# nikisalli/nightmare_rl

Hardware: AMD Instinct MI355X
Metric: env-steps/sec at N parallel Nightmare-v3 envs, 1/2/4/8 MI355X (higher is better)
Workload: dtype f32; 1 GPU; 4096 Nightmare-v3 envs per GPU, random-action rollout U(-1,1)^18, full step(): 2 x 8 ms substeps (18-DoF dynamics + floor contact, PGS x3 + noslip x4) + obs/reward/termination/reset; envs_per_gpu=4096, decimation=2

## Files before the change

### nightmare_rl_amd/csrc/nm_core.h

```cpp
#pragma once
#include <type_traits>
#include <stddef.h>

#include "simt.h"

#ifdef NM_MEASURE
#define NM_ABLATE(mask) (mask)
#else
#define NM_ABLATE(mask) 0
#endif
namespace nm {
using namespace simt;

constexpr int kNQ = 25, kNV = 24, kNU = 18, kNLEG = 6, kNCOL = 7, kNSENS = 13, kNOBS = 66, kNREW = 16;
constexpr int kLinkN = 25;
constexpr int kLegN = 3 * kLinkN;
constexpr int kBaseN = 10;
constexpr int kColN = 24;
constexpr int kMaxCon = 16;
constexpr int kMaxRow = 4 * kMaxCon;
constexpr int kMaxConBig = 44;
constexpr int kBigSlots = (4 * kMaxConBig + NM_WAVE - 1) / NM_WAVE;
constexpr int kJRow = 16;
enum { R_ACTION_RATE, R_ANG_VEL_XY, R_BASE_HEIGHT, R_BODY_CONTACT, R_DEFAULT_POS, R_DOF_ACC, R_DOF_VEL, R_FEET_AIR_TIME, R_FEET_CONTACT,
       R_LIN_VEL_Z, R_ORIENTATION, R_STAND_STILL, R_TORQUES, R_TRACK_ANG, R_TRACK_LIN, R_TERMINATION };

template <class real> struct Model {
  const real* hullv;
  const real* hullnv;
  real legc[kNLEG * kLegN];
  real basec[kBaseN];
  real colc[kNCOL * kColN];
  real footc[kNLEG * 4];
  real qpos0[kNQ];
  int maxnbr;
  int link_rot_id[3];
  real total_mass;
  real h, kv, ctrl_max, grav, mu;
  real solref_K, solref_B, si_d0, si_dmax, si_width, si_mid, si_power;
  real pgs_scale, pgs_tol, noslip_tol, tol_planemesh;
  int pgs_iters, noslip_iters, mpr_iters;
  real mpr_tol;
  real dt, p_gain, clip_obs, obs_lin, obs_ang, obs_dofpos, obs_dofvel, max_lin_x, max_ang, term_force, sigma, max_ep_len, default_pos[3];
  float action_scale, clip_actions;
  int resample_every;
  real rew_scale[kNREW];
  real ep_len_s;
  int rew_extra;
  int tibia_mode, body_mode;
  int collide_batch_min;
  real tibia_max, body_max, base_h_target, max_contact_force;
};

template <class real> struct Args {
  int N;
  uint64_t seed;
  int64_t env_offset;
  real *qpos, *qvel, *qwarm;
  real *dofpos, *dofvel, *act, *cmd, *epsum;
  real* feetair;
  int* feetflags;
  int64_t* eplen;
  uint32_t* rngctr;
  int* hullcache;
  const float* actions;
  const real* cmd_u;
  float *obs, *rew, *timeout_now;
  float* ret_acc;
  int64_t* done;
  real* stat_sum;
  int* stat_cnt;
  int* wave_done;
  int *nto, *to_list;
  int *nprev, *to_prev;
  unsigned long long* to_owner;
  float *ep_stats, *time_outs;
  long long* counters;
  real* dbg;
  int nsub;
  int nxcd;
  int physics_only;
  int ablate;
  const real* noise_vec;
  const real* noise_u;
  uint64_t noise_step;
  real* rec;
  int rec_env;
};
constexpr int kTicketGroup = 64, kTicketStride = 32, kTicketTop = 0;
constexpr uint64_t kNoiseKey = 0x4E4F495345ull;
constexpr int kDbgN = 256;

template <class real> struct Sh {
  real qpos[28], qvel[24], warm[24], ctrl[20];
  real Rb[9], wv[6];
  real anc[kNU * 3], axs[kNU * 3];
  real colR[kNCOL * 9], colp[kNCOL * 3];
  real Minv[kNLEG * 6], W[kNLEG * 18], Lb[15], Dbi[6];
  real MinvH[kNLEG * 6], WH[kNLEG * 18], LbH[15], DbiH[6];
  real qas[24], qfs[24], qfc[24];
  real vv[24];
  real sens[16], cvb[6];
  real bh[2];
  real mbb[36], sc[36];
  real legtmp[kNLEG * 66];
  NM_FN real* cpos() { return legtmp; }
  NM_FN real* cnrm() { return legtmp + 3 * kMaxConBig; }
  NM_FN real* cdist() { return legtmp + 6 * kMaxConBig; }
  NM_FN int* cleg() { return reinterpret_cast<int*>(legtmp + 7 * kMaxConBig); }
  NM_FN int* cleg1() { return reinterpret_cast<int*>(legtmp + 8 * kMaxConBig); }
  real efc_f[kMaxRow];
#ifdef NM_DEBUG_SOLVER
  real dbg_b[kMaxRow], dbg_a[kMaxRow], dbg_f0[kMaxRow];
#endif
  int ncon, nwarn, it_pgs, it_noslip, anypair;
  int nhop;
  int ntog;
  real eact[kNU], epact[kNU], epdv[kNU];
  real ecmd[4], eepsum[kNREW];
  int eplen_lo, eplen_hi;
  unsigned ectr;
  int cstart[8], ccnt[8];
  real sink[NM_WAVE];
  int hcache[8];
};

static_assert(kNLEG * 66 >= 9 * kMaxConBig, "contact list must fit the leg staging area");
template <class real, int G> struct ShW {
  Sh<real> e[G];
  alignas(16) real jrow[kMaxRow * kJRow];
};
#define NM_OFS(field) ((int)(offsetof(Sh<real>, field) / sizeof(real)))
#define NM_IOFS(field) ((int)(offsetof(Sh<real>, field) / sizeof(int)))

template <class A, class B, class C> NM_FN void cross3(A* r, const B* a, const C* b) {
  A x = a[1] * b[2] - a[2] * b[1], y = a[2] * b[0] - a[0] * b[2], z = a[0] * b[1] - a[1] * b[0];
  r[0] = x; r[1] = y; r[2] = z;
}
template <class A, class B, class C> NM_FN A dot3(const B* a, const C* b) { return a[0] * b[0] + a[1] * b[1] + a[2] * b[2]; }
template <class A, class B, class C> NM_FN void matvec3(A* r, const B* m, const C* v) {
  A x = m[0] * v[0] + m[1] * v[1] + m[2] * v[2], y = m[3] * v[0] + m[4] * v[1] + m[5] * v[2], z = m[6] * v[0] + m[7] * v[1] + m[8] * v[2];
  r[0] = x; r[1] = y; r[2] = z;
}
template <class A, class B, class C> NM_FN void matvec3_fma(A* r, const B* m, const C* v) {
  A x = vfma(A(m[2]), A(v[2]), vfma(A(m[1]), A(v[1]), A(m[0]) * A(v[0])));
  A y = vfma(A(m[5]), A(v[2]), vfma(A(m[4]), A(v[1]), A(m[3]) * A(v[0])));
  A z = vfma(A(m[8]), A(v[2]), vfma(A(m[7]), A(v[1]), A(m[6]) * A(v[0])));
  r[0] = x; r[1] = y; r[2] = z;
}
template <class A, class B, class C> NM_FN void matmul3(A* r, const B* a, const C* b) {
#pragma unroll
  for (int i = 0; i < 3; i++)
#pragma unroll
    for (int j = 0; j < 3; j++) r[3 * i + j] = a[3 * i] * b[j] + a[3 * i + 1] * b[3 + j] + a[3 * i + 2] * b[6 + j];
}
template <class A, class B, class C> NM_FN void inert_mul(A* r, const B* i, const C* v) {
  r[0] = i[0] * v[0] + i[3] * v[1] + i[4] * v[2] - i[8] * v[4] + i[7] * v[5];
  r[1] = i[3] * v[0] + i[1] * v[1] + i[5] * v[2] + i[8] * v[3] - i[6] * v[5];
  r[2] = i[4] * v[0] + i[5] * v[1] + i[2] * v[2] - i[7] * v[3] + i[6] * v[4];
  r[3] = i[8] * v[1] - i[7] * v[2] + i[9] * v[3];
  r[4] = i[6] * v[2] - i[8] * v[0] + i[9] * v[4];
  r[5] = i[7] * v[0] - i[6] * v[1] + i[9] * v[5];
}
template <class A, class B, class C> NM_FN void cross_motion(A* r, const B* vel, const C* v) {
  A a[3], b[3], c[3];
  cross3(a, vel, v); cross3(b, vel, v + 3); cross3(c, vel + 3, v);
  r[0] = a[0]; r[1] = a[1]; r[2] = a[2]; r[3] = b[0] + c[0]; r[4] = b[1] + c[1]; r[5] = b[2] + c[2];
}
template <class A, class B, class C> NM_FN void cross_force(A* r, const B* vel, const C* f) {
  A a[3], b[3], c[3];
  cross3(a, vel, f); cross3(b, vel + 3, f + 3); cross3(c, vel, f + 3);
  r[0] = a[0] + b[0]; r[1] = a[1] + b[1]; r[2] = a[2] + b[2]; r[3] = c[0]; r[4] = c[1]; r[5] = c[2];
}
template <class A, class B, class C> NM_FN A dot6(const B* a, const C* b) {
  return a[0] * b[0] + a[1] * b[1] + a[2] * b[2] + a[3] * b[3] + a[4] * b[4] + a[5] * b[5];
}
template <class real> NM_FN real lanesum6(const V<real>& x) {
  return ((rdlane(x, 0) + rdlane(x, 1)) + (rdlane(x, 2) + rdlane(x, 3))) + (rdlane(x, 4) + rdlane(x, 5));
}
template <class X, class real> NM_FN void spatial_inertia(X* I10, const X* R, const X* Ib, const X* d, X m, real) {
  X T[9];
#pragma unroll
  for (int i = 0; i < 3; i++) {
    T[3 * i + 0] = R[3 * i] * Ib[0] + R[3 * i + 1] * Ib[3] + R[3 * i + 2] * Ib[4];
    T[3 * i + 1] = R[3 * i] * Ib[3] + R[3 * i + 1] * Ib[1] + R[3 * i + 2] * Ib[5];
    T[3 * i + 2] = R[3 * i] * Ib[4] + R[3 * i + 1] * Ib[5] + R[3 * i + 2] * Ib[2];
  }
  X xx = T[0] * R[0] + T[1] * R[1] + T[2] * R[2], yy = T[3] * R[3] + T[4] * R[4] + T[5] * R[5], zz = T[6] * R[6] + T[7] * R[7] + T[8] * R[8];
  X xy = T[0] * R[3] + T[1] * R[4] + T[2] * R[5], xz = T[0] * R[6] + T[1] * R[7] + T[2] * R[8], yz = T[3] * R[6] + T[4] * R[7] + T[5] * R[8];
  I10[0] = xx + m * (d[1] * d[1] + d[2] * d[2]);
  I10[1] = yy + m * (d[0] * d[0] + d[2] * d[2]);
  I10[2] = zz + m * (d[0] * d[0] + d[1] * d[1]);
  I10[3] = xy - m * d[0] * d[1];
  I10[4] = xz - m * d[0] * d[2];
  I10[5] = yz - m * d[1] * d[2];
  I10[6] = m * d[0]; I10[7] = m * d[1]; I10[8] = m * d[2];
  I10[9] = m;
}
template <class X, class real> NM_FN void ldl3(X* r, const X* a, real one) {
  X i2 = vrcp(a[5]);
  X l21 = a[4] * i2, l20 = a[2] * i2;
  X m11 = a[3] - l21 * a[4], m01 = a[1] - l21 * a[2], m00 = a[0] - l20 * a[2];
  X i1 = vrcp(m11);
  X l10 = m01 * i1;
  X d0 = m00 - l10 * m01;
  r[0] = l21; r[1] = l20; r[2] = l10; r[3] = i2; r[4] = i1; r[5] = vrcp(d0);
}
template <class X, class Y> NM_FN void ldl3_solve(X* x, const X* f, const Y* y) {
  X y2 = y[2];
  X y1 = y[1] - f[0] * y2;
  X y0 = y[0] - f[1] * y2 - f[2] * y1;
  X x0 = y0 * f[5];
  X x1 = y1 * f[4] - f[2] * x0;
  x[2] = y2 * f[3] - f[0] * x1 - f[1] * x0;
  x[1] = x1; x[0] = x0;
}
template <class X, class real, class Acc> NM_FN void ldl6(Acc S, X* L, X* Dinv, real one) {
  X Lf[36], D[6];
#pragma unroll
  for (int j = 0; j < 6; j++) {
    X d = S(j, j);
#pragma unroll
    for (int k = 0; k < j; k++) d = d - Lf[6 * j + k] * Lf[6 * j + k] * D[k];
    D[j] = d;
    X di = vrcp(d);
    Dinv[j] = di;
#pragma unroll
    for (int i = j + 1; i < 6; i++) {
      X s = S(j, i);
#pragma unroll
      for (int k = 0; k < j; k++) s = s - Lf[6 * i + k] * Lf[6 * j + k] * D[k];
      Lf[6 * i + j] = s * di;
    }
  }
  int n = 0;
#pragma unroll
  for (int i = 1; i < 6; i++)
#pragma unroll
    for (int j = 0; j < i; j++) L[n++] = Lf[6 * i + j];
}
template <class LT, class X> NM_FN void ldl6_solve(const LT* L, const LT* Dinv, X* x) {
  int n = 0;
#pragma unroll
  for (int i = 1; i < 6; i++)
#pragma unroll
    for (int j = 0; j < i; j++) x[i] = x[i] - L[n++] * x[j];
#pragma unroll
  for (int i = 0; i < 6; i++) x[i] = x[i] * Dinv[i];
#pragma unroll
  for (int i = 5; i >= 1; i--) {
    n = i * (i - 1) / 2;
#pragma unroll
    for (int j = 0; j < i; j++) x[j] = x[j] - L[n + j] * x[i];
  }
}

NM_FN uint32_t rand_u24_bits(uint64_t seed, uint64_t genv, uint32_t ctr) {
  uint64_t x = seed + 0x9E3779B97F4A7C15ull * (genv + 1) + 0xD1B54A32D192ED03ull * (uint64_t)ctr;
  x ^= x >> 30; x *= 0xBF58476D1CE4E5B9ull;
  x ^= x >> 27; x *= 0x94D049BB133111EBull;
  x ^= x >> 31;
  return (uint32_t)(x >> 40);
}

#ifndef NM_EMUL
template <class T> NM_FN void nm_consume(T x) { asm volatile("" ::"v"(x) : "memory"); }
#endif

#if defined(NM_STAMPS) && !defined(NM_EMUL)
__device__ unsigned long long g_stamps[16];
NM_FN void nm_stamp(int k) {
  __shared__ unsigned long long tl, acc[16];
#ifdef NM_STAMPS_B
  asm volatile("s_waitcnt vmcnt(0) lgkmcnt(0)" ::: "memory");
#endif
  unsigned long long n = __builtin_amdgcn_s_memtime();
  if (NM_TID == 0) {
    if (k < 0) for (int i = 0; i < 16; i++) acc[i] = 0;
    else acc[k] += n - tl;
    if (k == 10) for (int i = 0; i < 16; i++) atomicAdd(&g_stamps[i], acc[i]);
    tl = n;
  }
}
#else
NM_FN void nm_stamp(int) {}
#endif
#ifdef NM_STAMPS_B
#define NM_ESTAMP(k)
#define NM_BSTAMP(k) nm_stamp(k)
#else
#define NM_ESTAMP(k) nm_stamp(k)
#define NM_BSTAMP(k)
#endif

constexpr int kLinkTmp = 22;

template <class real> NM_FN V<real> legsum(const V<real>& x, const VB& isleg) {
  return gsum8(sel(isleg, x, V<real>(real(0))));
}

template <class real, int G> NM_FN void stage_smooth(ShW<real, G>& w, const Model<real>& M, bool last) {
  typedef V<real> vr;
  real* lds = reinterpret_cast<real*>(&w.e[0]);
  static_assert((G & (G - 1)) == 0 && 2 * G <= 8, "lane groups: G envs x 2 factorisations");
  const V<int> lane0 = opaque_lane();
  const V<int> sub = lane0 & 7, grp = lane0 >> 3;
  const V<int> leg = vmin(sub, V<int>(5)), eo = (grp & (G - 1)) * (int)(sizeof(Sh<real>) / sizeof(real));
  const VB pass1 = (grp & G) != 0;
  const VB isleg = sub < V<int>(6);
#define LDG(field, i) ldsv(lds, eo + (NM_OFS(field) + (i)))
  const VB st_all = VB(true), st_leg = VB(true);
#define STG(field, i, val) stsv(lds, eo + (NM_OFS(field) + (i)), val, st_all)
#define LDL(field, idx) ldsv(lds, eo + (idx) + NM_OFS(field))
#define STL(field, idx, val) stsv(lds, eo + (idx) + NM_OFS(field), val, st_leg)
  const V<int> slot = leg * (3 * kLinkTmp);

  vr Rb[9];
  {
    vr qw = LDG(qpos, 3), qx = LDG(qpos, 4), qy = LDG(qpos, 5), qz = LDG(qpos, 6);
    {
      const vr in_ = vrcp(vsqrt(qw * qw + qx * qx + qy * qy + qz * qz));
      qw = qw * in_; qx = qx * in_; qy = qy * in_; qz = qz * in_;
      STG(qpos, 3, qw); STG(qpos, 4, qx); STG(qpos, 5, qy); STG(qpos, 6, qz);
    }
    vr q00 = qw * qw, q01 = qw * qx, q02 = qw * qy, q03 = qw * qz, q11 = qx * qx, q12 = qx * qy, q13 = qx * qz, q22 = qy * qy,
       q23 = qy * qz, q33 = qz * qz;
    Rb[0] = q00 + q11 - q22 - q33; Rb[4] = q00 - q11 + q22 - q33; Rb[8] = q00 - q11 - q22 + q33;
    Rb[1] = real(2) * (q12 - q03); Rb[2] = real(2) * (q13 + q02); Rb[3] = real(2) * (q12 + q03);
    Rb[5] = real(2) * (q23 - q01); Rb[6] = real(2) * (q13 - q02); Rb[7] = real(2) * (q23 + q01);
  }
  vr vb[6], ab[6];
  {
    vr wl[3] = {LDG(qvel, 3), LDG(qvel, 4), LDG(qvel, 5)};
    matvec3(vb, Rb, wl);
    vb[3] = LDG(qvel, 0); vb[4] = LDG(qvel, 1); vb[5] = LDG(qvel, 2);
    vr t[3];
    cross3(t, vb + 3, vb);
    ab[0] = ab[1] = ab[2] = vr(real(0));
    ab[3] = t[0]; ab[4] = t[1]; ab[5] = t[2] + M.grav;
  }
#pragma unroll
  for (int j = 0; j < 9; j++) { STG(colR, j, Rb[j]); STG(Rb, j, Rb[j]); }
#pragma unroll
  for (int j = 0; j < 3; j++) STG(colp, j, vr(real(0)));
#pragma unroll
  for (int j = 0; j < 6; j++) STG(wv, j, vb[j]);

  const V<int> mylink = (grp >> (G == 1 ? 0 : (G == 2 ? 1 : 2))) & 3;
  const VB isbase = mylink == 3;
#ifndef NM_NO_ROLE_ROT
  {
    const V<int> lk = vmin(mylink, V<int>(2));
    const V<int> cbr = leg * kLegN + lk * kLinkN;
    const vr ax[3] = {ldsv(M.legc, cbr + 12), ldsv(M.legc, cbr + 13), ldsv(M.legc, cbr + 14)};
    vr s_, co;
    vsincos(LDL(qpos, leg * 3 + lk + 7), &s_, &co);
    const vr oc = vr(real(1)) - co;
    vr Rl[9];
    Rl[0] = co + oc * ax[0] * ax[0]; Rl[1] = oc * ax[0] * ax[1] - s_ * ax[2]; Rl[2] = oc * ax[0] * ax[2] + s_ * ax[1];
    Rl[3] = oc * ax[0] * ax[1] + s_ * ax[2]; Rl[4] = co + oc * ax[1] * ax[1]; Rl[5] = oc * ax[1] * ax[2] - s_ * ax[0];
    Rl[6] = oc * ax[0] * ax[2] - s_ * ax[1]; Rl[7] = oc * ax[1] * ax[2] + s_ * ax[0]; Rl[8] = co + oc * ax[2] * ax[2];
#pragma unroll
    for (int j = 0; j < 9; j++) STL(legtmp, leg * 27 + lk * 9 + j, Rl[j]);
    wave_sync();
  }
#endif
  vr mcom[3] = {vr(real(0)), vr(real(0)), vr(real(0))};
  {
    vr Rp[9], pp[3], vpar[6], apar[6];
    vr cR[9], cpos[3], cS[6], cv[6], ca[6];
#pragma unroll
    for (int k = 0; k < 9; k++) Rp[k] = Rb[k];
    pp[0] = pp[1] = pp[2] = vr(real(0));
#pragma unroll
    for (int k = 0; k < 6; k++) { vpar[k] = vb[k]; apar[k] = ab[k]; }
#pragma unroll
    for (int k = 0; k < 3; k++) {
      sched_fence();
      const V<int> cb = leg * kLegN + k * kLinkN;
      vr q = LDL(qpos, leg * 3 + (7 + k)), qd = LDL(qvel, leg * 3 + (6 + k));
      vr pos[3], t3[3], aw[3], R[9];
      {
        vr bpos[3] = {ldsv(M.legc, cb), ldsv(M.legc, cb + 1), ldsv(M.legc, cb + 2)};
        matvec3(t3, Rp, bpos);
        pos[0] = pp[0] + t3[0]; pos[1] = pp[1] + t3[1]; pos[2] = pp[2] + t3[2];
      }
      {
        vr ax[3] = {ldsv(M.legc, cb + 12), ldsv(M.legc, cb + 13), ldsv(M.legc, cb + 14)};
        vr R0[9];
        {
          if (uniform(M.link_rot_id[k])) {
#pragma unroll
            for (int j = 0; j < 9; j++) R0[j] = Rp[j];
          } else {
            vr bR[9];
#pragma unroll
            for (int j = 0; j < 9; j++) bR[j] = ldsv(M.legc, cb + 3 + j);
            matmul3(R0, Rp, bR);
          }
        }
        matvec3(aw, R0, ax);
        vr Rl[9];
#ifndef NM_NO_ROLE_ROT
#pragma unroll
        for (int j = 0; j < 9; j++) Rl[j] = LDL(legtmp, leg * 27 + (k * 9 + j));
        (void)q;
#else
        vr s, co;
        vsincos(q, &s, &co);
        vr oc = vr(real(1)) - co;
        Rl[0] = co + oc * ax[0] * ax[0]; Rl[1] = oc * ax[0] * ax[1] - s * ax[2]; Rl[2] = oc * ax[0] * ax[2] + s * ax[1];
        Rl[3] = oc * ax[0] * ax[1] + s * ax[2]; Rl[4] = co + oc * ax[1] * ax[1]; Rl[5] = oc * ax[1] * ax[2] - s * ax[0];
        Rl[6] = oc * ax[0] * ax[2] - s * ax[1]; Rl[7] = oc * ax[1] * ax[2] + s * ax[0]; Rl[8] = co + oc * ax[2] * ax[2];
#endif
        matmul3(R, R0, Rl);
      }
#pragma unroll
      for (int j = 0; j < 3; j++) {
        STL(anc, leg * 9 + (3 * k + j), pos[j]);
        STL(axs, leg * 9 + (3 * k + j), aw[j]);
      }
      if (k == 2) {
#pragma unroll
        for (int j = 0; j < 9; j++) STL(colR, (leg + 1) * 9 + j, R[j]);
#pragma unroll
        for (int j = 0; j < 3; j++) STL(colp, (leg + 1) * 3 + j, pos[j]);
      }
      sched_fence();
      vr S[6];
      S[0] = aw[0]; S[1] = aw[1]; S[2] = aw[2];
      cross3(S + 3, pos, aw);
      {
        vr Sd[6];
        cross_motion(Sd, vpar, S);
#pragma unroll
        for (int j = 0; j < 6; j++) {
          vpar[j] = vpar[j] + S[j] * qd;
          apar[j] = apar[j] + Sd[j] * qd;
        }
      }
      if (k == 0) {
#pragma unroll
        for (int j = 0; j < 9; j++) cR[j] = sel(isbase, Rb[j], R[j]);
#pragma unroll
        for (int j = 0; j < 3; j++) cpos[j] = sel(isbase, vr(real(0)), pos[j]);
#pragma unroll
        for (int j = 0; j < 6; j++) { cS[j] = S[j]; cv[j] = sel(isbase, vb[j], vpar[j]); ca[j] = sel(isbase, ab[j], apar[j]); }
      } else {
        const VB mine = mylink == k;
#pragma unroll
        for (int j = 0; j < 9; j++) cR[j] = sel(mine, R[j], cR[j]);
#pragma unroll
        for (int j = 0; j < 3; j++) cpos[j] = sel(mine, pos[j], cpos[j]);
#pragma unroll
        for (int j = 0; j < 6; j++) { cS[j] = sel(mine, S[j], cS[j]); cv[j] = sel(mine, vpar[j], cv[j]); ca[j] = sel(mine, apar[j], ca[j]); }
      }
#pragma unroll
      for (int j = 0; j < 9; j++) Rp[j] = R[j];
      pp[0] = pos[0]; pp[1] = pos[1]; pp[2] = pos[2];
    }
    sched_fence();
    {
      static_assert(offsetof(Model<real>, basec) == offsetof(Model<real>, legc) + sizeof(real) * kNLEG * kLegN, "basec follows legc");
      const V<int> cbm = sel(isbase, V<int>(kNLEG * kLegN - 15), leg * kLegN + mylink * kLinkN);
      vr I10[10], f[6];
      {
        vr ipos[3] = {ldsv(M.legc, cbm + 15), ldsv(M.legc, cbm + 16), ldsv(M.legc, cbm + 17)};
        vr Ib[6];
#pragma unroll
        for (int j = 0; j < 6; j++) Ib[j] = ldsv(M.legc, cbm + 18 + j);
        vr mass = ldsv(M.legc, cbm + 24);
        vr d[3], t3[3];
        matvec3(t3, cR, ipos);
        d[0] = cpos[0] + t3[0]; d[1] = cpos[1] + t3[1]; d[2] = cpos[2] + t3[2];
        spatial_inertia(I10, cR, Ib, d, mass, real(0));
        mcom[0] = mass * d[0]; mcom[1] = mass * d[1]; mcom[2] = mass * d[2];
      }
      {
        vr t6[6], u6[6];
        inert_mul(t6, I10, ca);
        inert_mul(u6, I10, cv);
        cross_force(f, cv, u6);
#pragma unroll
        for (int j = 0; j < 6; j++) f[j] = f[j] + t6[j];
      }
      const V<int> o = sel(isbase, V<int>(NM_OFS(sc) + 9 - NM_OFS(legtmp)), slot + mylink * kLinkTmp);
#pragma unroll
      for (int j = 0; j < 6; j++) STL(legtmp, o + j, cS[j]);
#pragma unroll
      for (int j = 0; j < 10; j++) STL(legtmp, o + (6 + j), I10[j]);
#pragma unroll
      for (int j = 0; j < 6; j++) STL(legtmp, o + (16 + j), f[j]);
      if (last) {
#pragma unroll
        for (int j = 0; j < 3; j++) stsv(lds, eo + mylink * 3 + (NM_OFS(sc) + j), legsum<real>(mcom[j], isleg), st_all);
      }
    }
  }
  wave_sync();

  vr Ml[6], Mlb[3][6], cl[3], fs[6], Ic[10];
#pragma unroll
  for (int j = 0; j < 6; j++) fs[j] = vr(real(0));
#pragma unroll
  for (int j = 0; j < 10; j++) Ic[j] = vr(real(0));
#pragma unroll
  for (int k = 2; k >= 0; k--) {
    sched_fence();
    const V<int> o = slot + k * kLinkTmp;
    vr S[6], F[6];
#pragma unroll
    for (int j = 0; j < 6; j++) S[j] = LDL(legtmp, o + j);
#pragma unroll
    for (int j = 0; j < 10; j++) Ic[j] += LDL(legtmp, o + (6 + j));
#pragma unroll
    for (int j = 0; j < 6; j++) fs[j] += LDL(legtmp, o + (16 + j));
    cl[k] = dot6<vr>(S, fs);
    inert_mul(F, Ic, S);
    Mlb[k][0] = F[3]; Mlb[k][1] = F[4]; Mlb[k][2] = F[5];
#pragma unroll
    for (int j = 0; j < 3; j++) Mlb[k][3 + j] = F[0] * Rb[j] + F[1] * Rb[3 + j] + F[2] * Rb[6 + j];
    const int dk = (k == 0) ? 0 : (k == 1 ? 3 : 5);
    Ml[dk] = dot6<vr>(S, F);
#pragma unroll
    for (int jj = 0; jj < k; jj++) {
      vr Sj[6];
#pragma unroll
      for (int j = 0; j < 6; j++) Sj[j] = LDL(legtmp, slot + (jj * kLinkTmp + j));
      Ml[(jj == 0) ? k : 4] = dot6<vr>(Sj, F);
    }
  }
  sched_fence();
  vr Icb[10], cbias[6];
  {
    vr Ib10[10];
#pragma unroll
    for (int j = 0; j < 10; j++) Ib10[j] = LDG(sc, 15 + j);
    if (last) {
      vr ipos[3] = {vr(M.basec[0]), vr(M.basec[1]), vr(M.basec[2])};
      vr d[3];
      matvec3(d, Rb, ipos);
      vr cr[3], t[3];
#pragma unroll
      for (int j = 0; j < 3; j++) cr[j] = (M.basec[9] * d[j] + (LDG(sc, j) + LDG(sc, 3 + j) + LDG(sc, 6 + j))) / M.total_mass;
      cross3(t, vb, cr);
#pragma unroll
      for (int j = 0; j < 3; j++) { STG(cvb, j, vb[j]); STG(cvb, 3 + j, vb[3 + j] + t[j]); }
      STG(bh, 0, LDG(qpos, 2) + d[2]);
    }
    vr fb[6];
#pragma unroll
    for (int j = 0; j < 6; j++) fb[j] = LDG(sc, 25 + j) + legsum<real>(fs[j], isleg);
    cbias[0] = fb[3]; cbias[1] = fb[4]; cbias[2] = fb[5];
#pragma unroll
    for (int j = 0; j < 3; j++) cbias[3 + j] = Rb[j] * fb[0] + Rb[3 + j] * fb[1] + Rb[6 + j] * fb[2];
#pragma unroll
    for (int j = 0; j < 10; j++) Icb[j] = Ib10[j] + legsum<real>(Ic[j], isleg);
  }
  {
#pragma unroll
    for (int i = 0; i < 3; i++)
#pragma unroll
      for (int j = i; j < 3; j++) STG(mbb, 6 * i + j, (i == j) ? Icb[9] : vr(real(0)));
    vr T[9];
#pragma unroll
    for (int j = 0; j < 3; j++) {
      vr a[3] = {Rb[j], Rb[3 + j], Rb[6 + j]}, c[3];
      cross3(c, a, Icb + 6);
#pragma unroll
      for (int i = 0; i < 3; i++) STG(mbb, 6 * i + 3 + j, c[i]);
      T[j] = Icb[0] * a[0] + Icb[3] * a[1] + Icb[4] * a[2];
      T[3 + j] = Icb[3] * a[0] + Icb[1] * a[1] + Icb[5] * a[2];
      T[6 + j] = Icb[4] * a[0] + Icb[5] * a[1] + Icb[2] * a[2];
    }
#pragma unroll
    for (int i = 0; i < 3; i++)
#pragma unroll
      for (int j = i; j < 3; j++) STG(mbb, 6 * (3 + i) + 3 + j, Rb[i] * T[j] + Rb[3 + i] * T[3 + j] + Rb[6 + i] * T[6 + j]);
  }
  wave_sync();

  {
    sched_fence();
    constexpr int kFacH = NM_OFS(MinvH) - NM_OFS(Minv);
    static_assert(NM_OFS(WH) - NM_OFS(W) == kFacH && NM_OFS(LbH) - NM_OFS(Lb) == kFacH && NM_OFS(DbiH) - NM_OFS(Dbi) == kFacH, "factor blocks");
    static_assert(kNLEG * 66 >= 36 + 24 + 24, "leg staging area holds the second Schur complement and the junk rows");
    const V<int> eoF = eo + sel(pass1, V<int>(kFacH), V<int>(0));
    const V<int> eoS = eo + sel(pass1, V<int>(NM_OFS(legtmp)), V<int>(NM_OFS(sc)));
    const V<int> eoQ = eo + sel(pass1, V<int>(NM_OFS(legtmp) + 36), V<int>(NM_OFS(qfs)));
    const V<int> eoA = eo + sel(pass1, V<int>(NM_OFS(legtmp) + 60), V<int>(NM_OFS(qas)));
    vr Mh[6];
    const vr dg = sel(pass1, vr(M.h * M.kv), vr(real(0)));
    Mh[0] = Ml[0] + dg; Mh[1] = Ml[1]; Mh[2] = Ml[2]; Mh[3] = Ml[3] + dg; Mh[4] = Ml[4]; Mh[5] = Ml[5] + dg;
    vr Mi[6], W[3][6];
    ldl3(Mi, Mh, real(1));
#pragma unroll
    for (int j = 0; j < 6; j++) {
      vr col[3] = {Mlb[0][j], Mlb[1][j], Mlb[2][j]}, r3[3];
      ldl3_solve(r3, Mi, col);
      W[0][j] = r3[0]; W[1][j] = r3[1]; W[2][j] = r3[2];
    }
#pragma unroll
    for (int j = 0; j < 6; j++) stsv(lds, eoF + leg * 6 + (NM_OFS(Minv) + j), Mi[j], st_leg);
#pragma unroll
    for (int k = 0; k < 3; k++)
#pragma unroll
      for (int j = 0; j < 6; j++) stsv(lds, eoF + leg * 18 + (NM_OFS(W) + 6 * k + j), W[k][j], st_leg);
#pragma unroll
    for (int i = 0; i < 6; i++)
#pragma unroll
      for (int j = i; j < 6; j++) {
        vr cij = Mlb[0][i] * W[0][j] + Mlb[1][i] * W[1][j] + Mlb[2][i] * W[2][j];
        stsv(lds, eoS + (6 * i + j), LDG(mbb, 6 * i + j) - legsum<real>(cij, isleg), st_all);
      }
    wave_sync();
    vr L[15], Di[6];
    ldl6([&](int r, int c) { return ldsv(lds, eoS + (6 * r + c)); }, L, Di, real(1));
#pragma unroll
    for (int j = 0; j < 15; j++) stsv(lds, eoF + (NM_OFS(Lb) + j), L[j], st_all);
#pragma unroll
    for (int j = 0; j < 6; j++) stsv(lds, eoF + (NM_OFS(Dbi) + j), Di[j], st_all);
    {
      vr y[3], t[3];
#pragma unroll
      for (int k = 0; k < 3; k++) {
        vr ctrl = LDL(ctrl, leg * 3 + k), qd = LDL(qvel, leg * 3 + (6 + k));
        ctrl = vmin(vmax(ctrl, vr(-M.ctrl_max)), vr(M.ctrl_max));
        y[k] = M.kv * ctrl - M.kv * qd - cl[k];
        stsv(lds, eoQ + leg * 3 + (6 + k), y[k], st_leg);
      }
      ldl3_solve(t, Mi, y);
      vr xb[6];
#pragma unroll
      for (int j = 0; j < 6; j++) {
        vr wy = W[0][j] * y[0] + W[1][j] * y[1] + W[2][j] * y[2];
        xb[j] = -cbias[j] - legsum<real>(wy, isleg);
        stsv(lds, eoQ + j, -cbias[j], st_all);
      }
      ldl6_solve(L, Di, xb);
#pragma unroll
      for (int j = 0; j < 6; j++) stsv(lds, eoA + j, xb[j], st_all);
#pragma unroll
      for (int k = 0; k < 3; k++) {
        vr x = t[k];
#pragma unroll
        for (int j = 0; j < 6; j++) x = x - W[k][j] * xb[j];
        stsv(lds, eoA + leg * 3 + (6 + k), x, st_leg);
      }
    }
  }
  wave_sync();
#undef LDG
#undef STG
#undef LDL
#undef STL
}

template <class real> struct Sup { real v[3], v1[3], v2[3]; };
template <class real> NM_FN real ccd_eps() { return sizeof(real) == 8 ? real(2.220446049250313e-16) : real(1.1920929e-7); }
template <class real> NM_FN bool ccd_zero(real x) { return vabs(x) < ccd_eps<real>(); }
template <class real> NM_FN bool ccd_eq(real a, real b) {
  real ab = vabs(a - b);
  if (ab < ccd_eps<real>()) return true;
  real fa = vabs(a), fb = vabs(b);
  return ab < ccd_eps<real>() * (fb > fa ? fb : fa);
}
template <class acc, class real> NM_FN void hull_support(const Sh<real>& sh, const Model<real>& M, int g, const acc* dir, acc* out) {
  typedef V<acc> vr;
  const V<int> lane = lane_id();
  acc R[9], p[3];
#pragma unroll
  for (int j = 0; j < 9; j++) R[j] = (acc)sh.colR[9 * g + j];
#pragma unroll
  for (int j = 0; j < 3; j++) p[j] = (acc)sh.colp[3 * g + j];
  const real* cc = M.colc + kColN * g;
  const int nvert = (int)cc[5], vadr = (int)cc[6];
  const acc ld[3] = {R[0] * dir[0] + R[3] * dir[1] + R[6] * dir[2], R[1] * dir[0] + R[4] * dir[1] + R[7] * dir[2],
                     R[2] * dir[0] + R[5] * dir[1] + R[8] * dir[2]};
  vr best = vr(acc(-1e30));
  for (int it = 0; it * NM_WAVE < nvert; it++) {
    V<int> vi = lane + it * NM_WAVE;
    VB ok = vi < nvert;
    V<int> ad = (sel(ok, vi, V<int>(0)) + vadr) * 4;
    vr val = ld[0] * vcvt<acc>(gldv(M.hullv, ad)) + ld[1] * vcvt<acc>(gldv(M.hullv, ad + 1)) + ld[2] * vcvt<acc>(gldv(M.hullv, ad + 2));
    best = sel(ok & (val > best), val, best);
  }
  acc sv; int si;
  wargmax(best, lane, &sv, &si);
  V<int> ifirst = V<int>(1 << 30);
  for (int it = 0; it * NM_WAVE < nvert; it++) {
    V<int> vi = lane + it * NM_WAVE;
    VB ok = vi < nvert;
    V<int> ad = (sel(ok, vi, V<int>(0)) + vadr) * 4;
    vr val = ld[0] * vcvt<acc>(gldv(M.hullv, ad)) + ld[1] * vcvt<acc>(gldv(M.hullv, ad + 1)) + ld[2] * vcvt<acc>(gldv(M.hullv, ad + 2));
    ifirst = sel(ok & (val >= vr(sv - acc(1e-7))) & (vi < ifirst), vi, ifirst);
  }
  wargmax(to_real<acc>(-ifirst), lane, &sv, &si);
  si = (int)(-sv);
  const real* vp = M.hullv + 4 * (vadr + si);
  const acc v[3] = {(acc)vp[0], (acc)vp[1], (acc)vp[2]};
  acc t[3];
  matvec3(t, R, v);
  out[0] = p[0] + t[0]; out[1] = p[1] + t[1]; out[2] = p[2] + t[2];
}
template <class acc, class real> NM_COLD void mpr_support(const Sh<real>& sh, const Model<real>& M, int g1, int g2, const acc* dir, Sup<acc>& s) {
  acc nd[3] = {-dir[0], -dir[1], -dir[2]};
  hull_support<acc>(sh, M, g1, dir, s.v1);
  hull_support<acc>(sh, M, g2, nd, s.v2);
  s.v[0] = s.v1[0] - s.v2[0]; s.v[1] = s.v1[1] - s.v2[1]; s.v[2] = s.v1[2] - s.v2[2];
}
template <class real> NM_FN void sub3(real* r, const real* a, const real* b) { r[0] = a[0] - b[0]; r[1] = a[1] - b[1]; r[2] = a[2] - b[2]; }
template <class real> NM_FN void ccd_normalize(real* v) { real s = real(1) / vsqrt(v[0] * v[0] + v[1] * v[1] + v[2] * v[2]); v[0] *= s; v[1] *= s; v[2] *= s; }
template <class real> NM_FN void portal_dir(const Sup<real>* p, real* dir) {
  real a[3], b[3];
  sub3(a, p[2].v, p[1].v); sub3(b, p[3].v, p[1].v);
  cross3(dir, a, b);
  ccd_normalize(dir);
}
template <class real> NM_FN bool portal_reach_tol(const Sup<real>* p, const Sup<real>& v4, const real* dir, real tol) {
  real dv4 = dot3<real>(v4.v, dir);
  real d1 = dv4 - dot3<real>(p[1].v, dir), d2 = dv4 - dot3<real>(p[2].v, dir), d3 = dv4 - dot3<real>(p[3].v, dir);
  real m = vmin(vmin(d1, d2), d3);
  return ccd_eq(m, tol) || m < tol;
}
template <class real> NM_FN void expand_portal(Sup<real>* p, const Sup<real>& v4) {
  real v4v0[3];
  cross3(v4v0, v4.v, p[0].v);
  if (dot3<real>(p[1].v, v4v0) > real(0)) {
    if (dot3<real>(p[2].v, v4v0) > real(0)) p[1] = v4; else p[3] = v4;
  } else {
    if (dot3<real>(p[3].v, v4v0) > real(0)) p[2] = v4; else p[1] = v4;
  }
}
template <class real> NM_FN real point_seg_dist2(const real* x0, const real* b, real* wit) {
  real dd[3];
  sub3(dd, b, x0);
  real t = -dot3<real>(x0, dd) / dot3<real>(dd, dd);
  if (t < real(0) || ccd_zero(t)) { wit[0] = x0[0]; wit[1] = x0[1]; wit[2] = x0[2]; }
  else if (t > real(1) || ccd_eq(t, real(1))) { wit[0] = b[0]; wit[1] = b[1]; wit[2] = b[2]; }
  else { wit[0] = x0[0] + t * dd[0]; wit[1] = x0[1] + t * dd[1]; wit[2] = x0[2] + t * dd[2]; }
  return dot3<real>(wit, wit);
}
template <class real> NM_FN real point_tri_dist2(const real* x0, const real* B, const real* C, real* wit) {
  real d1[3], d2[3];
  sub3(d1, B, x0); sub3(d2, C, x0);
  real v = dot3<real>(d1, d1), w = dot3<real>(d2, d2), p = dot3<real>(x0, d1), q = dot3<real>(x0, d2), r = dot3<real>(d1, d2);
  real dd = w * v - r * r, s, t;
  if (ccd_zero(dd)) { s = real(-1); t = real(-1); }
  else { s = (q * r - w * p) / dd; t = (-s * r - q) / w; }
  if ((ccd_zero(s) || s > real(0)) && (ccd_eq(s, real(1)) || s < real(1)) && (ccd_zero(t) || t > real(0)) && (ccd_eq(t, real(1)) || t < real(1)) &&
      (ccd_eq(t + s, real(1)) || t + s < real(1))) {
    wit[0] = x0[0] + s * d1[0] + t * d2[0]; wit[1] = x0[1] + s * d1[1] + t * d2[1]; wit[2] = x0[2] + s * d1[2] + t * d2[2];
    return dot3<real>(wit, wit);
  }
  real w2[3];
  real dist = point_seg_dist2(x0, B, wit);
  real dist2 = point_seg_dist2(x0, C, w2);
  if (dist2 < dist) { dist = dist2; wit[0] = w2[0]; wit[1] = w2[1]; wit[2] = w2[2]; }
  dist2 = point_seg_dist2(B, C, w2);
  if (dist2 < dist) { dist = dist2; wit[0] = w2[0]; wit[1] = w2[1]; wit[2] = w2[2]; }
  return dist;
}
template <class real_, class st> NM_COLD bool mpr_penetration(const Sh<st>& sh, const Model<st>& M, int g1, int g2, real_* depth, real_* dir_out, real_* pos) {
  typedef real_ real;
  Sup<real> p[4], v4;
  real dir[3], va[3], vb[3], dot;
  const real mpr_tol = (real)M.mpr_tol;
  {
    real R1[9], R2[9], c1[3], c2[3];
#pragma unroll
    for (int k = 0; k < 9; k++) { R1[k] = (real)sh.colR[9 * g1 + k]; R2[k] = (real)sh.colR[9 * g2 + k]; }
#pragma unroll
    for (int k = 0; k < 3; k++) { c1[k] = (real)M.colc[kColN * g1 + k]; c2[k] = (real)M.colc[kColN * g2 + k]; }
    real t1[3], t2[3];
    matvec3(t1, R1, c1); matvec3(t2, R2, c2);
#pragma unroll
    for (int k = 0; k < 3; k++) {
      p[0].v1[k] = (real)sh.colp[3 * g1 + k] + t1[k];
      p[0].v2[k] = (real)sh.colp[3 * g2 + k] + t2[k];
      p[0].v[k] = p[0].v1[k] - p[0].v2[k];
    }
  }
  if (ccd_eq(p[0].v[0], real(0)) && ccd_eq(p[0].v[1], real(0)) && ccd_eq(p[0].v[2], real(0))) p[0].v[0] += ccd_eps<real>() * real(10);
  dir[0] = -p[0].v[0]; dir[1] = -p[0].v[1]; dir[2] = -p[0].v[2];
  ccd_normalize(dir);
  mpr_support<real>(sh, M, g1, g2, dir, p[1]);
  dot = dot3<real>(p[1].v, dir);
  if (ccd_zero(dot) || dot < real(0)) return false;
  cross3(dir, p[0].v, p[1].v);
  if (ccd_zero(dot3<real>(dir, dir))) {
    if (ccd_eq(p[1].v[0], real(0)) && ccd_eq(p[1].v[1], real(0)) && ccd_eq(p[1].v[2], real(0))) return false;
    *depth = vsqrt(dot3<real>(p[1].v, p[1].v));
    dir_out[0] = p[1].v[0]; dir_out[1] = p[1].v[1]; dir_out[2] = p[1].v[2];
    ccd_normalize(dir_out);
#pragma unroll
    for (int k = 0; k < 3; k++) pos[k] = real(0.5) * (p[1].v1[k] + p[1].v2[k]);
    return true;
  }
  ccd_normalize(dir);
  mpr_support<real>(sh, M, g1, g2, dir, p[2]);
  dot = dot3<real>(p[2].v, dir);
  if (ccd_zero(dot) || dot < real(0)) return false;
  sub3(va, p[1].v, p[0].v); sub3(vb, p[2].v, p[0].v);
  cross3(dir, va, vb);
  ccd_normalize(dir);
  if (dot3<real>(dir, p[0].v) > real(0)) {
    Sup<real> t = p[1]; p[1] = p[2]; p[2] = t;
    dir[0] = -dir[0]; dir[1] = -dir[1]; dir[2] = -dir[2];
  }
  for (int size = 3, guard = 0; size < 4; guard++) {
    if (guard > 64) return false;
    mpr_support<real>(sh, M, g1, g2, dir, p[3]);
    dot = dot3<real>(p[3].v, dir);
    if (ccd_zero(dot) || dot < real(0)) return false;
    bool cont = false;
    cross3(va, p[1].v, p[3].v);
    dot = dot3<real>(va, p[0].v);
    if (dot < real(0) && !ccd_zero(dot)) { p[2] = p[3]; cont = true; }
    if (!cont) {
      cross3(va, p[3].v, p[2].v);
      dot = dot3<real>(va, p[0].v);
      if (dot < real(0) && !ccd_zero(dot)) { p[1] = p[3]; cont = true; }
    }
    if (cont) {
      sub3(va, p[1].v, p[0].v); sub3(vb, p[2].v, p[0].v);
      cross3(dir, va, vb);
      ccd_normalize(dir);
    } else size = 4;
  }
  for (int guard = 0;; guard++) {
    portal_dir(p, dir);
    dot = dot3<real>(dir, p[1].v);
    if (ccd_zero(dot) || dot > real(0)) break;
    if (guard > 100) return false;
    mpr_support<real>(sh, M, g1, g2, dir, v4);
    dot = dot3<real>(v4.v, dir);
    if (!(ccd_zero(dot) || dot > real(0)) || portal_reach_tol(p, v4, dir, mpr_tol)) return false;
    expand_portal(p, v4);
  }
  for (int it = 0;; it++) {
    portal_dir(p, dir);
    mpr_support<real>(sh, M, g1, g2, dir, v4);
    if (portal_reach_tol(p, v4, dir, mpr_tol) || it > M.mpr_iters) {
      real pd[3];
      *depth = vsqrt(point_tri_dist2(p[1].v, p[2].v, p[3].v, pd));
      if (ccd_zero(pd[0]) && ccd_zero(pd[1]) && ccd_zero(pd[2])) { pd[0] = dir[0]; pd[1] = dir[1]; pd[2] = dir[2]; }
      ccd_normalize(pd);
      dir_out[0] = pd[0]; dir_out[1] = pd[1]; dir_out[2] = pd[2];
      real b[4], t[3], sum;
      portal_dir(p, dir);
      cross3(t, p[1].v, p[2].v); b[0] = dot3<real>(t, p[3].v);
      cross3(t, p[3].v, p[2].v); b[1] = dot3<real>(t, p[0].v);
      cross3(t, p[0].v, p[1].v); b[2] = dot3<real>(t, p[3].v);
      cross3(t, p[2].v, p[1].v); b[3] = dot3<real>(t, p[0].v);
      sum = b[0] + b[1] + b[2] + b[3];
      if (ccd_zero(sum) || sum < real(0)) {
        b[0] = real(0);
        cross3(t, p[2].v, p[3].v); b[1] = dot3<real>(t, dir);
        cross3(t, p[3].v, p[1].v); b[2] = dot3<real>(t, dir);
        cross3(t, p[1].v, p[2].v); b[3] = dot3<real>(t, dir);
        sum = b[1] + b[2] + b[3];
      }
      real inv = real(1) / sum;
#pragma unroll
      for (int k = 0; k < 3; k++) {
        real p1 = b[0] * p[0].v1[k] + b[1] * p[1].v1[k] + b[2] * p[2].v1[k] + b[3] * p[3].v1[k];
        real p2 = b[0] * p[0].v2[k] + b[1] * p[1].v2[k] + b[2] * p[2].v2[k] + b[3] * p[3].v2[k];
        pos[k] = real(0.5) * (p1 * inv + p2 * inv);
      }
      return true;
    }
    expand_portal(p, v4);
  }
}

template <class real> NM_FN void pairs_narrow(Sh<real>& sh, const Model<real>& M, int* dropped, uint64_t m) {
  if (!m) return;
  int ncon = sh.ncon;
  while (m) {
    int pidx = __builtin_ctzll(m);
    m &= m - 1;
    int a = (pidx >= 5) + (pidx >= 9) + (pidx >= 12) + (pidx >= 14);
    int s0 = a == 0 ? 0 : (a == 1 ? 5 : (a == 2 ? 9 : (a == 3 ? 12 : 14)));
    int h1 = a + 1, h2 = h1 + 1 + (pidx - s0);
    {
      const real *R1 = sh.colR + 9 * h1, *R2 = sh.colR + 9 * h2, *k1 = M.colc + kColN * h1, *k2 = M.colc + kColN * h2;
      real t1[3], t2[3], dd[3];
      matvec3(t1, R1, k1); matvec3(t2, R2, k2);
#pragma unroll
      for (int k = 0; k < 3; k++) dd[k] = (sh.colp[3 * h1 + k] + t1[k]) - (sh.colp[3 * h2 + k] + t2[k]);
      real bound = k1[3] + k2[3];
      if (dot3<real>(dd, dd) > bound * bound) continue;
    }
    typedef double acc;
    acc depth, dir[3], pos[3];
    if (!mpr_penetration<acc>(sh, M, h1, h2, &depth, dir, pos)) continue;
    if (!(depth > acc(0))) continue;
    if (ncon >= kMaxConBig) { *dropped += 1; continue; }
    sh.cpos()[3 * ncon] = (real)pos[0]; sh.cpos()[3 * ncon + 1] = (real)pos[1]; sh.cpos()[3 * ncon + 2] = (real)pos[2];
    sh.cnrm()[3 * ncon] = (real)dir[0]; sh.cnrm()[3 * ncon + 1] = (real)dir[1]; sh.cnrm()[3 * ncon + 2] = (real)dir[2];
    sh.cdist()[ncon] = (real)(-depth);
    sh.cleg()[ncon] = h2 - 1;
    sh.cleg1()[ncon] = h1 - 1;
    sh.anypair = 1;
    ncon++;
  }
  sh.ncon = ncon;
  wave_sync();
}


template <class real> NM_FN void stage_collide_pairs(Sh<real>& sh, const Model<real>& M, int* dropped) {
  typedef V<real> vr;
  const V<int> lane = lane_id();
  const VB isp = lane < 15;
  const V<int> pl = sel(isp, lane, V<int>(0));
  V<int> i1 = sel(pl >= 5, V<int>(1), V<int>(0)) + sel(pl >= 9, V<int>(1), V<int>(0)) + sel(pl >= 12, V<int>(1), V<int>(0)) +
              sel(pl >= 14, V<int>(1), V<int>(0));
  V<int> st = sel(i1 == 0, V<int>(0), sel(i1 == 1, V<int>(5), sel(i1 == 2, V<int>(9), sel(i1 == 3, V<int>(12), V<int>(14)))));
  V<int> g1 = i1 + 1, g2 = g1 + 1 + (pl - st);
  vr c1[3], c2[3], e[2];
  V<int> gg[2] = {g1, g2};
  vr u[3];
#pragma unroll
// ... 98 lines not shown
    best = sel(take, val, best);
    ibest = sel(take, vi, ibest);
  }
  real sv; int si;
  wmaxfirst(best, &sv, &si);
  if (popc64(ballot(best == vr(sv))) == 1) return rdlane(ibest, si);
  wargmax(best, ibest, &sv, &si);
  return si;
}
template <class real> NM_FN real hull_tie_tol() { return sizeof(real) == 8 ? real(1e-13) : real(4e-7); }
constexpr int kMaxHop = 3;
template <class real> constexpr real kObbSlack() { return real(1e-5); }

constexpr int kSelfLane = 63;
constexpr int kSlackScale = 1 << 20;
constexpr int kBatchLane0 = kSelfLane + 1 - kNCOL;
template <class real> NM_FN void hull_ring(const Model<real>& M, int gv, V<int>& nbg, V<real>* v) {
  const V<int> lane = lane_id();
  const VB nbl = lane < M.maxnbr;
  V<real> o[4];
  gld4(M.hullnv, (sel(nbl, lane, V<int>(M.maxnbr)) + gv * (M.maxnbr + 1)) * 4, o);
  v[0] = o[0]; v[1] = o[1]; v[2] = o[2];
  nbg = to_int(o[3]);
}
template <class real> struct Rings {
  V<int> nb[kNCOL];
  V<real> vv[kNCOL][3];
  int cur[kNCOL];
};
template <class real> NM_FN void collide_rings(const Sh<real>& sh, const Model<real>& M, Rings<real>& r) {
#pragma unroll
  for (int g = 0; g < kNCOL; g++) {
    const int vadr = (int)M.colc[kColN * g + 6];
    r.cur[g] = uniform(sh.hcache[g]);
    hull_ring(M, vadr + r.cur[g], r.nb[g], r.vv[g]);
  }
}
template <class real> NM_FN void stage_collide(Sh<real>& sh, const Model<real>& M, int* dropped, Rings<real>& rg, bool pairs = true) {
  typedef V<real> vr;
  const V<int> lane = lane_id();
  const real bz = sh.qpos[2];
  const VB nbl = lane < M.maxnbr;
  V<int>* nb = rg.nb;
  vr (*vv)[3] = rg.vv;
  int* cur = rg.cur;
  real pz[kNCOL], ldv[kNCOL][3], sv[kNCOL];
  bool near[kNCOL];
  vr val[kNCOL];
#pragma unroll
  for (int g = 0; g < kNCOL; g++) {
    const real* R = sh.colR + 9 * g;
    const real* cc = M.colc + kColN * g;
    pz[g] = sh.colp[3 * g + 2] + bz;
    const real cz = R[6] * cc[0] + R[7] * cc[1] + R[8] * cc[2] + pz[g];
    near[g] = !(cz - cc[3] > real(0));
    ldv[g][0] = -R[6]; ldv[g][1] = -R[7]; ldv[g][2] = -R[8];
    val[g] = ldv[g][0] * vv[g][0] + ldv[g][1] * vv[g][1] + ldv[g][2] * vv[g][2];
    sv[g] = rdlane(val[g], kSelfLane);
  }
  NM_BSTAMP(11);
#pragma unroll
  for (int g = 0; g < kNCOL; g++) {
    const real tol = hull_tie_tol<real>();
    if (near[g] && wany(nbl & (nb[g] >= 0) & (val[g] >= vr(sv[g] - tol)))) {
      {
        const real* cc = M.colc + kColN * g;
        real top = ldv[g][0] * cc[8] + ldv[g][1] * cc[9] + ldv[g][2] * cc[10];
#pragma unroll
        for (int a = 0; a < 3; a++) top += cc[20 + a] * vabs(ldv[g][0] * cc[11 + 3 * a] + ldv[g][1] * cc[12 + 3 * a] + ldv[g][2] * cc[13 + 3 * a]);
        if (uniform(pz[g] - top > kObbSlack<real>())) { near[g] = false; continue; }
      }
      const int nvert = (int)M.colc[kColN * g + 5], vadr = (int)M.colc[kColN * g + 6];
      const real* ld = ldv[g];
      int si = cur[g];
      bool full = false;
      for (int hop = 0;; hop++) {
        const VB nbv = nbl & (nb[g] >= 0);
        if (!wany(nbv & (val[g] >= vr(sv[g] - tol)))) break;
        if (hop == kMaxHop || !wany(nbv & (val[g] > vr(sv[g] + tol)))) { full = true; break; }
        real bv; int lbest;
        wmaxfirst(sel(nbv, val[g], vr(real(-1e30))), &bv, &lbest);
        si = rdlane(nb[g], lbest);
        NM_BSTAMP(12);
        hull_ring(M, vadr + si, nb[g], vv[g]);
        val[g] = ld[0] * vv[g][0] + ld[1] * vv[g][1] + ld[2] * vv[g][2];
        sv[g] = rdlane(val[g], kSelfLane);
        NM_BSTAMP(14);
        sh.nhop += 1;
      }
      if (full) {
        NM_BSTAMP(12);
        const int held = si;
        si = support_exhaustive(M, ld, nvert, vadr);
        sh.hcache[7] += 1;
#ifdef NM_MEASURE
        sh.nhop += g == 0 ? 1000 : 100000;
#endif
        if (si != held) {
          hull_ring(M, vadr + si, nb[g], vv[g]);
          val[g] = ld[0] * vv[g][0] + ld[1] * vv[g][1] + ld[2] * vv[g][2];
          sv[g] = rdlane(val[g], kSelfLane);
        }
        NM_BSTAMP(15);
      }
      if (si != cur[g]) sh.hcache[g] = si;
    }
  }
  NM_BSTAMP(12);
  int total = 0;
  unsigned hitbits = 0;
#pragma unroll
  for (int g = 0; g < kNCOL; g++) hitbits |= (uniform(near[g] && pz[g] - sv[g] < real(0)) ? 1u : 0u) << g;
  const int nhit = popc64(hitbits);
  bool batch = false;
  if (nhit >= M.collide_batch_min) {
    const uint64_t hitm = (uint64_t)hitbits << kBatchLane0;
    vr X[3] = {vv[kNCOL - 1][0], vv[kNCOL - 1][1], vv[kNCOL - 1][2]}, svl = val[kNCOL - 1];
    V<int> slackl = nb[kNCOL - 1];
    V<int> lb = lane;
#pragma unroll
    for (int g = kNCOL - 2; g >= 0; g--) {
      order_after(lb, X[0]);
      const VB mg = lb == kBatchLane0 + g;
      X[0] = sel(mg, vv[g][0], X[0]); X[1] = sel(mg, vv[g][1], X[1]); X[2] = sel(mg, vv[g][2], X[2]);
      svl = sel(mg, val[g], svl);
      slackl = sel(mg, nb[g], slackl);
    }
    const VB ml = lane >= kBatchLane0;
    const V<int> gl = sel(ml, lane - kBatchLane0, V<int>(0));
    const vr pzl = ldsv(sh.colp, gl * 3 + 2) + bz;
    const vr distl = pzl - svl;
    const VB wr = in_mask(hitm);
    const VB lone = distl * real(-0.5 * kSlackScale) < to_real<real>(slackl);
    if (!wany(wr & !lone)) {
      vr Rl[9], pl[2], pnt[3];
#pragma unroll
      for (int j = 0; j < 9; j++) Rl[j] = ldsv(sh.colR, gl * 9 + j);
#pragma unroll
      for (int j = 0; j < 2; j++) pl[j] = ldsv(sh.colp, gl * 3 + j);
      matvec3_fma(pnt, Rl, X);
      pnt[0] = pnt[0] + pl[0]; pnt[1] = pnt[1] + pl[1]; pnt[2] = pnt[2] + ldsv(sh.colp, gl * 3 + 2);
      const V<int> slot = lane_rank(hitm);
      const V<int> sl = sel(wr, slot, V<int>(0));
      stsv(sh.cpos(), sl * 3, pnt[0], wr);
      stsv(sh.cpos(), sl * 3 + 1, pnt[1], wr);
      stsv(sh.cpos(), sl * 3 + 2, pnt[2] - real(0.5) * distl, wr);
      stsv(sh.cdist(), sl, distl, wr);
      stsv(sh.cleg(), sl, gl - 1, wr);
      stsv(sh.cstart, gl, slot, ml);
      stsv(sh.ccnt, gl, sel(wr, V<int>(1), V<int>(0)), ml);
      total = nhit;
      batch = true;
    }
  }
  if (!batch) {
#pragma unroll
  for (int g = 0; g < kNCOL; g++) {
    const real* R = sh.colR + 9 * g;
    const real* p = sh.colp + 3 * g;
    const real dist = pz[g] - sv[g];
    const bool hitg = (hitbits >> g) & 1;
    int nextra = 0;
    if (hitg) {
      vr pnt[3];
      matvec3_fma(pnt, R, vv[g]);
      pnt[0] = pnt[0] + p[0]; pnt[1] = pnt[1] + p[1]; pnt[2] = pnt[2] + p[2];
      const real first[3] = {rdlane(pnt[0], kSelfLane), rdlane(pnt[1], kSelfLane), rdlane(pnt[2], kSelfLane) - real(0.5) * dist};
      const real tol = M.tol_planemesh * M.colc[kColN * g + 3];
      vr dd[3] = {pnt[0] - first[0], pnt[1] - first[1], pnt[2] - first[2]};
      vr d2 = dd[0] * dd[0] + dd[1] * dd[1] + dd[2] * dd[2];
      const VB ok = nbl & (nb[g] >= 0) & (val[g] > vr(pz[g])) & !(d2 < vr(tol * tol));
      const uint64_t m = ballot(ok);
      if (m == 0) {
        const VB wr = (lane == kSelfLane) & VB(total < kMaxConBig);
        const int sl = vmin(total, kMaxConBig - 1);
        stsv(sh.cpos(), V<int>(sl * 3), pnt[0], wr);
        stsv(sh.cpos(), V<int>(sl * 3 + 1), pnt[1], wr);
        stsv(sh.cpos(), V<int>(sl * 3 + 2), pnt[2] - real(0.5) * dist, wr);
        stsv(sh.cdist(), V<int>(sl), vr(dist), wr);
        stsv(sh.cleg(), V<int>(sl), V<int>(g - 1), wr);
      } else {
      nextra = vmin(popc64(m), 3);
      const V<int> rank = lane_rank(m);
      const VB self = lane == kSelfLane;
      const V<int> slot = sel(self, V<int>(total), rank + (total + 1));
      const VB wr = (self | (ok & (rank < 3))) & (slot < kMaxConBig);
      const V<int> sl = sel(wr, slot, V<int>(0));
      const vr cd = sel(self, vr(dist), pnt[2] + bz);
      stsu(sh.cpos(), sl * 3, pnt[0], wr, sh.sink);
      stsu(sh.cpos(), sl * 3 + 1, pnt[1], wr, sh.sink);
      stsu(sh.cpos(), sl * 3 + 2, pnt[2] - real(0.5) * cd, wr, sh.sink);
      stsu(sh.cdist(), sl, cd, wr, sh.sink);
      stsu(sh.cleg(), sl, V<int>(g - 1), wr, sh.sink);
      }
    }
    const int ng = hitg ? 1 + nextra : 0;
    const int c0 = vmin(total, kMaxConBig), c1 = vmin(total + ng, kMaxConBig);
    sh.cstart[g] = c0;
    sh.ccnt[g] = c1 - c0;
    total += ng;
  }
  }
  const int ncon = vmin(total, kMaxConBig);
  *dropped += total - ncon;
  sh.ncon = ncon;
  sh.cstart[7] = ncon;
  sh.anypair = 0;
  wave_sync();
  NM_BSTAMP(13);
  nm_stamp(3);
  if (pairs) stage_collide_pairs(sh, M, dropped);
  nm_stamp(4);
}


template <int C, int N, class F> NM_FN void for_contacts(int ncon, F&& f) {
  if constexpr (C < N) {
    if (C < ncon) {
      f(std::integral_constant<int, C>{});
      for_contacts<C + 1, N>(ncon, f);
    }
  }
}
template <class F> NM_FN void sfor4(F&& f) {
  f(std::integral_constant<int, 0>{}); f(std::integral_constant<int, 1>{}); f(std::integral_constant<int, 2>{}); f(std::integral_constant<int, 3>{});
}
template <int NP, int P = 0, class F> NM_FN void sfor_pairs(int ncon, F&& f) {
  if constexpr (P < NP) {
    if (P / 2 < ncon) {
      f(std::integral_constant<int, P>{});
      f(std::integral_constant<int, P + 1>{});
      sfor_pairs<NP, P + 2>(ncon, f);
    }
  }
}
template <class X> NM_FN void pgs_row_prepare(const X& Rr, const X& f, const X& ARinv, X& k0, X& k1, X& nf) {
  k0 = -ARinv;
  k1 = (Rr * f) * k0;
  nf = -f;
}
template <class X> NM_FN X pgs_row_delta(const X& g, const X& k0, const X& k1, const X& nf) { return vmax(vfma(g, k0, k1), nf); }
template <class X> NM_FN X pgs_row_cost(const X& dl, const X& hA, const X& g, const X& Rr, const X& f) { return dl * vfma(hA, dl, vfma(Rr, f, g)); }
template <class real, class X, class B> NM_FN void noslip_pair_prepare(const X& f, const X& fp, const B& small, X& lo, X& hi) {
  const X mean = real(0.5) * (fp - f);
  lo = sel(small, mean, -f);
  hi = sel(small, mean, fp);
}
template <class X> NM_FN X noslip_pair_delta(const X& dg, const X& invK1, const X& lo, const X& hi) { return vmin(vmax(-dg * invK1, lo), hi); }
template <class X> NM_FN X noslip_pair_cost(const X& d, const X& hK1, const X& dg) { return d * vfma(hK1, d, dg); }
template <class real, class X> NM_FN auto noslip_pair_bad(const X& change) { return change > X(real(1e-10)); }

template <class real, bool PAIR> NM_FN void stage_constraint_body(Sh<real>& sh, real* jrow, const Model<real>& M, bool last, bool nosweep) {
  typedef V<real> vr;
  const V<int> lane = lane_id();
  const int ncon = uniform(sh.ncon), nefc = 4 * ncon;
  if (nefc == 0) {
#pragma unroll
    for (int j = 0; j < 24; j++) sh.qfc[j] = real(0);
    if (last)
#pragma unroll
      for (int j = 0; j < kNSENS; j++) sh.sens[j] = real(0);
    wave_sync();
    return;
  }
  const VB act = lane < nefc;
  const V<int> c = sel(act, lane >> 2, V<int>(0));
  const V<int> tk = (lane >> 1) & 1, sg = lane & 1;
  vr cp[3] = {ldsv(sh.cpos(), c * 3), ldsv(sh.cpos(), c * 3 + 1), ldsv(sh.cpos(), c * 3 + 2)};
  vr dist = ldsv(sh.cdist(), c);
  V<int> L = ldsv(sh.cleg(), c);
  const VB onleg = L >= 0;
  const V<int> Lc = vmax(L, V<int>(0));
  constexpr bool anypair = PAIR;
  V<int> L1 = V<int>(-1);
  if (anypair) L1 = ldsv(sh.cleg1(), c);
  const VB onleg1 = L1 >= 0;
  const V<int> Lc1 = vmax(L1, V<int>(0));
  const V<int> q4 = lane & 3;
  vr smu = sel(sg == 0, vr(M.mu), vr(-M.mu));
  vr nrm[3] = {vr(real(0)), vr(real(0)), vr(real(1))};
  vr e[3] = {sel(q4 == 2, vr(real(-1)), vr(real(0))), sel(q4 == 1, vr(real(1)), vr(real(0))), sel((q4 == 0) | (q4 == 3), vr(real(1)), vr(real(0)))};
  if (anypair) {
    nrm[0] = ldsv(sh.cnrm(), c * 3); nrm[1] = ldsv(sh.cnrm(), c * 3 + 1); nrm[2] = ldsv(sh.cnrm(), c * 3 + 2);
    VB usey = (nrm[1] < vr(real(0.5))) & (nrm[1] > vr(real(-0.5)));
    vr y0[3] = {vr(real(0)), sel(usey, vr(real(1)), vr(real(0))), sel(usey, vr(real(0)), vr(real(1)))};
    vr dt = nrm[1] * y0[1] + nrm[2] * y0[2];
    vr t1[3] = {y0[0] - dt * nrm[0], y0[1] - dt * nrm[1], y0[2] - dt * nrm[2]}, t2[3];
    vr il = vr(real(1)) / vsqrt(t1[0] * t1[0] + t1[1] * t1[1] + t1[2] * t1[2]);
    t1[0] = t1[0] * il; t1[1] = t1[1] * il; t1[2] = t1[2] * il;
    cross3(t2, nrm, t1);
#pragma unroll
    for (int j = 0; j < 3; j++) e[j] = sel(q4 == 1, t1[j], sel(q4 == 2, t2[j], nrm[j]));
  }
  vr Fb[6], Fl[3], Fm[3] = {vr(real(0)), vr(real(0)), vr(real(0))};
  {
    vr m[3];
    cross3(m, cp, e);
    Fb[0] = e[0]; Fb[1] = e[1]; Fb[2] = e[2];
#pragma unroll
    for (int j = 0; j < 3; j++) Fb[3 + j] = sh.Rb[j] * m[0] + sh.Rb[3 + j] * m[1] + sh.Rb[6 + j] * m[2];
#pragma unroll
    for (int k = 0; k < 3; k++) {
      vr a[3], r[3], rel[3], mm[3];
#pragma unroll
      for (int j = 0; j < 3; j++) {
        a[j] = ldsv(sh.axs, Lc * 9 + (3 * k + j));
        r[j] = ldsv(sh.anc, Lc * 9 + (3 * k + j));
        rel[j] = cp[j] - r[j];
      }
      cross3(mm, rel, e);
      Fl[k] = sel(onleg, dot3<vr>(a, mm), vr(real(0)));
    }
  }
  if (anypair) {
#pragma unroll
    for (int k = 0; k < 3; k++) {
      vr a[3], r[3], rel[3], mm[3];
#pragma unroll
      for (int j = 0; j < 3; j++) {
        a[j] = ldsv(sh.axs, Lc1 * 9 + (3 * k + j));
        r[j] = ldsv(sh.anc, Lc1 * 9 + (3 * k + j));
        rel[j] = cp[j] - r[j];
      }
      cross3(mm, rel, e);
      Fm[k] = sel(onleg1 & act, -dot3<vr>(a, mm), vr(real(0)));
    }
#pragma unroll
    for (int j = 0; j < 6; j++) Fb[j] = sel(onleg1, vr(real(0)), Fb[j]);
  }
#pragma unroll
  for (int j = 0; j < 6; j++) Fb[j] = sel(act, Fb[j], vr(real(0)));
#pragma unroll
  for (int k = 0; k < 3; k++) Fl[k] = sel(act, Fl[k], vr(real(0)));
  vr uF[6];
#pragma unroll
  for (int j = 0; j < 6; j++) {
    uF[j] = Fb[j];
#pragma unroll
    for (int k = 0; k < 3; k++) uF[j] = uF[j] - ldsv(sh.W, Lc * 18 + (6 * k + j)) * Fl[k];
  }
  if (anypair) {
#pragma unroll
    for (int j = 0; j < 6; j++)
#pragma unroll
      for (int k = 0; k < 3; k++) uF[j] = uF[j] - ldsv(sh.W, Lc1 * 18 + (6 * k + j)) * Fm[k];
  }
#pragma unroll
  for (int j = 0; j < 6; j++) stsv(jrow, lane * kJRow + j, uF[j], lane < kMaxRow);
#pragma unroll
  for (int k = 0; k < 3; k++) stsv(jrow, lane * kJRow + (6 + k), Fl[k], lane < kMaxRow);
  if (anypair) {
#pragma unroll
    for (int k = 0; k < 3; k++) stsv(jrow, lane * kJRow + (10 + k), Fm[k], lane < kMaxRow);
  }
  vr Jb[6], Jl[3], Jm[3] = {vr(real(0)), vr(real(0)), vr(real(0))};
#pragma unroll
  for (int j = 0; j < 6; j++) Jb[j] = quad<0x00>(Fb[j]) + smu * quad<0xA5>(Fb[j]);
#pragma unroll
  for (int k = 0; k < 3; k++) Jl[k] = quad<0x00>(Fl[k]) + smu * quad<0xA5>(Fl[k]);
  if (anypair) {
#pragma unroll
    for (int k = 0; k < 3; k++) Jm[k] = quad<0x00>(Fm[k]) + smu * quad<0xA5>(Fm[k]);
  }
  vr u[6];
#pragma unroll
  for (int j = 0; j < 6; j++) u[j] = quad<0x00>(uF[j]) + smu * quad<0xA5>(uF[j]);

  vr imp;
  {
    vr x = vabs(dist) * vrcp(M.si_width);
    vr ylo, yhi;
    if (M.si_power == real(2)) {
      vr omx = vmax(vr(real(1)) - x, vr(real(0)));
      ylo = (x * x) * vrcp(M.si_mid);
      yhi = vr(real(1)) - (omx * omx) * vrcp(real(1) - M.si_mid);
    } else {
      ylo = vpow(x, vr(M.si_power)) / vpow(vr(M.si_mid), vr(M.si_power - real(1)));
      yhi = vr(real(1)) - vpow(vmax(vr(real(1)) - x, vr(real(0))), vr(M.si_power)) / vpow(vr(real(1) - M.si_mid), vr(M.si_power - real(1)));
    }
    vr y = sel(x <= vr(M.si_mid), ylo, yhi);
    imp = M.si_d0 + y * (M.si_dmax - M.si_d0);
    imp = sel(x >= vr(real(1)), vr(M.si_dmax), imp);
    imp = sel(x <= vr(real(0)), vr(M.si_d0), imp);
  }
  vr invw = ldsv(M.colc, (Lc + sel(onleg, V<int>(1), V<int>(0))) * kColN + 4);
  if (anypair) invw = invw + sel(onleg1, ldsv(M.colc, (Lc1 + 1) * kColN + 4), vr(real(0)));
  vr Rr = vmax((vr(real(1)) - imp) * (invw + M.mu * M.mu * invw) * vrcp(imp), vr(real(1e-15))) * (real(2) * M.mu * M.mu);
  vr Dd = vrcp(Rr);
  vr vel = vr(real(0)), jas = vr(real(0)), jaw = vr(real(0));
#pragma unroll
  for (int j = 0; j < 6; j++) {
    vel += Jb[j] * sh.qvel[j]; jas += Jb[j] * sh.qas[j]; jaw += Jb[j] * sh.warm[j];
  }
#pragma unroll
  for (int k = 0; k < 3; k++) {
    V<int> di = Lc * 3 + (6 + k);
    vel += Jl[k] * ldsv(sh.qvel, di); jas += Jl[k] * ldsv(sh.qas, di); jaw += Jl[k] * ldsv(sh.warm, di);
  }
  if (anypair) {
#pragma unroll
    for (int k = 0; k < 3; k++) {
      V<int> di = Lc1 * 3 + (6 + k);
      vel += Jm[k] * ldsv(sh.qvel, di); jas += Jm[k] * ldsv(sh.qas, di); jaw += Jm[k] * ldsv(sh.warm, di);
    }
  }
  vr aref = -M.solref_B * vel - M.solref_K * imp * dist;
  vr bb = jas - aref;

  vr t[3], t1m[3] = {vr(real(0)), vr(real(0)), vr(real(0))}, xb[6];
  {
    vr Mi[6];
#pragma unroll
    for (int j = 0; j < 6; j++) Mi[j] = ldsv(sh.Minv, Lc * 6 + j);
    ldl3_solve(t, Mi, Jl);
    if (anypair) {
      vr Mi1[6];
#pragma unroll
      for (int j = 0; j < 6; j++) Mi1[j] = ldsv(sh.Minv, Lc1 * 6 + j);
      ldl3_solve(t1m, Mi1, Jm);
    }
#pragma unroll
    for (int j = 0; j < 6; j++) xb[j] = u[j];
    ldl6_solve(sh.Lb, sh.Dbi, xb);
  }
  wave_sync();
  vr A[kMaxRow];
#pragma unroll
  for (int i = 0; i < kMaxRow; i++) A[i] = vr(real(0));
  auto build_contact = [&](auto ccT) {
    constexpr int cc = decltype(ccT)::value;
    if (cc < ncon) {
      const int Lcc = uniform(sh.cleg()[cc]);
      const VB same = onleg & (L == Lcc);
      VB s01 = VB(false), s10 = VB(false), s11 = VB(false);
      if (anypair) {
        const int L1cc = uniform(sh.cleg1()[cc]);
        s01 = onleg1 & (L1 == Lcc);
        s10 = onleg & (L == L1cc);
        s11 = onleg1 & (L1 == L1cc);
      }
      vr a3[3];
  #pragma unroll
      for (int r = 0; r < 3; r++) {
        const real* jr = jrow + (4 * cc + r) * kJRow;
        vr a = jr[0] * xb[0] + jr[1] * xb[1] + jr[2] * xb[2] + jr[3] * xb[3] + jr[4] * xb[4] + jr[5] * xb[5];
        a += sel(same, jr[6] * t[0] + jr[7] * t[1] + jr[8] * t[2], vr(real(0)));
        if (anypair) {
          a += sel(s01, jr[6] * t1m[0] + jr[7] * t1m[1] + jr[8] * t1m[2], vr(real(0)));
          a += sel(s10, jr[10] * t[0] + jr[11] * t[1] + jr[12] * t[2], vr(real(0)));
          a += sel(s11, jr[10] * t1m[0] + jr[11] * t1m[1] + jr[12] * t1m[2], vr(real(0)));
        }
        a3[r] = a;
      }
      A[4 * cc] = a3[0] + M.mu * a3[1];
      A[4 * cc + 1] = a3[0] - M.mu * a3[1];
      A[4 * cc + 2] = a3[0] + M.mu * a3[2];
      A[4 * cc + 3] = a3[0] - M.mu * a3[2];
    }
  };
#define NM_BUILD4(c0) build_contact(std::integral_constant<int, c0>{}); build_contact(std::integral_constant<int, c0 + 1>{}); \
                      build_contact(std::integral_constant<int, c0 + 2>{}); build_contact(std::integral_constant<int, c0 + 3>{});
  NM_BUILD4(0) NM_BUILD4(4) NM_BUILD4(8) NM_BUILD4(12)
#undef NM_BUILD4
  vr Ajj = u[0] * xb[0] + u[1] * xb[1] + u[2] * xb[2] + u[3] * xb[3] + u[4] * xb[4] + u[5] * xb[5] + (Jl[0] * t[0] + Jl[1] * t[1] + Jl[2] * t[2]);
  if (anypair) Ajj += Jm[0] * t1m[0] + Jm[1] * t1m[1] + Jm[2] * t1m[2];
  vr ARjj = Ajj + Rr;
  vr ARinv = sel(act, vrcp(ARjj), vr(real(0)));

  nm_stamp(5);
  vr jar = jaw - aref;
  vr f = sel(act & (jar < vr(real(0))), -Dd * jar, vr(real(0)));
  vr g = bb;
  for_contacts<0, kMaxCon>(ncon, [&](auto ccT) {
    constexpr int cc = decltype(ccT)::value;
#pragma unroll
    for (int r = 0; r < 4; r++) g += A[4 * cc + r] * rdlane(f, 4 * cc + r);
  });
  {
    real cost = wsum<real>(sel(act, f * (bb + real(0.5) * (g - bb + Rr * f)), vr(real(0))));
    if (cost > real(0)) { f = vr(real(0)); g = bb; }
  }
#ifdef NM_DEBUG_SOLVER
  stsv(sh.dbg_b, lane, bb, lane < kMaxRow); stsv(sh.dbg_a, lane, ARjj, lane < kMaxRow); stsv(sh.dbg_f0, lane, f, lane < kMaxRow);
#endif
  const vr hA = real(0.5) * ARjj;
  for (int iter = 0; iter < (nosweep ? 0 : M.pgs_iters); iter++) {
    vr k0, k1, nf;
    pgs_row_prepare(Rr, f, ARinv, k0, k1, nf);
    vr gcap = g;
    uint64_t rowm = mask_shl(1ull, 0);
    for_contacts<0, kMaxCon>(ncon, [&](auto ccT) {
      constexpr int cc = decltype(ccT)::value;
      sfor4([&](auto rT) {
        constexpr int i = 4 * cc + decltype(rT)::value;
        gcap = sel_mask(rowm, g, gcap);
        rowm = mask_shl(rowm, 1);
        const vr dl = pgs_row_delta(g, k0, k1, nf);
        g = vfma(A[i], vr(rdlane(dl, i)), g);
      });
    });
    const vr dcap = pgs_row_delta(gcap, k0, k1, nf);
    const vr ccap = pgs_row_cost(dcap, hA, gcap, Rr, f);
    f = f + dcap;
    sh.it_pgs = iter + 1;
    if (-wsum<real>(ccap) * M.pgs_scale < M.pgs_tol) break;
  }
  nm_stamp(6);
  {
    const V<int> lv = opaque_lane();
    const VB even = (lv & 1) == 0;
    vr Amq = vr(real(0));
    for_contacts<0, kMaxCon>(ncon, [&](auto ccT) {
      constexpr int cc = decltype(ccT)::value;
      Amq = sel(lv == 4 * cc, A[4 * cc + 1], Amq);
      Amq = sel(lv == 4 * cc + 2, A[4 * cc + 3], Amq);
    });
    Amq = sel(even, Amq, shfl_xor1(Amq));
    const vr K1 = Ajj + shfl_xor1(Ajj) - Amq - Amq;
    const VB small = K1 < vr(real(1e-15));
    const vr invK1 = vrcp(K1), hK1 = real(0.5) * K1;
    for_contacts<0, kMaxCon>(ncon, [&](auto ccT) {
      constexpr int cc = decltype(ccT)::value;
      A[4 * cc] = A[4 * cc] - A[4 * cc + 1];
      A[4 * cc + 2] = A[4 * cc + 2] - A[4 * cc + 3];
    });
    for (int iter = 0; iter < (nosweep ? 0 : M.noslip_iters); iter++) {
      real improvement = real(0);
      if (iter == 0) improvement = wsum<real>(sel(act, real(0.5) * f * f * Rr, vr(real(0))));
      vr lo, hi;
      noslip_pair_prepare<real>(f, shfl_xor1(f), small, lo, hi);
      vr dcap = vr(real(0)), dgcap = vr(real(0));
      uint64_t pairm = mask_shl(3ull, 0);
      sfor_pairs<kMaxRow / 2>(ncon, [&](auto pT) {
        constexpr int p = decltype(pT)::value;
        const vr dg = g - shfl_xor1(g);
        vr d = noslip_pair_delta(dg, invK1, lo, hi);
        d = sel(noslip_pair_bad<real>(noslip_pair_cost(d, hK1, dg)), vr(real(0)), d);
        g = vfma(A[2 * p], vr(rdlane(d, 2 * p)), g);
        dcap = sel_mask(pairm, d, dcap);
        dgcap = sel_mask(pairm, dg, dgcap);
        pairm = mask_shl(pairm, 2);
      });
      f = f + dcap;
      improvement = improvement - wsum<real>(sel(even, noslip_pair_cost(dcap, hK1, dgcap), vr(real(0))));
      sh.it_noslip = iter + 1;
      if (improvement * M.pgs_scale < M.noslip_tol) break;
    }
  }
  nm_stamp(7);
  stsv(sh.efc_f, lane, f, lane < kMaxRow);
  vr nf = vr(real(0));
  VB hit = VB(false), hit1 = VB(false);
  if (last) {
    nf = f + shfl_xor1(f);
    nf = nf + shfl_xor2(nf);
    auto foot_hit = [&](const V<int>& Lx, real sgn) {
      vr ft[3], fr, s[3], Rt[9];
#pragma unroll
      for (int j = 0; j < 3; j++) s[j] = ldsv(M.footc, Lx * 4 + j);
      fr = ldsv(M.footc, Lx * 4 + 3);
#pragma unroll
      for (int j = 0; j < 9; j++) Rt[j] = ldsv(sh.colR, (Lx + 1) * 9 + j);
      matvec3(ft, Rt, s);
#pragma unroll
      for (int j = 0; j < 3; j++) ft[j] = ft[j] + ldsv(sh.colp, (Lx + 1) * 3 + j);
      vr dif[3] = {cp[0] - ft[0], cp[1] - ft[1], cp[2] - ft[2]};
      vr b2 = sgn * (nrm[0] * dif[0] + nrm[1] * dif[1] + nrm[2] * dif[2]);
      vr cc = dif[0] * dif[0] + dif[1] * dif[1] + dif[2] * dif[2] - fr * fr;
      vr det = b2 * b2 - cc;
      vr sq = vsqrt(vmax(det, vr(real(0))));
      return !(det < vr(real(1e-15))) & (((-b2 - sq) >= vr(real(0))) | ((-b2 + sq) >= vr(real(0))));
    };
    hit = foot_hit(Lc, real(-1));
    if (anypair) hit1 = foot_hit(Lc1, real(1));
  }
#pragma unroll
  for (int j = 0; j < 6; j++) sh.qfc[j] = wsum<real>(Jb[j] * f);
  if (!anypair) {
    vr s3[3];
#pragma unroll
    for (int k = 0; k < 3; k++) {
      vr x = Jl[k] * f;
      x = x + shfl_xor1(x);
      s3[k] = x + shfl_xor2(x);
    }
    const vr tn = sel(act & (nf > vr(real(0))), nf, vr(real(0))), tf = sel(hit, tn, vr(real(0)));
    const VB lead = act & ((lane & 3) == 0);
    wave_sync();
#pragma unroll
    for (int k = 0; k < 3; k++) stsv(jrow, c * 8 + k, s3[k], lead);
    if (last) { stsv(jrow, c * 8 + 3, tn, lead); stsv(jrow, c * 8 + 4, tf, lead); }
    wave_sync();
    const VB on = lane < 30;
    const V<int> lg = sel(on, (lane * 13) >> 6, V<int>(0)), qq = lane - lg * 5;
    const V<int> c0 = ldsv(sh.cstart, lg + 1), cn = ldsv(sh.ccnt, lg + 1);
    vr acc = vr(real(0));
#pragma unroll
    for (int k = 0; k < 4; k++) {
      VB in = on & (cn > k);
      acc = acc + sel(in, ldsv(jrow, sel(in, (c0 + k) * 8 + qq, V<int>(0))), vr(real(0)));
    }
    stsv(sh.qfc, 6 + lg * 3 + qq, acc, on & (qq < 3));
    if (last) {
      stsv(sh.sens, lg, acc, on & (qq == 3));
      stsv(sh.sens, lg + 6, acc, on & (qq == 4));
      sh.sens[12] = wsum<real>(sel(act & ((lane & 3) == 0) & (L < 0), tn, vr(real(0))));
    }
  } else {
#pragma unroll
    for (int l = 0; l < 6; l++)
#pragma unroll
      for (int k = 0; k < 3; k++) sh.qfc[6 + 3 * l + k] = wsum<real>(sel(L == l, Jl[k] * f, vr(real(0))) + sel(L1 == l, Jm[k] * f, vr(real(0))));
    if (last) {
      VB head = act & ((lane & 3) == 0) & (nf > vr(real(0)));
#pragma unroll
      for (int l = 0; l < 6; l++) {
        VB onl = (L == l) | (L1 == l);
        sh.sens[l] = wsum<real>(sel(head & onl, nf, vr(real(0))));
        sh.sens[6 + l] = wsum<real>(sel(head & (((L == l) & hit) | ((L1 == l) & hit1)), nf, vr(real(0))));
      }
      sh.sens[12] = wsum<real>(sel(head & (L < 0), nf, vr(real(0))));
    }
  }
  wave_sync();
}

template <class real> NM_COLD void stage_constraint_pairs(Sh<real>& sh, real* jrow, const Model<real>& M, bool last, bool nosweep) {
  stage_constraint_body<real, true>(sh, jrow, M, last, nosweep);
}

constexpr int kMaxCon2 = 8, kMaxRow2 = 4 * kMaxCon2;
#ifdef NM_EMUL
inline long& nm_emul_together() { static long n = 0; return n; }
#endif
template <class real> NM_FN void stage_constraint2(ShW<real, 2>& w, const Model<real>& M, bool last, bool nosweep) {
  typedef V<real> vr;
  constexpr int kSR = (int)(sizeof(Sh<real>) / sizeof(real)), kSI = (int)(sizeof(Sh<real>) / sizeof(int));
  const V<int> lane = lane_id();
  const V<int> h = lane >> 5, hl = lane & 31;
  const VB h1 = h != 0;
  real* rbw = reinterpret_cast<real*>(&w.e[0]);
  int* ibw = reinterpret_cast<int*>(&w.e[0]);
  const real* rb = rbw;
  const int* ib = ibw;
  real* jrow = w.jrow;
  const V<int> ho = h * kSR, hoi = h * kSI, jh = h * (kMaxRow2 * kJRow);
  const int oLeg = NM_OFS(legtmp);
  const int oCleg = (int)((offsetof(Sh<real>, legtmp) + 7 * kMaxConBig * sizeof(real)) / sizeof(int));
#define SHR(field, idx) ldsv(rb, ho + ((idx) + NM_OFS(field)))
#define SHI(field, idx) ldsv(ib, hoi + ((idx) + NM_IOFS(field)))
  const int n0 = uniform(w.e[0].ncon), n1 = uniform(w.e[1].ncon), nmax = vmax(n0, n1);
  const V<int> nconv = sel(h1, V<int>(n1), V<int>(n0)), nefc = nconv * 4;
  const VB act = hl < nefc;
  const V<int> c = sel(act, hl >> 2, V<int>(0));
  const V<int> sg = hl & 1;
  vr cp[3] = {ldsv(rb, ho + (c * 3 + oLeg)), ldsv(rb, ho + (c * 3 + (oLeg + 1))), ldsv(rb, ho + (c * 3 + (oLeg + 2)))};
  vr dist = ldsv(rb, ho + (c + (oLeg + 6 * kMaxConBig)));
  V<int> L = ldsv(ib, hoi + (c + oCleg));
  {
    const VB any = nconv > 0;
    cp[0] = sel(any, cp[0], vr(real(0))); cp[1] = sel(any, cp[1], vr(real(0))); cp[2] = sel(any, cp[2], vr(real(0)));
    dist = sel(any, dist, vr(real(0)));
    L = sel(any, L, V<int>(-1));
  }
  const VB onleg = L >= 0;
  const V<int> Lc = vmax(L, V<int>(0));
  const V<int> q4 = hl & 3;
  vr smu = sel(sg == 0, vr(M.mu), vr(-M.mu));
  vr nrm[3] = {vr(real(0)), vr(real(0)), vr(real(1))};
  vr e[3] = {sel(q4 == 2, vr(real(-1)), vr(real(0))), sel(q4 == 1, vr(real(1)), vr(real(0))), sel((q4 == 0) | (q4 == 3), vr(real(1)), vr(real(0)))};
  vr Fb[6], Fl[3];
  {
    vr m[3];
    cross3(m, cp, e);
    Fb[0] = e[0]; Fb[1] = e[1]; Fb[2] = e[2];
#pragma unroll
    for (int j = 0; j < 3; j++) Fb[3 + j] = SHR(Rb, V<int>(j)) * m[0] + SHR(Rb, V<int>(3 + j)) * m[1] + SHR(Rb, V<int>(6 + j)) * m[2];
#pragma unroll
    for (int k = 0; k < 3; k++) {
      vr a[3], r[3], rel[3], mm[3];
#pragma unroll
      for (int j = 0; j < 3; j++) {
        a[j] = SHR(axs, Lc * 9 + (3 * k + j));
        r[j] = SHR(anc, Lc * 9 + (3 * k + j));
        rel[j] = cp[j] - r[j];
      }
      cross3(mm, rel, e);
      Fl[k] = sel(onleg, dot3<vr>(a, mm), vr(real(0)));
    }
  }
#pragma unroll
  for (int j = 0; j < 6; j++) Fb[j] = sel(act, Fb[j], vr(real(0)));
#pragma unroll
  for (int k = 0; k < 3; k++) Fl[k] = sel(act, Fl[k], vr(real(0)));
  vr uF[6];
#pragma unroll
  for (int j = 0; j < 6; j++) {
    uF[j] = Fb[j];
#pragma unroll
    for (int k = 0; k < 3; k++) uF[j] = uF[j] - SHR(W, Lc * 18 + (6 * k + j)) * Fl[k];
  }
#pragma unroll
  for (int j = 0; j < 6; j++) stsv(jrow, lane * kJRow + j, uF[j], VB(true));
#pragma unroll
  for (int k = 0; k < 3; k++) stsv(jrow, lane * kJRow + (6 + k), Fl[k], VB(true));
  vr Jb[6], Jl[3];
#pragma unroll
  for (int j = 0; j < 6; j++) Jb[j] = quad<0x00>(Fb[j]) + smu * quad<0xA5>(Fb[j]);
#pragma unroll
  for (int k = 0; k < 3; k++) Jl[k] = quad<0x00>(Fl[k]) + smu * quad<0xA5>(Fl[k]);
  vr u[6];
#pragma unroll
  for (int j = 0; j < 6; j++) u[j] = quad<0x00>(uF[j]) + smu * quad<0xA5>(uF[j]);

  vr imp;
  {
    vr x = vabs(dist) * vrcp(M.si_width);
    vr ylo, yhi;
    if (M.si_power == real(2)) {
      vr omx = vmax(vr(real(1)) - x, vr(real(0)));
      ylo = (x * x) * vrcp(M.si_mid);
      yhi = vr(real(1)) - (omx * omx) * vrcp(real(1) - M.si_mid);
    } else {
      ylo = vpow(x, vr(M.si_power)) / vpow(vr(M.si_mid), vr(M.si_power - real(1)));
      yhi = vr(real(1)) - vpow(vmax(vr(real(1)) - x, vr(real(0))), vr(M.si_power)) / vpow(vr(real(1) - M.si_mid), vr(M.si_power - real(1)));
    }
    vr y = sel(x <= vr(M.si_mid), ylo, yhi);
    imp = M.si_d0 + y * (M.si_dmax - M.si_d0);
    imp = sel(x >= vr(real(1)), vr(M.si_dmax), imp);
    imp = sel(x <= vr(real(0)), vr(M.si_d0), imp);
  }
  vr invw = ldsv(M.colc, (Lc + sel(onleg, V<int>(1), V<int>(0))) * kColN + 4);
  vr Rr = vmax((vr(real(1)) - imp) * (invw + M.mu * M.mu * invw) * vrcp(imp), vr(real(1e-15))) * (real(2) * M.mu * M.mu);
  vr Dd = vrcp(Rr);
  vr vel = vr(real(0)), jas = vr(real(0)), jaw = vr(real(0));
#pragma unroll
  for (int j = 0; j < 6; j++) {
    vel += Jb[j] * SHR(qvel, V<int>(j)); jas += Jb[j] * SHR(qas, V<int>(j)); jaw += Jb[j] * SHR(warm, V<int>(j));
  }
#pragma unroll
  for (int k = 0; k < 3; k++) {
    V<int> di = Lc * 3 + (6 + k);
    vel += Jl[k] * SHR(qvel, di); jas += Jl[k] * SHR(qas, di); jaw += Jl[k] * SHR(warm, di);
  }
  vr aref = -M.solref_B * vel - M.solref_K * imp * dist;
  vr bb = jas - aref;

  vr t[3], xb[6];
  {
    vr Mi[6];
#pragma unroll
    for (int j = 0; j < 6; j++) Mi[j] = SHR(Minv, Lc * 6 + j);
    ldl3_solve(t, Mi, Jl);
    vr Lbv[15], Dbv[6];
#pragma unroll
    for (int j = 0; j < 15; j++) Lbv[j] = SHR(Lb, V<int>(j));
#pragma unroll
    for (int j = 0; j < 6; j++) Dbv[j] = SHR(Dbi, V<int>(j));
#pragma unroll
    for (int j = 0; j < 6; j++) xb[j] = u[j];
    ldl6_solve(Lbv, Dbv, xb);
  }
  wave_sync();
  vr A[kMaxRow2];
#pragma unroll
  for (int i = 0; i < kMaxRow2; i++) A[i] = vr(real(0));
  auto build_contact = [&](auto ccT) {
    constexpr int cc = decltype(ccT)::value;
    if (cc < nmax) {
      const V<int> Lcc = ldsv(ib, hoi + (cc + oCleg));
      const VB same = onleg & (L == Lcc);
      const VB has = V<int>(cc) < nconv;
      vr a3[3];
#pragma unroll
      for (int r = 0; r < 3; r++) {
        const V<int> jr = jh + (4 * cc + r) * kJRow;
        vr a = ldsv(jrow, jr) * xb[0] + ldsv(jrow, jr + 1) * xb[1] + ldsv(jrow, jr + 2) * xb[2] + ldsv(jrow, jr + 3) * xb[3] + ldsv(jrow, jr + 4) * xb[4] +
               ldsv(jrow, jr + 5) * xb[5];
        a += sel(same, ldsv(jrow, jr + 6) * t[0] + ldsv(jrow, jr + 7) * t[1] + ldsv(jrow, jr + 8) * t[2], vr(real(0)));
        a3[r] = a;
      }
      A[4 * cc] = sel(has, a3[0] + M.mu * a3[1], vr(real(0)));
      A[4 * cc + 1] = sel(has, a3[0] - M.mu * a3[1], vr(real(0)));
      A[4 * cc + 2] = sel(has, a3[0] + M.mu * a3[2], vr(real(0)));
      A[4 * cc + 3] = sel(has, a3[0] - M.mu * a3[2], vr(real(0)));
    }
  };
#define NM_BUILD4(c0) build_contact(std::integral_constant<int, c0>{}); build_contact(std::integral_constant<int, c0 + 1>{}); \
                      build_contact(std::integral_constant<int, c0 + 2>{}); build_contact(std::integral_constant<int, c0 + 3>{});
  NM_BUILD4(0) NM_BUILD4(4)
#undef NM_BUILD4
  vr Ajj = u[0] * xb[0] + u[1] * xb[1] + u[2] * xb[2] + u[3] * xb[3] + u[4] * xb[4] + u[5] * xb[5] + (Jl[0] * t[0] + Jl[1] * t[1] + Jl[2] * t[2]);
  vr ARjj = Ajj + Rr;
  vr ARinv = sel(act, vrcp(ARjj), vr(real(0)));

  nm_stamp(5);
  vr jar = jaw - aref;
  vr f = sel(act & (jar < vr(real(0))), -Dd * jar, vr(real(0)));
  vr g = bb;
  for_contacts<0, kMaxCon2>(nmax, [&](auto ccT) {
    constexpr int cc = decltype(ccT)::value;
    sfor4([&](auto rT) { constexpr int i = 4 * cc + decltype(rT)::value; g = fma_half_lane<i>(A[i], f, g, h1); });
  });
  {
    const vr cost = hsum32(sel(act, f * (bb + real(0.5) * (g - bb + Rr * f)), vr(real(0))));
    const VB worse = cost > vr(real(0));
    f = sel(worse, vr(real(0)), f);
    g = sel(worse, bb, g);
  }
  const vr hA = real(0.5) * ARjj;
  V<int> itp = V<int>(0), itn = V<int>(0);
  {
    VB run = VB(true);
    for (int iter = 0; iter < (nosweep ? 0 : M.pgs_iters); iter++) {
      vr k0, k1, nf;
      pgs_row_prepare(Rr, f, ARinv, k0, k1, nf);
      k0 = sel(run, k0, vr(real(0))); k1 = sel(run, k1, vr(real(0))); nf = sel(run, nf, vr(real(0)));
      vr gcap = g;
      uint64_t rowm = mask_shl(0x0000000100000001ull, 0);
      for_contacts<0, kMaxCon2>(nmax, [&](auto ccT) {
        constexpr int cc = decltype(ccT)::value;
        sfor4([&](auto rT) {
          constexpr int i = 4 * cc + decltype(rT)::value;
          gcap = sel_mask(rowm, g, gcap);
          rowm = mask_shl(rowm, 1);
          const vr dl = pgs_row_delta(g, k0, k1, nf);
          g = fma_half_lane<i>(A[i], dl, g, h1);
        });
      });
      const vr dcap = pgs_row_delta(gcap, k0, k1, nf);
      const vr ccap = pgs_row_cost(dcap, hA, gcap, Rr, f);
      f = f + dcap;
      itp = itp + sel(run, V<int>(1), V<int>(0));
      run = run & !((-hsum32(ccap)) * M.pgs_scale < vr(M.pgs_tol));
      if (!wany(run)) break;
    }
  }
  nm_stamp(6);
  {
    const V<int> lv = opaque_lane() & 31;
    const VB even = (lv & 1) == 0;
    vr Amq = vr(real(0));
    for_contacts<0, kMaxCon2>(nmax, [&](auto ccT) {
      constexpr int cc = decltype(ccT)::value;
      Amq = sel(lv == 4 * cc, A[4 * cc + 1], Amq);
      Amq = sel(lv == 4 * cc + 2, A[4 * cc + 3], Amq);
    });
    Amq = sel(even, Amq, shfl_xor1(Amq));
    const vr K1 = Ajj + shfl_xor1(Ajj) - Amq - Amq;
    const VB small = K1 < vr(real(1e-15));
    const vr invK1 = vrcp(K1), hK1 = real(0.5) * K1;
    for_contacts<0, kMaxCon2>(nmax, [&](auto ccT) {
      constexpr int cc = decltype(ccT)::value;
      A[4 * cc] = A[4 * cc] - A[4 * cc + 1];
      A[4 * cc + 2] = A[4 * cc + 2] - A[4 * cc + 3];
    });
    VB run = VB(true);
    const bool anysmall = wany(small & act);
    for (int iter = 0; iter < (nosweep ? 0 : M.noslip_iters); iter++) {
      vr improvement = vr(real(0));
      if (iter == 0) improvement = hsum32(sel(act, real(0.5) * f * f * Rr, vr(real(0))));
      vr lo, hi;
      noslip_pair_prepare<real>(f, shfl_xor1(f), small, lo, hi);
      lo = sel(run, lo, vr(real(0))); hi = sel(run, hi, vr(real(0)));
      vr dcap = vr(real(0)), dgcap = vr(real(0));
      uint64_t pairm = mask_shl(0x0000000300000003ull, 0);
      auto pair_sweep = [&](auto checkT) {
        sfor_pairs<kMaxRow2 / 2>(nmax, [&](auto pT) {
          constexpr int p = decltype(pT)::value;
          const vr dg = g - shfl_xor1(g);
          vr d = noslip_pair_delta(dg, invK1, lo, hi);
          if constexpr (decltype(checkT)::value) d = sel(noslip_pair_bad<real>(noslip_pair_cost(d, hK1, dg)), vr(real(0)), d);
          g = fma_half_lane<2 * p>(A[2 * p], d, g, h1);
          dcap = sel_mask(pairm, d, dcap);
          dgcap = sel_mask(pairm, dg, dgcap);
          pairm = mask_shl(pairm, 2);
        });
      };
      if (anysmall) pair_sweep(std::true_type{}); else pair_sweep(std::false_type{});
      f = f + dcap;
      improvement = improvement - hsum32(sel(even, noslip_pair_cost(dcap, hK1, dgcap), vr(real(0))));
      itn = itn + sel(run, V<int>(1), V<int>(0));
      run = run & !(improvement * M.pgs_scale < vr(M.noslip_tol));
      if (!wany(run)) break;
    }
  }
  nm_stamp(7);
  stsv(ibw, hoi + NM_IOFS(it_pgs), itp, VB(true));
  stsv(ibw, hoi + NM_IOFS(it_noslip), itn, VB(true));
  stsv(rbw, ho + (hl + NM_OFS(efc_f)), f, VB(true));
  stsv(rbw, ho + (hl + (kMaxRow2 + NM_OFS(efc_f))), vr(real(0)), VB(true));
  vr nf = vr(real(0));
  VB hit = VB(false);
  if (last) {
    nf = f + shfl_xor1(f);
    nf = nf + shfl_xor2(nf);
    vr ft[3], fr, sv3[3], Rt[9];
#pragma unroll
    for (int j = 0; j < 3; j++) sv3[j] = ldsv(M.footc, Lc * 4 + j);
    fr = ldsv(M.footc, Lc * 4 + 3);
#pragma unroll
    for (int j = 0; j < 9; j++) Rt[j] = SHR(colR, (Lc + 1) * 9 + j);
    matvec3(ft, Rt, sv3);
#pragma unroll
    for (int j = 0; j < 3; j++) ft[j] = ft[j] + SHR(colp, (Lc + 1) * 3 + j);
    vr dif[3] = {cp[0] - ft[0], cp[1] - ft[1], cp[2] - ft[2]};
    vr b2 = real(-1) * (nrm[0] * dif[0] + nrm[1] * dif[1] + nrm[2] * dif[2]);
    vr cq = dif[0] * dif[0] + dif[1] * dif[1] + dif[2] * dif[2] - fr * fr;
    vr det = b2 * b2 - cq;
    vr sq = vsqrt(vmax(det, vr(real(0))));
    hit = !(det < vr(real(1e-15))) & (((-b2 - sq) >= vr(real(0))) | ((-b2 + sq) >= vr(real(0))));
  }
#pragma unroll
  for (int j = 0; j < 6; j++) stsv(rbw, ho + (j + NM_OFS(qfc)), hsum32(Jb[j] * f), VB(true));
  {
    vr s3[3];
#pragma unroll
    for (int k = 0; k < 3; k++) {
      vr x = Jl[k] * f;
      x = x + shfl_xor1(x);
      s3[k] = x + shfl_xor2(x);
    }
    const vr tn = sel(act & (nf > vr(real(0))), nf, vr(real(0))), tf = sel(hit, tn, vr(real(0)));
    const VB lead = act & ((hl & 3) == 0);
    wave_sync();
#pragma unroll
    for (int k = 0; k < 3; k++) stsu(jrow, jh + (c * 8 + k), s3[k], lead, w.e[0].sink);
    if (last) { stsu(jrow, jh + (c * 8 + 3), tn, lead, w.e[0].sink); stsu(jrow, jh + (c * 8 + 4), tf, lead, w.e[0].sink); }
    wave_sync();
    const VB on = hl < 30;
    const V<int> lg = sel(on, (hl * 13) >> 6, V<int>(0)), qq = hl - lg * 5;
    const V<int> c0 = SHI(cstart, lg + 1), cn = SHI(ccnt, lg + 1);
    vr acc = vr(real(0));
#pragma unroll
    for (int k = 0; k < 4; k++) {
      VB in = on & (cn > k);
      acc = acc + sel(in, ldsv(jrow, jh + sel(in, (c0 + k) * 8 + qq, V<int>(0))), vr(real(0)));
    }
    stsu(rbw, ho + (lg * 3 + qq + (6 + NM_OFS(qfc))), acc, on & (qq < 3), w.e[0].sink);
    if (last) {
      stsu(rbw, ho + (lg + NM_OFS(sens)), acc, on & (qq == 3), w.e[0].sink);
      stsu(rbw, ho + (lg + (6 + NM_OFS(sens))), acc, on & (qq == 4), w.e[0].sink);
      stsv(rbw, ho + V<int>(12 + NM_OFS(sens)), hsum32(sel(act & ((hl & 3) == 0) & (L < 0), tn, vr(real(0)))), VB(true));
    }
  }
  wave_sync();
#undef SHR
#undef SHI
}

template <class real> struct BigRows {
  V<real> Jb[kBigSlots][6], Jl[kBigSlots][3], Jm[kBigSlots][3], Rr[kBigSlots], bb[kBigSlots], f[kBigSlots], ARinv[kBigSlots], hA[kBigSlots];
  V<real> invK1[kBigSlots], hK1[kBigSlots];
  V<int> L[kBigSlots], L1[kBigSlots];
  VB act[kBigSlots], small[kBigSlots];
};
template <class real> NM_FN void big_minv(Sh<real>& sh, const real* yb, const V<real>* yl, bool accumulate) {
  typedef V<real> vr;
  const V<int> lane = opaque_lane();
  const VB isleg = lane < kNLEG;
  const V<int> leg = vmin(lane, V<int>(kNLEG - 1));
  vr t[3], Mi[6], xb[6];
#pragma unroll
  for (int j = 0; j < 6; j++) Mi[j] = ldsv(sh.Minv, leg * 6 + j);
  ldl3_solve(t, Mi, yl);
#pragma unroll
  for (int j = 0; j < 6; j++) {
    vr wy = ldsv(sh.W, leg * 18 + j) * yl[0] + ldsv(sh.W, leg * 18 + (6 + j)) * yl[1] + ldsv(sh.W, leg * 18 + (12 + j)) * yl[2];
    xb[j] = vr(yb[j] - lanesum6<real>(sel(isleg, wy, vr(real(0)))));
  }
  {
    vr Lf[15], Di[6];
#pragma unroll
    for (int j = 0; j < 15; j++) Lf[j] = vr(sh.Lb[j]);
#pragma unroll
    for (int j = 0; j < 6; j++) Di[j] = vr(sh.Dbi[j]);
    ldl6_solve(Lf, Di, xb);
  }
  vr x[3];
#pragma unroll
  for (int k = 0; k < 3; k++) {
    x[k] = t[k];
#pragma unroll
    for (int j = 0; j < 6; j++) x[k] = x[k] - ldsv(sh.W, leg * 18 + (6 * k + j)) * xb[j];
  }
  wave_sync();
#pragma unroll
  for (int j = 0; j < 6; j++) {
    vr nv = accumulate ? ldsv(sh.vv, V<int>(j)) + xb[j] : xb[j];
    stsv(sh.vv, V<int>(j), nv, lane == 0);
  }
#pragma unroll
  for (int k = 0; k < 3; k++) {
    vr nv = accumulate ? ldsv(sh.vv, leg * 3 + (6 + k)) + x[k] : x[k];
    stsv(sh.vv, leg * 3 + (6 + k), nv, isleg);
  }
  wave_sync();
}
template <class real> NM_FN void big_update_v(Sh<real>& sh, const real* jb, const real* jl, const real* jm, int Li, int L1i) {
  typedef V<real> vr;
  const V<int> leg = vmin(opaque_lane(), V<int>(kNLEG - 1));
  vr yl[3];
#pragma unroll
  for (int k = 0; k < 3; k++) yl[k] = sel(leg == Li, vr(jl[k]), vr(real(0))) + sel(leg == L1i, vr(jm[k]), vr(real(0)));
  big_minv(sh, jb, yl, true);
}
template <class real> NM_FN V<real> big_residual(const Sh<real>& sh, const BigRows<real>& r, int k) {
  V<real> g = r.bb[k];
  const V<int> Lc = vmax(r.L[k], V<int>(0)), Lc1 = vmax(r.L1[k], V<int>(0));
#pragma unroll
  for (int j = 0; j < 6; j++) g += r.Jb[k][j] * sh.vv[j];
#pragma unroll
  for (int j = 0; j < 3; j++) g += r.Jl[k][j] * ldsv(sh.vv, Lc * 3 + (6 + j)) + r.Jm[k][j] * ldsv(sh.vv, Lc1 * 3 + (6 + j));
  return g;
}
template <class real> NM_FN void big_jtf(Sh<real>& sh, const BigRows<real>& r) {
  typedef V<real> vr;
#pragma unroll
  for (int j = 0; j < 6; j++) {
    vr a = vr(real(0));
#pragma unroll
    for (int k = 0; k < kBigSlots; k++) a += r.Jb[k][j] * r.f[k];
    sh.qfc[j] = wsum<real>(a);
  }
  for (int l = 0; l < kNLEG; l++)
#pragma unroll
    for (int j = 0; j < 3; j++) {
      vr a = vr(real(0));
#pragma unroll
      for (int k = 0; k < kBigSlots; k++)
        a += sel(r.L[k] == l, r.Jl[k][j] * r.f[k], vr(real(0))) + sel(r.L1[k] == l, r.Jm[k][j] * r.f[k], vr(real(0)));
      sh.qfc[6 + 3 * l + j] = wsum<real>(a);
    }
  wave_sync();
}
template <class real> NM_COLD void stage_constraint_big(Sh<real>& sh, const Model<real>& M, bool last, bool nosweep) {
  typedef V<real> vr;
  const V<int> lane = opaque_lane();
  const int ncon = uniform(sh.ncon), nefc = 4 * ncon;
  BigRows<real> r;
  const V<int> q4 = lane & 3;
  const vr smu = sel((lane & 1) == 0, vr(M.mu), vr(-M.mu));
  const VB even = (lane & 1) == 0;
#pragma unroll
  for (int k = 0; k < kBigSlots; k++) {
    const V<int> row = lane + NM_WAVE * k;
    const VB act = row < nefc;
    const V<int> c = sel(act, row >> 2, V<int>(0));
    vr cp[3] = {ldsv(sh.cpos(), c * 3), ldsv(sh.cpos(), c * 3 + 1), ldsv(sh.cpos(), c * 3 + 2)};
    vr nrm[3] = {ldsv(sh.cnrm(), c * 3), ldsv(sh.cnrm(), c * 3 + 1), ldsv(sh.cnrm(), c * 3 + 2)};
    const vr dist = ldsv(sh.cdist(), c);
    const V<int> L = sel(act, ldsv(sh.cleg(), c), V<int>(-1)), L1 = sel(act, ldsv(sh.cleg1(), c), V<int>(-1));
    const VB onleg = L >= 0, onleg1 = L1 >= 0;
    const V<int> Lc = vmax(L, V<int>(0)), Lc1 = vmax(L1, V<int>(0));
    vr e[3];
    {
      VB usey = (nrm[1] < vr(real(0.5))) & (nrm[1] > vr(real(-0.5)));
      vr y0[3] = {vr(real(0)), sel(usey, vr(real(1)), vr(real(0))), sel(usey, vr(real(0)), vr(real(1)))};
      vr dt = nrm[1] * y0[1] + nrm[2] * y0[2];
      vr t1[3] = {y0[0] - dt * nrm[0], y0[1] - dt * nrm[1], y0[2] - dt * nrm[2]}, t2[3];
      vr il = vr(real(1)) / vsqrt(t1[0] * t1[0] + t1[1] * t1[1] + t1[2] * t1[2]);
      t1[0] = t1[0] * il; t1[1] = t1[1] * il; t1[2] = t1[2] * il;
      cross3(t2, nrm, t1);
#pragma unroll
      for (int j = 0; j < 3; j++) e[j] = sel(q4 == 1, t1[j], sel(q4 == 2, t2[j], nrm[j]));
    }
    vr Fb[6], Fl[3], Fm[3];
    {
      vr m[3];
      cross3(m, cp, e);
      Fb[0] = e[0]; Fb[1] = e[1]; Fb[2] = e[2];
#pragma unroll
      for (int j = 0; j < 3; j++) Fb[3 + j] = sh.Rb[j] * m[0] + sh.Rb[3 + j] * m[1] + sh.Rb[6 + j] * m[2];
#pragma unroll
      for (int kk = 0; kk < 3; kk++) {
        vr a[3], rel[3], mm[3], a1[3], rel1[3], mm1[3];
#pragma unroll
        for (int j = 0; j < 3; j++) {
          a[j] = ldsv(sh.axs, Lc * 9 + (3 * kk + j));
          rel[j] = cp[j] - ldsv(sh.anc, Lc * 9 + (3 * kk + j));
          a1[j] = ldsv(sh.axs, Lc1 * 9 + (3 * kk + j));
          rel1[j] = cp[j] - ldsv(sh.anc, Lc1 * 9 + (3 * kk + j));
        }
        cross3(mm, rel, e);
        cross3(mm1, rel1, e);
        Fl[kk] = sel(onleg & act, dot3<vr>(a, mm), vr(real(0)));
        Fm[kk] = sel(onleg1 & act, -dot3<vr>(a1, mm1), vr(real(0)));
      }
#pragma unroll
      for (int j = 0; j < 6; j++) Fb[j] = sel(act & !onleg1, Fb[j], vr(real(0)));
    }
    vr uF[6];
#pragma unroll
    for (int j = 0; j < 6; j++) {
      uF[j] = Fb[j];
#pragma unroll
      for (int kk = 0; kk < 3; kk++) uF[j] = uF[j] - ldsv(sh.W, Lc * 18 + (6 * kk + j)) * Fl[kk] - ldsv(sh.W, Lc1 * 18 + (6 * kk + j)) * Fm[kk];
    }
    vr u[6];
#pragma unroll
    for (int j = 0; j < 6; j++) {
      r.Jb[k][j] = quad<0x00>(Fb[j]) + smu * quad<0xA5>(Fb[j]);
      u[j] = quad<0x00>(uF[j]) + smu * quad<0xA5>(uF[j]);
    }
#pragma unroll
    for (int j = 0; j < 3; j++) {
      r.Jl[k][j] = quad<0x00>(Fl[j]) + smu * quad<0xA5>(Fl[j]);
      r.Jm[k][j] = quad<0x00>(Fm[j]) + smu * quad<0xA5>(Fm[j]);
    }
    vr imp;
    {
      vr x = vabs(dist) * vrcp(M.si_width);
      vr ylo, yhi;
      if (M.si_power == real(2)) {
        vr omx = vmax(vr(real(1)) - x, vr(real(0)));
        ylo = (x * x) * vrcp(M.si_mid);
        yhi = vr(real(1)) - (omx * omx) * vrcp(real(1) - M.si_mid);
      } else {
        ylo = vpow(x, vr(M.si_power)) / vpow(vr(M.si_mid), vr(M.si_power - real(1)));
        yhi = vr(real(1)) - vpow(vmax(vr(real(1)) - x, vr(real(0))), vr(M.si_power)) / vpow(vr(real(1) - M.si_mid), vr(M.si_power - real(1)));
      }
      vr y = sel(x <= vr(M.si_mid), ylo, yhi);
      imp = M.si_d0 + y * (M.si_dmax - M.si_d0);
      imp = sel(x >= vr(real(1)), vr(M.si_dmax), imp);
      imp = sel(x <= vr(real(0)), vr(M.si_d0), imp);
    }
    vr invw = ldsv(M.colc, (Lc + sel(onleg, V<int>(1), V<int>(0))) * kColN + 4);
    invw = invw + sel(onleg1, ldsv(M.colc, (Lc1 + 1) * kColN + 4), vr(real(0)));
    const vr Rr = vmax((vr(real(1)) - imp) * (invw + M.mu * M.mu * invw) * vrcp(imp), vr(real(1e-15))) * (real(2) * M.mu * M.mu);
    vr vel = vr(real(0)), jas = vr(real(0)), jaw = vr(real(0));
#pragma unroll
    for (int j = 0; j < 6; j++) {
      vel += r.Jb[k][j] * sh.qvel[j]; jas += r.Jb[k][j] * sh.qas[j]; jaw += r.Jb[k][j] * sh.warm[j];
    }
#pragma unroll
    for (int j = 0; j < 3; j++) {
      V<int> di = Lc * 3 + (6 + j), di1 = Lc1 * 3 + (6 + j);
      vel += r.Jl[k][j] * ldsv(sh.qvel, di) + r.Jm[k][j] * ldsv(sh.qvel, di1);
      jas += r.Jl[k][j] * ldsv(sh.qas, di) + r.Jm[k][j] * ldsv(sh.qas, di1);
      jaw += r.Jl[k][j] * ldsv(sh.warm, di) + r.Jm[k][j] * ldsv(sh.warm, di1);
    }
    const vr aref = -M.solref_B * vel - M.solref_K * imp * dist;
    vr t[3], t1m[3], xb[6];
    {
      vr Mi[6], Mi1[6];
#pragma unroll
      for (int j = 0; j < 6; j++) { Mi[j] = ldsv(sh.Minv, Lc * 6 + j); Mi1[j] = ldsv(sh.Minv, Lc1 * 6 + j); }
      ldl3_solve(t, Mi, r.Jl[k]);
      ldl3_solve(t1m, Mi1, r.Jm[k]);
#pragma unroll
      for (int j = 0; j < 6; j++) xb[j] = u[j];
      ldl6_solve(sh.Lb, sh.Dbi, xb);
    }
    vr Ajj = r.Jl[k][0] * t[0] + r.Jl[k][1] * t[1] + r.Jl[k][2] * t[2] + (r.Jm[k][0] * t1m[0] + r.Jm[k][1] * t1m[1] + r.Jm[k][2] * t1m[2]);
    vr Apq = r.Jl[k][0] * shfl_xor1(t[0]) + r.Jl[k][1] * shfl_xor1(t[1]) + r.Jl[k][2] * shfl_xor1(t[2]) +
             (r.Jm[k][0] * shfl_xor1(t1m[0]) + r.Jm[k][1] * shfl_xor1(t1m[1]) + r.Jm[k][2] * shfl_xor1(t1m[2]));
#pragma unroll
    for (int j = 0; j < 6; j++) { Ajj += u[j] * xb[j]; Apq += u[j] * shfl_xor1(xb[j]); }
    Apq = sel(even, Apq, shfl_xor1(Apq));
    const vr K1 = Ajj + shfl_xor1(Ajj) - Apq - Apq;
    r.small[k] = K1 < vr(real(1e-15));
    r.invK1[k] = vrcp(K1);
    r.hK1[k] = real(0.5) * K1;
    const vr ARjj = Ajj + Rr;
    r.ARinv[k] = sel(act, vrcp(ARjj), vr(real(0)));
    r.hA[k] = real(0.5) * ARjj;
    r.Rr[k] = Rr;
    r.bb[k] = jas - aref;
    r.L[k] = L; r.L1[k] = L1; r.act[k] = act;
    const vr jar = jaw - aref;
    r.f[k] = sel(act & (jar < vr(real(0))), -vrcp(Rr) * jar, vr(real(0)));
  }
  {
    big_jtf(sh, r);
    const V<int> leg = vmin(lane, V<int>(kNLEG - 1));
    vr yl[3] = {ldsv(sh.qfc, leg * 3 + 6), ldsv(sh.qfc, leg * 3 + 7), ldsv(sh.qfc, leg * 3 + 8)};
    real yb[6];
#pragma unroll
    for (int j = 0; j < 6; j++) yb[j] = sh.qfc[j];
    big_minv(sh, yb, yl, false);
    vr cterm = vr(real(0));
#pragma unroll
    for (int k = 0; k < kBigSlots; k++) {
      const vr g = big_residual(sh, r, k);
      cterm += sel(r.act[k], r.f[k] * (r.bb[k] + real(0.5) * (g - r.bb[k] + r.Rr[k] * r.f[k])), vr(real(0)));
    }
    if (wsum<real>(cterm) > real(0)) {
#pragma unroll
      for (int k = 0; k < kBigSlots; k++) r.f[k] = vr(real(0));
      wave_sync();
      stsv(sh.vv, sel(lane < 24, lane, V<int>(0)), real(0), lane < 24);
      wave_sync();
    }
  }
  for (int iter = 0; iter < (nosweep ? 0 : M.pgs_iters); iter++) {
    real improvement = real(0);
#pragma unroll
    for (int k = 0; k < kBigSlots; k++) {
      for (int ln = 0; ln < NM_WAVE; ln++) {
        if (NM_WAVE * k + ln >= nefc) break;
        vr k0, k1, nf;
        pgs_row_prepare(r.Rr[k], r.f[k], r.ARinv[k], k0, k1, nf);
        const vr gk = big_residual(sh, r, k);
        const vr dl = pgs_row_delta(gk, k0, k1, nf);
        const vr change = pgs_row_cost(dl, r.hA[k], gk, r.Rr[k], r.f[k]);
        const real d = rdlane(dl, ln);
        improvement -= rdlane(change, ln);
        r.f[k] = sel(lane == ln, r.f[k] + dl, r.f[k]);
        real jb[6], jl[3], jm[3];
#pragma unroll
        for (int j = 0; j < 6; j++) jb[j] = rdlane(r.Jb[k][j], ln) * d;
#pragma unroll
        for (int j = 0; j < 3; j++) { jl[j] = rdlane(r.Jl[k][j], ln) * d; jm[j] = rdlane(r.Jm[k][j], ln) * d; }
        big_update_v(sh, jb, jl, jm, rdlane(r.L[k], ln), rdlane(r.L1[k], ln));
      }
    }
    sh.it_pgs = iter + 1;
    if (improvement * M.pgs_scale < M.pgs_tol) break;
  }
  for (int iter = 0; iter < (nosweep ? 0 : M.noslip_iters); iter++) {
    real improvement = real(0);
    if (iter == 0) {
      vr a = vr(real(0));
#pragma unroll
      for (int k = 0; k < kBigSlots; k++) a += sel(r.act[k], real(0.5) * r.f[k] * r.f[k] * r.Rr[k], vr(real(0)));
      improvement = wsum<real>(a);
    }
#pragma unroll
    for (int k = 0; k < kBigSlots; k++) {
      for (int pp = 0; pp < NM_WAVE / 2; pp++) {
        if (NM_WAVE * k + 2 * pp >= nefc) break;
        const vr g = big_residual(sh, r, k);
        vr lo, hi;
        noslip_pair_prepare<real>(r.f[k], shfl_xor1(r.f[k]), r.small[k], lo, hi);
        const vr dg = g - shfl_xor1(g);
        vr d = noslip_pair_delta(dg, r.invK1[k], lo, hi);
        const vr change = noslip_pair_cost(d, r.hK1[k], dg);
        const VB bad = noslip_pair_bad<real>(change);
        d = sel(bad, vr(real(0)), d);
        const real d0 = rdlane(d, 2 * pp), d1 = rdlane(d, 2 * pp + 1);
        improvement -= rdlane(sel(bad, vr(real(0)), change), 2 * pp);
        r.f[k] = sel((lane >> 1) == pp, r.f[k] + d, r.f[k]);
        real jb[6], jl[3], jm[3];
#pragma unroll
        for (int j = 0; j < 6; j++) jb[j] = rdlane(r.Jb[k][j], 2 * pp) * d0 + rdlane(r.Jb[k][j], 2 * pp + 1) * d1;
#pragma unroll
        for (int j = 0; j < 3; j++) {
          jl[j] = rdlane(r.Jl[k][j], 2 * pp) * d0 + rdlane(r.Jl[k][j], 2 * pp + 1) * d1;
          jm[j] = rdlane(r.Jm[k][j], 2 * pp) * d0 + rdlane(r.Jm[k][j], 2 * pp + 1) * d1;
        }
        big_update_v(sh, jb, jl, jm, rdlane(r.L[k], 2 * pp), rdlane(r.L1[k], 2 * pp));
      }
    }
    sh.it_noslip = iter + 1;
    if (improvement * M.pgs_scale < M.noslip_tol) break;
  }
  big_jtf(sh, r);
  stsv(sh.efc_f, lane, r.f[0], lane < kMaxRow);
  if (last) {
    vr s_all[kNLEG], s_foot[kNLEG], s_base = vr(real(0));
#pragma unroll
    for (int l = 0; l < kNLEG; l++) { s_all[l] = vr(real(0)); s_foot[l] = vr(real(0)); }
#pragma unroll
    for (int k = 0; k < kBigSlots; k++) {
      const V<int> row = lane + NM_WAVE * k;
      const V<int> c = sel(r.act[k], row >> 2, V<int>(0));
      vr cp[3] = {ldsv(sh.cpos(), c * 3), ldsv(sh.cpos(), c * 3 + 1), ldsv(sh.cpos(), c * 3 + 2)};
      vr nrm[3] = {ldsv(sh.cnrm(), c * 3), ldsv(sh.cnrm(), c * 3 + 1), ldsv(sh.cnrm(), c * 3 + 2)};
      vr nf = r.f[k] + shfl_xor1(r.f[k]);
      nf = nf + shfl_xor2(nf);
      auto foot_hit = [&](const V<int>& Lx, real sgn) {
        vr ft[3], fr, sp[3], Rt[9];
#pragma unroll
        for (int j = 0; j < 3; j++) sp[j] = ldsv(M.footc, Lx * 4 + j);
        fr = ldsv(M.footc, Lx * 4 + 3);
#pragma unroll
        for (int j = 0; j < 9; j++) Rt[j] = ldsv(sh.colR, (Lx + 1) * 9 + j);
        matvec3(ft, Rt, sp);
#pragma unroll
        for (int j = 0; j < 3; j++) ft[j] = ft[j] + ldsv(sh.colp, (Lx + 1) * 3 + j);
        vr dif[3] = {cp[0] - ft[0], cp[1] - ft[1], cp[2] - ft[2]};
        vr b2 = sgn * (nrm[0] * dif[0] + nrm[1] * dif[1] + nrm[2] * dif[2]);
        vr cc = dif[0] * dif[0] + dif[1] * dif[1] + dif[2] * dif[2] - fr * fr;
        vr det = b2 * b2 - cc;
        vr sq = vsqrt(vmax(det, vr(real(0))));
        return !(det < vr(real(1e-15))) & (((-b2 - sq) >= vr(real(0))) | ((-b2 + sq) >= vr(real(0))));
      };
      const VB hit = foot_hit(vmax(r.L[k], V<int>(0)), real(-1)), hit1 = foot_hit(vmax(r.L1[k], V<int>(0)), real(1));
      const VB head = r.act[k] & ((lane & 3) == 0) & (nf > vr(real(0)));
#pragma unroll
      for (int l = 0; l < kNLEG; l++) {
        s_all[l] += sel(head & ((r.L[k] == l) | (r.L1[k] == l)), nf, vr(real(0)));
        s_foot[l] += sel(head & (((r.L[k] == l) & hit) | ((r.L1[k] == l) & hit1)), nf, vr(real(0)));
      }
      s_base += sel(head & (r.L[k] < 0), nf, vr(real(0)));
    }
#pragma unroll
    for (int l = 0; l < kNLEG; l++) { sh.sens[l] = wsum<real>(s_all[l]); sh.sens[6 + l] = wsum<real>(s_foot[l]); }
    sh.sens[12] = wsum<real>(s_base);
  }
  wave_sync();
}
template <class real> NM_COLD void floor_frames(Sh<real>& sh) {
  const V<int> lane = lane_id();
  const int nfloor = uniform(sh.cstart[7]);
  const VB on = lane < nfloor;
  const V<int> c = sel(on, lane, V<int>(0));
  stsv(sh.cleg1(), c, V<int>(-1), on);
  stsv(sh.cnrm(), c * 3, V<real>(real(0)), on);
  stsv(sh.cnrm(), c * 3 + 1, V<real>(real(0)), on);
  stsv(sh.cnrm(), c * 3 + 2, V<real>(real(1)), on);
  wave_sync();
}
template <class real> NM_FN void stage_constraint(Sh<real>& sh, real* jrow, const Model<real>& M, bool last, bool nosweep = false) {
  if (uniform(sh.ncon) > kMaxCon) { floor_frames(sh); stage_constraint_big<real>(sh, M, last, nosweep); }
  else if (uniform(sh.anypair) != 0) { floor_frames(sh); stage_constraint_pairs<real>(sh, jrow, M, last, nosweep); }
  else stage_constraint_body<real, false>(sh, jrow, M, last, nosweep);
}

template <class real, int G> NM_FN void stage_integrate(ShW<real, G>& w, const Model<real>& M) {
  typedef V<real> vr;
  real* lds = reinterpret_cast<real*>(&w.e[0]);
  const V<int> lane0 = opaque_lane();
  const V<int> sub = lane0 & 7, grp = lane0 >> 3;
  const V<int> leg = vmin(sub, V<int>(5)), eo = (grp & (G - 1)) * (int)(sizeof(Sh<real>) / sizeof(real));
  const VB pass1 = (grp & G) != 0;
  const VB isleg = sub < V<int>(6);
#define LDG(field, i) ldsv(lds, eo + (NM_OFS(field) + (i)))
#define LDL(field, idx) ldsv(lds, eo + (idx) + NM_OFS(field))
  constexpr int kFacH = NM_OFS(MinvH) - NM_OFS(Minv);
  static_assert(NM_OFS(WH) - NM_OFS(W) == kFacH && NM_OFS(LbH) - NM_OFS(Lb) == kFacH && NM_OFS(DbiH) - NM_OFS(Dbi) == kFacH, "factor blocks");
  static_assert(sizeof(Sh<real>::mbb) / sizeof(real) >= 24 && sizeof(Sh<real>::sc) / sizeof(real) >= 28 && sizeof(Sh<real>::vv) / sizeof(real) >= 24, "junk rows");
  const V<int> eoF = eo + sel(pass1, V<int>(kFacH), V<int>(0));
  vr xl[3], xb[6];
  {
    vr y[3], t[3], Mi[6];
#pragma unroll
    for (int k = 0; k < 3; k++) y[k] = LDL(qfc, leg * 3 + (6 + k)) + sel(pass1, LDL(qfs, leg * 3 + (6 + k)), vr(real(0)));
#pragma unroll
    for (int j = 0; j < 6; j++) Mi[j] = ldsv(lds, eoF + leg * 6 + (NM_OFS(Minv) + j));
    ldl3_solve(t, Mi, y);
#pragma unroll
    for (int j = 0; j < 6; j++) {
      vr wy = ldsv(lds, eoF + leg * 18 + (NM_OFS(W) + j)) * y[0] + ldsv(lds, eoF + leg * 18 + (NM_OFS(W) + 6 + j)) * y[1] +
              ldsv(lds, eoF + leg * 18 + (NM_OFS(W) + 12 + j)) * y[2];
      xb[j] = LDG(qfc, j) - legsum<real>(wy, isleg) + sel(pass1, LDG(qfs, j), vr(real(0)));
    }
    {
      vr L[15], Di[6];
#pragma unroll
      for (int j = 0; j < 15; j++) L[j] = ldsv(lds, eoF + (NM_OFS(Lb) + j));
#pragma unroll
      for (int j = 0; j < 6; j++) Di[j] = ldsv(lds, eoF + (NM_OFS(Dbi) + j));
      ldl6_solve(L, Di, xb);
    }
#pragma unroll
    for (int k = 0; k < 3; k++) {
      vr x = t[k];
#pragma unroll
      for (int j = 0; j < 6; j++) x = x - ldsv(lds, eoF + leg * 18 + (NM_OFS(W) + 6 * k + j)) * xb[j];
      xl[k] = x;
    }
  }
  vr qacc_l[3], qacc_b[6];
#pragma unroll
  for (int k = 0; k < 3; k++) qacc_l[k] = xl[k] + LDL(qas, leg * 3 + (6 + k));
#pragma unroll
  for (int j = 0; j < 6; j++) qacc_b[j] = xb[j] + LDG(qas, j);
  const vr* qint_l = xl; const vr* qint_b = xb;
  VB badl = (visbad(qacc_l[0]) | visbad(qacc_l[1]) | visbad(qacc_l[2])) & isleg;
#pragma unroll
  for (int j = 0; j < 6; j++) badl = badl | visbad(qacc_b[j]);
  const VB gbad = gsum8(sel(badl, V<int>(1), V<int>(0))) > 0;
  const VB okl = VB(true), okb = VB(true);
  wave_sync();
  vr nv[6];
#pragma unroll
  for (int j = 0; j < 6; j++) nv[j] = LDG(qvel, j) + M.h * qint_b[j];
  vr np_[3], nq[4];
#pragma unroll
  for (int j = 0; j < 3; j++) np_[j] = LDG(qpos, j) + M.h * nv[j];
  {
    vr n = vsqrt(nv[3] * nv[3] + nv[4] * nv[4] + nv[5] * nv[5]);
    VB rot = !(n < vr(real(1e-15)));
    vr ns = sel(rot, n, vr(real(1)));
    vr ang = M.h * n, sn, cs;
    vsincos(real(0.5) * ang, &sn, &cs);
    rot = rot & (ang != vr(real(0)));
    const vr isn = vrcp(ns) * sn;
    vr qr[4] = {sel(rot, cs, vr(real(1))), sel(rot, nv[3] * isn, vr(real(0))), sel(rot, nv[4] * isn, vr(real(0))),
                sel(rot, nv[5] * isn, vr(real(0)))};
    vr a[4] = {LDG(qpos, 3), LDG(qpos, 4), LDG(qpos, 5), LDG(qpos, 6)};
    vr t[4] = {a[0] * qr[0] - a[1] * qr[1] - a[2] * qr[2] - a[3] * qr[3], a[0] * qr[1] + a[1] * qr[0] + a[2] * qr[3] - a[3] * qr[2],
               a[0] * qr[2] - a[1] * qr[3] + a[2] * qr[0] + a[3] * qr[1], a[0] * qr[3] + a[1] * qr[2] - a[2] * qr[1] + a[3] * qr[0]};
    vr nn = vsqrt(t[0] * t[0] + t[1] * t[1] + t[2] * t[2] + t[3] * t[3]);
#pragma unroll
    for (int j = 0; j < 4; j++) nq[j] = t[j] * vrcp(nn);
  }
  vr jq[3], jv[3];
#pragma unroll
  for (int k = 0; k < 3; k++) {
    jv[k] = LDL(qvel, leg * 3 + (6 + k)) + M.h * qint_l[k];
    jq[k] = LDL(qpos, leg * 3 + (7 + k)) + M.h * jv[k];
  }
  wave_sync();
  const V<int> eoV = eo + sel(pass1, V<int>(NM_OFS(qvel)), V<int>(NM_OFS(mbb)));
  const V<int> eoP = eo + sel(pass1, V<int>(NM_OFS(qpos)), V<int>(NM_OFS(sc)));
  const V<int> eoW = eo + sel(pass1, V<int>(NM_OFS(vv)), V<int>(NM_OFS(warm)));
#pragma unroll
  for (int j = 0; j < 6; j++) {
    stsv(lds, eoV + j, nv[j], okb);
    stsv(lds, eoW + j, qacc_b[j], okb);
  }
#pragma unroll
  for (int j = 0; j < 3; j++) stsv(lds, eoP + j, np_[j], okb);
#pragma unroll
  for (int j = 0; j < 4; j++) stsv(lds, eoP + (3 + j), nq[j], okb);
#pragma unroll
  for (int k = 0; k < 3; k++) {
    stsv(lds, eoV + leg * 3 + (6 + k), jv[k], okl);
    stsv(lds, eoP + leg * 3 + (7 + k), jq[k], okl);
    stsv(lds, eoW + leg * 3 + (6 + k), qacc_l[k], okl);
  }
  wave_sync();
  for (int e = 0; e < G; e++) {
    if (rdlane(sel(gbad, V<int>(1), V<int>(0)), 8 * e) != 0) {
      Sh<real>& sh = w.e[e];
      const V<int> lane = opaque_lane();
      sh.nwarn += 1;
      vr q0 = ldsv(M.qpos0, sel(lane < kNQ, lane, V<int>(0)));
      real vz = -M.grav * M.h;
      q0 = sel(lane == 2, q0 + vz * M.h, q0);
      stsv(sh.qpos, lane, q0, lane < kNQ);
      stsv(sh.qvel, lane, sel(lane == 2, vr(vz), vr(real(0))), lane < kNV);
      stsv(sh.warm, lane, sel(lane == 2, vr(-M.grav), vr(real(0))), lane < kNV);
      stsv(sh.ctrl, lane, real(0), lane < kNU);
      wave_sync();
    }
  }
#undef LDG
#undef LDL
}

template <class real> NM_FN void reset_data(Sh<real>& sh, const Model<real>& M) {
  const V<int> lane = opaque_lane();
  stsv(sh.qpos, lane, ldsv(M.qpos0, sel(lane < kNQ, lane, V<int>(0))), lane < kNQ);
  stsv(sh.qvel, lane, real(0), lane < kNV);
  stsv(sh.warm, lane, real(0), lane < kNV);
  stsv(sh.ctrl, lane, real(0), lane < kNU);
  wave_sync();
}

#ifndef NM_PRIO
#define NM_PRIO 3
#endif
#if !defined(NM_EMUL)
NM_FN void nm_set_priority(int load) {
  if (load >= NM_PRIO + 4) __builtin_amdgcn_s_setprio(3);
  else if (load >= NM_PRIO + 2) __builtin_amdgcn_s_setprio(2);
  else if (load >= NM_PRIO) __builtin_amdgcn_s_setprio(1);
  else __builtin_amdgcn_s_setprio(0);
}
#else
inline void nm_set_priority(int) {}
#endif

template <class real, int G> NM_FN void substep(ShW<real, G>& w, const Model<real>& M, bool last, int* dropped, int ablate) {
  const V<int> lane = opaque_lane();
  if constexpr (G == 2) {
    constexpr int kSR = (int)(sizeof(Sh<real>) / sizeof(real));
    real* rbw = reinterpret_cast<real*>(&w.e[0]);
    const V<int> hl = lane & 31, ho = (lane >> 5) * kSR;
    {
      const VB bad = (visbad(ldsv(rbw, ho + (sel(hl < kNQ, hl, V<int>(0)) + NM_OFS(qpos)))) & (hl < kNQ)) |
                     (visbad(ldsv(rbw, ho + (sel(hl < kNV, hl, V<int>(0)) + NM_OFS(qvel)))) & (hl < kNV));
      const uint64_t bm = ballot(bad);
      if (bm) {
#pragma unroll
        for (int e = 0; e < 2; e++)
          if ((bm >> (32 * e)) & 0xffffffffull) { w.e[e].nwarn += 1; reset_data(w.e[e], M); }
      }
    }
  } else {
    for (int e = 0; e < G; e++) {
      Sh<real>& sh = w.e[e];
      {
        VB bad = (visbad(ldsv(sh.qpos, sel(lane < kNQ, lane, V<int>(0)))) & (lane < kNQ)) |
                 (visbad(ldsv(sh.qvel, sel(lane < kNV, lane, V<int>(0)))) & (lane < kNV));
        if (wany(bad)) { sh.nwarn += 1; reset_data(sh, M); }
      }
    }
  }
  wave_sync();
  nm_stamp(1);
  if (!(ablate & 8)) stage_smooth(w, M, last);
  nm_stamp(2);
  for (int e = 0; e < G; e++) {
    Sh<real>& sh = w.e[e];
    if (!(ablate & 1)) { Rings<real> rg; collide_rings(sh, M, rg); stage_collide(sh, M, dropped, rg, G != 2 && !(ablate & 16)); }
    else { sh.ncon = 0; sh.anypair = 0; wave_sync(); }
  }
  if constexpr (G == 2) {
    if (!(ablate & 1) && !(ablate & 16)) stage_collide_pairs2(w, M, dropped);
  }
  for (int e = 0; e < G; e++)
    if (ablate & 4) { w.e[e].ncon = 0; w.e[e].anypair = 0; wave_sync(); }
  bool together = false;
  if constexpr (G == 2) {
    const int n0 = uniform(w.e[0].ncon), n1 = uniform(w.e[1].ncon);
    nm_set_priority(n0 + n1);
    together = n0 + n1 >= 1 && n0 <= kMaxCon2 && n1 <= kMaxCon2 && uniform(w.e[0].anypair) == 0 && uniform(w.e[1].anypair) == 0 && !(ablate & 32);
    if (!last) w.e[1].ntog = n0 * 64 + n1;
    if (together) {
#ifdef NM_EMUL
      nm_emul_together() += 1;
#endif
      w.e[0].ntog += 1;
      stage_constraint2(w, M, last, (ablate & 2) != 0);
      nm_stamp(8);
    }
  }
  if (!together)
    for (int e = 0; e < G; e++) {
      stage_constraint(w.e[e], w.jrow, M, last, (ablate & 2) != 0);
      nm_stamp(8);
    }
  stage_integrate(w, M);
  nm_stamp(9);
}


template <class real> NM_FN void env_load(Sh<real>& sh, const Model<real>& M, const Args<real>& A, int env) {
  typedef V<real> vr;
  const V<int> lane = opaque_lane();
  const VB l18 = lane < kNU;
  const V<int> l18c = sel(l18, lane, V<int>(0));
  const vr q_in = gldv(A.qpos, sel(lane < kNQ, lane, V<int>(0)) + env * kNQ);
  const vr v_in = gldv(A.qvel, sel(lane < kNV, lane, V<int>(0)) + env * kNV);
  const vr w_in = gldv(A.qwarm, sel(lane < kNV, lane, V<int>(0)) + env * kNV);
  const V<int> hc_in = gldv(A.hullcache, sel(lane < 8, lane, V<int>(0)) + env * 8);
  const V<float> a_in = gldv(A.actions, l18c + env * kNU);
  vr cmd_in = vr(real(0)), eps_in = vr(real(0)), prev_act = vr(real(0)), prev_dofvel = vr(real(0)), dofpos_old = vr(real(0));
  int64_t ep = 0;
  uint32_t ctr_in = 0;
  if (!A.physics_only) {
    cmd_in = gldv(A.cmd, sel(lane < 3, lane, V<int>(0)) + env * 3);
    eps_in = gldv(A.epsum, sel(lane < kNREW, lane, V<int>(0)) + env * kNREW);
    ep = gld1(A.eplen, env);
    ctr_in = gld1(A.rngctr, env);
    prev_act = gldv(A.act, l18c + env * kNU);
    prev_dofvel = gldv(A.dofvel, l18c + env * kNU);
    dofpos_old = gldv(A.dofpos, l18c + env * kNU);
  }
  stsv(sh.qpos, lane, q_in, lane < kNQ);
  stsv(sh.qvel, lane, v_in, lane < kNV);
  stsv(sh.warm, lane, w_in, lane < kNV);
  stsv(sh.hcache, lane, sel(lane == 0, hc_in & V<int>(0xffff), hc_in), lane < 8);
  sh.nwarn = 0;
  sh.nhop = 0;
  sh.ntog = 0;
  V<float> af = a_in * M.action_scale;
  af = vmin(vmax(af, V<float>(-M.clip_actions)), V<float>(M.clip_actions));
  vr act;
  vr defp;
  {
    V<int> m3 = lane % 3;
    defp = sel(m3 == 1, vr(M.default_pos[1]), sel(m3 == 0, vr(M.default_pos[0]), vr(M.default_pos[2])));
  }
#ifdef NM_EMUL
  for (int i = 0; i < NM_WAVE; i++) act.v[i] = (real)af.v[i];
#else
  act = (real)af;
#endif
  if (!A.physics_only) {
    stsv(sh.ecmd, lane, cmd_in, lane < 3);
    stsv(sh.eepsum, lane, eps_in, lane < kNREW);
    sh.eplen_lo = (int)(uint32_t)(ep & 0xffffffffll);
    sh.eplen_hi = (int)(ep >> 32);
    sh.ectr = ctr_in;
    stsv(sh.ctrl, lane, ((act - defp) - dofpos_old) * M.p_gain, l18);
  } else {
    wave_sync();
    stsv(sh.ctrl, lane, ((act - defp) - ldsv(sh.qpos, l18c + 7)) * M.p_gain, l18);
  }
  stsv(sh.eact, lane, act, l18); stsv(sh.epact, lane, prev_act, l18); stsv(sh.epdv, lane, prev_dofvel, l18);
  wave_sync();
}

template <class real> NM_FN void env_debug(Sh<real>& sh, const Args<real>& A, int env, int dropped) {
  const V<int> lane = opaque_lane();
  {
    real* dbg = A.dbg + (size_t)env * kDbgN;
    gstv(dbg, lane, ldsv(sh.qas, sel(lane < 24, lane, V<int>(0))), lane < 24);
    gstv(dbg, lane + 24, ldsv(sh.qfs, sel(lane < 24, lane, V<int>(0))), lane < 24);
    gstv(dbg, lane + 48, ldsv(sh.qfc, sel(lane < 24, lane, V<int>(0))), lane < 24);
    gstv(dbg, lane + 72, ldsv(sh.sens, sel(lane < 13, lane, V<int>(0))), lane < 13);
    gstv(dbg, lane + 88, ldsv(sh.cvb, sel(lane < 6, lane, V<int>(0))), lane < 6);
    gstv(dbg, lane + 96, ldsv(sh.cdist(), sel(lane < kMaxCon, lane, V<int>(0))), lane < kMaxCon);
    gstv(dbg, lane + 112, ldsv(sh.cpos(), sel(lane < 3 * kMaxCon, lane, V<int>(0))), lane < 3 * kMaxCon);
    gstv(dbg, V<int>(160), to_real<real>(sh.ncon), lane == 0);
    gstv(dbg, V<int>(161), to_real<real>(sh.nwarn), lane == 0);
    gstv(dbg, V<int>(162), to_real<real>(dropped), lane == 0);
    gstv(dbg, lane + 165, ldsv(sh.cnrm(), sel(lane < 6, lane, V<int>(0))), lane < 6);
    gstv(dbg, lane + 150, to_real<real>(ldsv(sh.hcache, sel(lane < 7, lane, V<int>(0)))), lane < 7);
    gstv(dbg, V<int>(158), to_real<real>(sh.hcache[7]), lane == 0);
    gstv(dbg, V<int>(159), to_real<real>(sh.nhop), lane == 0);
    gstv(dbg, V<int>(157), to_real<real>(sh.anypair), lane == 0);
    gstv(dbg, V<int>(156), to_real<real>(sh.ntog), lane == 0);
    gstv(dbg, V<int>(163), to_real<real>(sh.it_pgs), lane == 0);
    gstv(dbg, V<int>(164), to_real<real>(sh.it_noslip), lane == 0);
    gstv(dbg, lane + 176, ldsv(sh.efc_f, lane), lane < kMaxRow);
#ifdef NM_DEBUG_SOLVER
    gstv(dbg, lane + 240, ldsv(sh.dbg_b, sel(lane < 4, lane, V<int>(0))), lane < 4);
    gstv(dbg, lane + 244, ldsv(sh.dbg_a, sel(lane < 4, lane, V<int>(0))), lane < 4);
    gstv(dbg, lane + 248, ldsv(sh.dbg_f0, sel(lane < 4, lane, V<int>(0))), lane < 4);
#endif
  }
}

template <class real> NM_FN void env_finish(Sh<real>& sh, const Model<real>& M, const Args<real>& A, int env,
                                            int dropped, bool live) {
  typedef V<real> vr;
  if (!live) return;
  const V<int> lane = opaque_lane();
  const VB l18 = lane < kNU;
  const V<int> l18c = sel(l18, lane, V<int>(0));
  const vr act = ldsv(sh.eact, l18c), prev_act = ldsv(sh.epact, l18c), prev_dofvel = ldsv(sh.epdv, l18c);
  vr defp;
  {
    V<int> m3 = lane % 3;
    defp = sel(m3 == 1, vr(M.default_pos[1]), sel(m3 == 0, vr(M.default_pos[0]), vr(M.default_pos[2])));
  }
  {
    const V<int> hc = ldsv(sh.hcache, sel(lane < 8, lane, V<int>(0)));
    const vr q = ldsv(sh.qpos, sel(lane < kNQ, lane, V<int>(0))), v = ldsv(sh.qvel, sel(lane < kNV, lane, V<int>(0))),
             w = ldsv(sh.warm, sel(lane < kNV, lane, V<int>(0)));
    gstv(A.hullcache, lane + env * 8, hc, lane < 8);
    gstv(A.qpos, lane + env * kNQ, q, lane < kNQ);
    gstv(A.qvel, lane + env * kNV, v, lane < kNV);
    gstv(A.qwarm, lane + env * kNV, w, lane < kNV);
  }
  if (A.rec && env == A.rec_env) {
    gstv(A.rec, lane, ldsv(sh.qpos, sel(lane < kNQ, lane, V<int>(0))), lane < kNQ);
    gstv(A.rec, lane + kNQ, ldsv(sh.qvel, sel(lane < kNV, lane, V<int>(0))), lane < kNV);
    gstv(A.rec, V<int>(kNQ + kNV), to_real<real>(sh.nwarn), lane == 0);
  }
  if (A.dbg) env_debug(sh, A, env, dropped);
  if ((dropped | sh.nwarn) && A.stat_cnt) {
#ifdef NM_EMUL
    A.stat_cnt[1] += dropped; A.stat_cnt[2] += sh.nwarn;
#else
    if (NM_TID == 0) { nm_consume(atomicAdd(A.stat_cnt + 1, dropped)); nm_consume(atomicAdd(A.stat_cnt + 2, sh.nwarn)); }
#endif
  }
  if (A.physics_only) return;
  NM_ESTAMP(11);

  int64_t eplen = (((int64_t)sh.eplen_hi << 32) | (int64_t)(uint32_t)sh.eplen_lo) + 1;
  real bq[4] = {sh.qpos[3], -sh.qpos[4], -sh.qpos[5], -sh.qpos[6]};
  auto rot = [&](real* r, const real* v) {
    real tx = real(2) * (bq[2] * v[2] - bq[3] * v[1]), ty = real(2) * (bq[3] * v[0] - bq[1] * v[2]), tz = real(2) * (bq[1] * v[1] - bq[2] * v[0]);
    r[0] = v[0] + bq[0] * tx + (bq[2] * tz - bq[3] * ty);
    r[1] = v[1] + bq[0] * ty + (bq[3] * tx - bq[1] * tz);
// ... 598 lines not shown
```

### nightmare_rl_amd/csrc/simt.h

```cpp
#pragma once
#include <stdint.h>

#define NM_WAVE 64

#ifndef NM_EMUL
#include <hip/hip_runtime.h>
#define NM_FN __device__ __forceinline__
#define NM_COLD __device__ __noinline__
namespace simt {
template <class T> using V = T;
using VB = bool;

#ifdef NM_WG_WAVES
#define NM_TID ((int)(threadIdx.x & 63))
#else
#define NM_TID ((int)threadIdx.x)
#endif
NM_FN int lane_id() { return NM_TID; }
template <class T> NM_FN T sel(bool c, T a, T b) { return c ? a : b; }
NM_FN float vsqrt(float x) { return sqrtf(x); }
NM_FN double vsqrt(double x) { return sqrt(x); }
NM_FN float vabs(float x) { return fabsf(x); }
NM_FN double vabs(double x) { return fabs(x); }
NM_FN float vmax(float a, float b) { return fmaxf(a, b); }
NM_FN double vmax(double a, double b) { return fmax(a, b); }
NM_FN float vmin(float a, float b) { return fminf(a, b); }
NM_FN double vmin(double a, double b) { return fmin(a, b); }
NM_FN int vmin(int a, int b) { return a < b ? a : b; }
NM_FN int vmax(int a, int b) { return a > b ? a : b; }
NM_FN void vsincos(float x0, float* s, float* c) {
  const float x = fminf(fmaxf(x0, -4194304.0f), 4194304.0f);
  const float k = rintf(x * 0.636619772f);
  float r = fmaf(-k, 1.5707963705062866f, x);
  r = fmaf(-k, -4.371139000186241e-8f, r);
  const float r2 = r * r;
  const float ps = fmaf(r * r2, fmaf(r2, fmaf(r2, -1.9515295891e-4f, 8.3321608736e-3f), -1.6666654611e-1f), r);
  const float pc = fmaf(r2 * r2, fmaf(r2, fmaf(r2, 2.443315711809948e-5f, -1.388731625493765e-3f), 4.166664568298827e-2f), fmaf(r2, -0.5f, 1.0f));
  const int n = (int)k;
  const float sa = (n & 1) ? pc : ps, ca = (n & 1) ? ps : pc;
  *s = (n & 2) ? -sa : sa;
  *c = ((n + 1) & 2) ? -ca : ca;
}
NM_FN void vsincos(double x, double* s, double* c) { sincos(x, s, c); }
NM_FN float vexp(float x) { return expf(x); }
NM_FN double vexp(double x) { return exp(x); }
NM_FN float vacos(float x) { return acosf(x); }
NM_FN double vacos(double x) { return acos(x); }
NM_FN float vpow(float x, float p) { return powf(x, p); }
NM_FN double vpow(double x, double p) { return pow(x, p); }
NM_FN bool visbad(float x) { return !(fabsf(x) <= 1e10f); }
NM_FN bool visbad(double x) { return !(fabs(x) <= 1e10); }
template <class T> NM_FN T to_real(int i) { return (T)i; }
template <class T, class S> NM_FN T vcvt(S x) { return (T)x; }
NM_FN float vrcp(float x) { return __builtin_amdgcn_rcpf(x); }
NM_FN double vrcp(double x) { return 1.0 / x; }

NM_FN float vfma(float a, float b, float c) { return __builtin_fmaf(a, b, c); }
NM_FN double vfma(double a, double b, double c) { return __builtin_fma(a, b, c); }
NM_FN float sel_mask(uint64_t m, float a, float b) {
  float r;
  asm("v_cndmask_b32_e64 %0, %1, %2, %3" : "=v"(r) : "v"(b), "v"(a), "s"(m));
  return r;
}
NM_FN double sel_mask(uint64_t m, double a, double b) {
  int rl, rh;
  asm("v_cndmask_b32_e64 %0, %2, %3, %6\n\tv_cndmask_b32_e64 %1, %4, %5, %6" : "=&v"(rl), "=v"(rh)
      : "v"(__double2loint(b)), "v"(__double2loint(a)), "v"(__double2hiint(b)), "v"(__double2hiint(a)), "s"(m));
  return __hiloint2double(rh, rl);
}
NM_FN uint64_t mask_shl(uint64_t m, int k) { m <<= k; asm("" : "+s"(m)); return m; }
template <int I> NM_FN float fma_half_lane(float a, float x, float g, bool h1);
template <int I> NM_FN double fma_half_lane(double a, double x, double g, bool h1);
NM_FN int rdlane(int x, int l) { return __builtin_amdgcn_readlane(x, l); }
NM_FN float rdlane(float x, int l) { return __int_as_float(__builtin_amdgcn_readlane(__float_as_int(x), l)); }
NM_FN double rdlane(double x, int l) {
  int lo = __builtin_amdgcn_readlane(__double2loint(x), l), hi = __builtin_amdgcn_readlane(__double2hiint(x), l);
  return __hiloint2double(hi, lo);
}
template <int I> NM_FN float fma_half_lane(float a, float x, float g, bool h1) {
  const float s0 = rdlane(x, I), s1 = rdlane(x, 32 + I);
  return vfma(a, h1 ? s1 : s0, g);
}
template <int I> NM_FN double fma_half_lane(double a, double x, double g, bool h1) {
  const double s0 = rdlane(x, I), s1 = rdlane(x, 32 + I);
  return vfma(a, h1 ? s1 : s0, g);
}
template <class T> NM_FN T wrlane(T x, T v, int l) {
  int ln = NM_TID;
  asm volatile("" : "+v"(ln));
  return ln == l ? v : x;
}
NM_FN int opaque_lane() { int ln = NM_TID; asm volatile("" : "+v"(ln)); return ln; }
template <class T> NM_FN T uniform(T x) { return rdlane(x, 0); }
NM_FN bool uniform(bool x) { return __builtin_amdgcn_readfirstlane((int)x) != 0; }
#define NM_DPP_QUAD_XOR1 0xB1
#define NM_DPP_QUAD_XOR2 0x4E
#define NM_DPP_HALF_MIRROR 0x141
#define NM_DPP_ROW_MIRROR 0x140
template <int CTRL> NM_FN int dpp(int x) { return __builtin_amdgcn_mov_dpp(x, CTRL, 0xF, 0xF, true); }
template <int CTRL> NM_FN float dpp(float x) { return __int_as_float(dpp<CTRL>(__float_as_int(x))); }
template <int CTRL> NM_FN double dpp(double x) { return __hiloint2double(dpp<CTRL>(__double2hiint(x)), dpp<CTRL>(__double2loint(x))); }
template <int P, class T> NM_FN T quad(T x) { return dpp<P>(x); }
template <class T> NM_FN T shfl_xor1(T x) { return dpp<NM_DPP_QUAD_XOR1>(x); }
template <class T> NM_FN T shfl_xor2(T x) { return dpp<NM_DPP_QUAD_XOR2>(x); }
template <class T> NM_FN T wsum8(T x) {
  x = x + dpp<NM_DPP_QUAD_XOR1>(x);
  x = x + dpp<NM_DPP_QUAD_XOR2>(x);
  x = x + dpp<NM_DPP_HALF_MIRROR>(x);
  return rdlane(x, 0);
}
template <class T> NM_FN T gsum8(T x) {
  x = x + dpp<NM_DPP_QUAD_XOR1>(x);
  x = x + dpp<NM_DPP_QUAD_XOR2>(x);
  x = x + dpp<NM_DPP_HALF_MIRROR>(x);
  return x;
}
template <class T> NM_FN T wsum(T x) {
  x = x + dpp<NM_DPP_QUAD_XOR1>(x);
  x = x + dpp<NM_DPP_QUAD_XOR2>(x);
  x = x + dpp<NM_DPP_HALF_MIRROR>(x);
  x = x + dpp<NM_DPP_ROW_MIRROR>(x);
  return (rdlane(x, 0) + rdlane(x, 16)) + (rdlane(x, 32) + rdlane(x, 48));
}
template <class T> NM_FN T hsum32(T x) {
  x = x + dpp<NM_DPP_QUAD_XOR1>(x);
  x = x + dpp<NM_DPP_QUAD_XOR2>(x);
  x = x + dpp<NM_DPP_HALF_MIRROR>(x);
  x = x + dpp<NM_DPP_ROW_MIRROR>(x);
  const T s0 = rdlane(x, 0) + rdlane(x, 16), s1 = rdlane(x, 32) + rdlane(x, 48);
  return (NM_TID & 32) ? s1 : s0;
}
NM_FN bool wany(bool c) { return __ballot(c) != 0ull; }
NM_FN int lane_rank(uint64_t m) { return (int)__builtin_amdgcn_mbcnt_hi((uint32_t)(m >> 32), __builtin_amdgcn_mbcnt_lo((uint32_t)m, 0u)); }
NM_FN int popc64(uint64_t m) { return __popcll(m); }
NM_FN uint64_t ballot(bool c) { return __ballot(c); }
NM_FN bool in_mask(uint64_t m) { return __builtin_amdgcn_inverse_ballot_w64(m); }
template <class T> NM_FN void order_after(int& a, const T& dep) { asm volatile("" : "+v"(a) : "v"(dep)); }
template <class T> NM_FN void wargmax(T val, int idx, T* best, int* ibest) {
#define NM_AM_STEP(CTRL)                                                   \
  {                                                                        \
    T ov = dpp<CTRL>(val);                                                 \
    int oi = dpp<CTRL>(idx);                                               \
    bool take = (ov > val) | ((ov == val) & (oi < idx));                   \
    val = take ? ov : val;                                                 \
    idx = take ? oi : idx;                                                 \
  }
  NM_AM_STEP(NM_DPP_QUAD_XOR1) NM_AM_STEP(NM_DPP_QUAD_XOR2) NM_AM_STEP(NM_DPP_HALF_MIRROR) NM_AM_STEP(NM_DPP_ROW_MIRROR)
#undef NM_AM_STEP
  T bv = rdlane(val, 0);
  int bi = rdlane(idx, 0);
#pragma unroll
  for (int r = 16; r < 64; r += 16) {
    T ov = rdlane(val, r);
    int oi = rdlane(idx, r);
    bool take = (ov > bv) | ((ov == bv) & (oi < bi));
    bv = take ? ov : bv;
    bi = take ? oi : bi;
  }
  *best = bv;
  *ibest = bi;
}
template <class T> NM_FN void wmaxfirst(T val, T* best, int* lane_of_best) {
  T m = val;
  m = vmax(m, dpp<NM_DPP_QUAD_XOR1>(m));
  m = vmax(m, dpp<NM_DPP_QUAD_XOR2>(m));
  m = vmax(m, dpp<NM_DPP_HALF_MIRROR>(m));
  m = vmax(m, dpp<NM_DPP_ROW_MIRROR>(m));
  const T b = vmax(vmax(rdlane(m, 0), rdlane(m, 16)), vmax(rdlane(m, 32), rdlane(m, 48)));
  *best = b;
  *lane_of_best = (int)__builtin_ctzll(__ballot(val == b));
}
template <class T> NM_FN T ldsv(const T* a, int i) { return a[i]; }
template <class T> NM_FN void stsv(T* a, int i, T v, bool m) { if (m) a[i] = v; }
template <class T, class S> NM_FN void stsu(T* a, int i, T v, bool m, S* sink) {
  T* p = m ? a + i : reinterpret_cast<T*>(sink) + NM_TID;
  *p = v;
}
#define NM_GLOBAL(T) __attribute__((address_space(1))) T
typedef float nm_f4 __attribute__((ext_vector_type(4)));
typedef double nm_d4 __attribute__((ext_vector_type(4)));
template <class T> NM_FN T gldv(const T* p, int i) { return ((const NM_GLOBAL(T)*)p)[i]; }
template <class T> NM_FN void gstv(T* p, int i, T v, bool m) { if (m) ((NM_GLOBAL(T)*)p)[i] = v; }
template <class T> NM_FN T gld1(const T* p, size_t i) { return ((const NM_GLOBAL(T)*)p)[i]; }
template <class T> NM_FN void gst1(T* p, size_t i, T v) { ((NM_GLOBAL(T)*)p)[i] = v; }
NM_FN void gadd1(float* p, size_t i, float v) { __builtin_amdgcn_global_atomic_fadd_f32((NM_GLOBAL(float)*)p + i, v); }
NM_FN void gld3(const float* p, int i, float* o) { const nm_f4 t = *(const NM_GLOBAL(nm_f4)*)((const NM_GLOBAL(float)*)p + i); o[0] = t.x; o[1] = t.y; o[2] = t.z; }
NM_FN void gld3(const double* p, int i, double* o) { const nm_d4 t = *(const NM_GLOBAL(nm_d4)*)((const NM_GLOBAL(double)*)p + i); o[0] = t.x; o[1] = t.y; o[2] = t.z; }
NM_FN void gld4(const float* p, int i, float* o) { const nm_f4 t = *(const NM_GLOBAL(nm_f4)*)((const NM_GLOBAL(float)*)p + i); o[0] = t.x; o[1] = t.y; o[2] = t.z; o[3] = t.w; }
NM_FN void gld4(const double* p, int i, double* o) { const nm_d4 t = *(const NM_GLOBAL(nm_d4)*)((const NM_GLOBAL(double)*)p + i); o[0] = t.x; o[1] = t.y; o[2] = t.z; o[3] = t.w; }
NM_FN int to_int(float x) { return (int)x; }
NM_FN int to_int(double x) { return (int)x; }
NM_FN void wave_sync() {
  __builtin_amdgcn_fence(__ATOMIC_RELEASE, "wavefront");
  __builtin_amdgcn_wave_barrier();
  __builtin_amdgcn_fence(__ATOMIC_ACQUIRE, "wavefront");
}
NM_FN void sched_fence() { __builtin_amdgcn_sched_barrier(0); }
}

#else
#include <cmath>
#include <cstring>
#define NM_FN inline
#define NM_COLD inline
namespace simt {
template <class T> struct V {
  T v[NM_WAVE];
  V() {}
  V(T s) { for (int i = 0; i < NM_WAVE; i++) v[i] = s; }
#define NM_BIN(op)                                                                                   \
  friend V operator op(const V& a, const V& b) { V r; for (int i = 0; i < NM_WAVE; i++) r.v[i] = a.v[i] op b.v[i]; return r; }
  NM_BIN(+) NM_BIN(-) NM_BIN(*) NM_BIN(/) NM_BIN(%) NM_BIN(&) NM_BIN(|) NM_BIN(>>) NM_BIN(<<)
#undef NM_BIN
#define NM_CMP(op)                                                                                      \
  friend V<bool> operator op(const V& a, const V& b) { V<bool> r; for (int i = 0; i < NM_WAVE; i++) r.v[i] = a.v[i] op b.v[i]; return r; }
  NM_CMP(<) NM_CMP(>) NM_CMP(<=) NM_CMP(>=) NM_CMP(==) NM_CMP(!=)
#undef NM_CMP
  friend V operator-(const V& a) { V r; for (int i = 0; i < NM_WAVE; i++) r.v[i] = -a.v[i]; return r; }
  friend V operator!(const V& a) { V r; for (int i = 0; i < NM_WAVE; i++) r.v[i] = !a.v[i]; return r; }
  V& operator+=(const V& b) { for (int i = 0; i < NM_WAVE; i++) v[i] += b.v[i]; return *this; }
  V& operator-=(const V& b) { for (int i = 0; i < NM_WAVE; i++) v[i] -= b.v[i]; return *this; }
  V& operator*=(const V& b) { for (int i = 0; i < NM_WAVE; i++) v[i] *= b.v[i]; return *this; }
};
using VB = V<bool>;

NM_FN V<int> lane_id() { V<int> r; for (int i = 0; i < NM_WAVE; i++) r.v[i] = i; return r; }
#define NM_SEL(T)                                                                                              \
  NM_FN V<T> sel(const VB& c, const V<T>& a, const V<T>& b) { V<T> r; for (int i = 0; i < NM_WAVE; i++) r.v[i] = c.v[i] ? a.v[i] : b.v[i]; return r; } \
  NM_FN T sel(bool c, T a, T b) { return c ? a : b; }
NM_SEL(float) NM_SEL(double) NM_SEL(int)
#undef NM_SEL
#define NM_MAP1(name, expr)                                                                                   \
  NM_FN V<float> name(const V<float>& a) { V<float> r; for (int i = 0; i < NM_WAVE; i++) { float x = a.v[i]; r.v[i] = expr; } return r; } \
  NM_FN V<double> name(const V<double>& a) { V<double> r; for (int i = 0; i < NM_WAVE; i++) { double x = a.v[i]; r.v[i] = expr; } return r; } \
  NM_FN float name(float x) { return expr; }                                                                  \
  NM_FN double name(double x) { return expr; }
NM_MAP1(vsqrt, std::sqrt(x)) NM_MAP1(vabs, std::fabs(x)) NM_MAP1(vexp, std::exp(x)) NM_MAP1(vacos, std::acos(x))
#undef NM_MAP1
#define NM_MAP2(name, expr, T)                                                                               \
  NM_FN V<T> name(const V<T>& a, const V<T>& b) { V<T> r; for (int i = 0; i < NM_WAVE; i++) { T x = a.v[i], y = b.v[i]; r.v[i] = expr; } return r; } \
  NM_FN T name(T x, T y) { return expr; }
NM_MAP2(vmax, (x > y ? x : y), float) NM_MAP2(vmax, (x > y ? x : y), double) NM_MAP2(vmax, (x > y ? x : y), int)
NM_MAP2(vmin, (x < y ? x : y), float) NM_MAP2(vmin, (x < y ? x : y), double) NM_MAP2(vmin, (x < y ? x : y), int)
NM_MAP2(vpow, std::pow(x, y), float) NM_MAP2(vpow, std::pow(x, y), double)
#undef NM_MAP2
template <class T> NM_FN void vsincos(const V<T>& x, V<T>* s, V<T>* c) { for (int i = 0; i < NM_WAVE; i++) { s->v[i] = std::sin(x.v[i]); c->v[i] = std::cos(x.v[i]); } }
NM_FN void vsincos(float x, float* s, float* c) { *s = std::sin(x); *c = std::cos(x); }
NM_FN void vsincos(double x, double* s, double* c) { *s = std::sin(x); *c = std::cos(x); }
template <class T> NM_FN VB visbad(const V<T>& a) { VB r; for (int i = 0; i < NM_WAVE; i++) r.v[i] = !(std::fabs(a.v[i]) <= (T)1e10); return r; }
NM_FN bool visbad(float x) { return !(std::fabs(x) <= 1e10f); }
NM_FN bool visbad(double x) { return !(std::fabs(x) <= 1e10); }
template <class T> NM_FN V<T> to_real(const V<int>& a) { V<T> r; for (int i = 0; i < NM_WAVE; i++) r.v[i] = (T)a.v[i]; return r; }
template <class T> NM_FN T to_real(int a) { return (T)a; }
template <class T> NM_FN V<T> vrcp(const V<T>& a) { V<T> r; for (int i = 0; i < NM_WAVE; i++) r.v[i] = (T)1 / a.v[i]; return r; }
NM_FN float vrcp(float x) { return 1.0f / x; }
NM_FN double vrcp(double x) { return 1.0 / x; }
template <class T, class S> NM_FN V<T> vcvt(const V<S>& a) { V<T> r; for (int i = 0; i < NM_WAVE; i++) r.v[i] = (T)a.v[i]; return r; }

template <class T> NM_FN V<T> vfma(const V<T>& a, const V<T>& b, const V<T>& c) { return a * b + c; }
NM_FN float vfma(float a, float b, float c) { return a * b + c; }
NM_FN double vfma(double a, double b, double c) { return a * b + c; }
template <class T> NM_FN V<T> sel_mask(uint64_t m, const V<T>& a, const V<T>& b) {
  V<T> r;
  for (int i = 0; i < NM_WAVE; i++) r.v[i] = ((m >> i) & 1ull) ? a.v[i] : b.v[i];
  return r;
}
NM_FN uint64_t mask_shl(uint64_t m, int k) { return m << k; }
template <int I, class T> NM_FN V<T> fma_half_lane(const V<T>& a, const V<T>& x, const V<T>& g, const VB&) {
  V<T> r;
  for (int i = 0; i < NM_WAVE; i++) r.v[i] = a.v[i] * x.v[(i & 32) + I] + g.v[i];
  return r;
}
template <class T> NM_FN T rdlane(const V<T>& x, int l) { return x.v[l]; }
template <class T> NM_FN T rdlane(T x, int) { return x; }
template <class T> NM_FN V<T> wrlane(V<T> x, T v, int l) { x.v[l] = v; return x; }
NM_FN V<int> opaque_lane() { return lane_id(); }
template <class T> NM_FN T uniform(const V<T>& x) { return x.v[0]; }
template <class T> NM_FN T uniform(T x) { return x; }
template <class T> NM_FN V<T> shfl_xor(const V<T>& x, int m) { V<T> r; for (int i = 0; i < NM_WAVE; i++) r.v[i] = x.v[i ^ m]; return r; }
template <int P, class T> NM_FN V<T> quad(const V<T>& x) { V<T> r; for (int i = 0; i < NM_WAVE; i++) r.v[i] = x.v[(i & ~3) | ((P >> (2 * (i & 3))) & 3)]; return r; }
template <class T> NM_FN V<T> shfl_xor1(const V<T>& x) { return shfl_xor(x, 1); }
template <class T> NM_FN V<T> shfl_xor2(const V<T>& x) { return shfl_xor(x, 2); }
template <class T> NM_FN V<T> half_mirror(const V<T>& x) { V<T> r; for (int i = 0; i < NM_WAVE; i++) r.v[i] = x.v[(i & ~7) | (7 - (i & 7))]; return r; }
template <class T> NM_FN V<T> row_mirror(const V<T>& x) { V<T> r; for (int i = 0; i < NM_WAVE; i++) r.v[i] = x.v[(i & ~15) | (15 - (i & 15))]; return r; }
template <class T> NM_FN V<T> gsum8(V<T> x) {
  x = x + shfl_xor(x, 1); x = x + shfl_xor(x, 2); x = x + half_mirror(x);
  return x;
}
template <class T> NM_FN T wsum8(V<T> x) {
  x = x + shfl_xor(x, 1); x = x + shfl_xor(x, 2); x = x + half_mirror(x);
  return x.v[0];
}
template <class T> NM_FN T wsum(V<T> x) {
  x = x + shfl_xor(x, 1); x = x + shfl_xor(x, 2); x = x + half_mirror(x); x = x + row_mirror(x);
  return (x.v[0] + x.v[16]) + (x.v[32] + x.v[48]);
}
template <class T> NM_FN V<T> hsum32(V<T> x) {
  x = x + shfl_xor(x, 1); x = x + shfl_xor(x, 2); x = x + half_mirror(x); x = x + row_mirror(x);
  const T s0 = x.v[0] + x.v[16], s1 = x.v[32] + x.v[48];
  V<T> r; for (int i = 0; i < NM_WAVE; i++) r.v[i] = i < 32 ? s0 : s1;
  return r;
}
NM_FN bool wany(const VB& c) { for (int i = 0; i < NM_WAVE; i++) if (c.v[i]) return true; return false; }
NM_FN V<int> lane_rank(uint64_t m) { V<int> r; for (int i = 0; i < NM_WAVE; i++) r.v[i] = __builtin_popcountll(m & ((1ull << i) - 1ull)); return r; }
NM_FN int popc64(uint64_t m) { return __builtin_popcountll(m); }
NM_FN uint64_t ballot(const VB& c) { uint64_t m = 0; for (int i = 0; i < NM_WAVE; i++) if (c.v[i]) m |= 1ull << i; return m; }
NM_FN VB in_mask(uint64_t m) { VB r; for (int i = 0; i < NM_WAVE; i++) r.v[i] = (m >> i) & 1; return r; }
template <class T> NM_FN void order_after(V<int>&, const V<T>&) {}
template <class T> NM_FN void wargmax(V<T> val, V<int> idx, T* best, int* ibest) {
  T bv = val.v[0]; int bi = idx.v[0];
  for (int i = 1; i < NM_WAVE; i++)
    if (val.v[i] > bv || (val.v[i] == bv && idx.v[i] < bi)) { bv = val.v[i]; bi = idx.v[i]; }
  *best = bv; *ibest = bi;
}
template <class T> NM_FN void wmaxfirst(const V<T>& val, T* best, int* lane_of_best) {
  T bv = val.v[0]; int bi = 0;
  for (int i = 1; i < NM_WAVE; i++) if (val.v[i] > bv) { bv = val.v[i]; bi = i; }
  *best = bv; *lane_of_best = bi;
}
template <class T> NM_FN V<T> ldsv(const T* a, const V<int>& i) { V<T> r; for (int k = 0; k < NM_WAVE; k++) r.v[k] = a[i.v[k]]; return r; }
template <class T> NM_FN T ldsv(const T* a, int i) { return a[i]; }
template <class T> NM_FN void stsv(T* a, const V<int>& i, const V<T>& v, const VB& m) { for (int k = 0; k < NM_WAVE; k++) if (m.v[k]) a[i.v[k]] = v.v[k]; }
template <class T> NM_FN void stsv(T* a, const V<int>& i, T v, const VB& m) { for (int k = 0; k < NM_WAVE; k++) if (m.v[k]) a[i.v[k]] = v; }
template <class T, class S> NM_FN void stsu(T* a, const V<int>& i, const V<T>& v, const VB& m, S*) { stsv(a, i, v, m); }
template <class T, class S> NM_FN void stsu(T* a, const V<int>& i, T v, const VB& m, S*) { stsv(a, i, v, m); }
template <class T> NM_FN T gld1(const T* p, size_t i) { return p[i]; }
template <class T> NM_FN void gst1(T* p, size_t i, T v) { p[i] = v; }
NM_FN void gadd1(float* p, size_t i, float v) { p[i] += v; }
template <class T> NM_FN V<T> gldv(const T* p, const V<int>& i) { return ldsv(p, i); }
template <class T> NM_FN void gstv(T* p, const V<int>& i, const V<T>& v, const VB& m) { stsv(p, i, v, m); }
template <class T> NM_FN void gstv(T* p, const V<int>& i, T v, const VB& m) { stsv(p, i, v, m); }
template <class T> NM_FN void gld4(const T* p, const V<int>& i, V<T>* o) { for (int k = 0; k < NM_WAVE; k++) for (int c = 0; c < 4; c++) o[c].v[k] = p[i.v[k] + c]; }
template <class T> NM_FN V<int> to_int(const V<T>& a) { V<int> r; for (int i = 0; i < NM_WAVE; i++) r.v[i] = (int)a.v[i]; return r; }
template <class T> NM_FN void gld3(const T* p, const V<int>& i, V<T>* o) { for (int k = 0; k < NM_WAVE; k++) for (int c = 0; c < 3; c++) o[c].v[k] = p[i.v[k] + c]; }
template <class T> NM_FN void gld3(const T* p, int i, T* o) { o[0] = p[i]; o[1] = p[i + 1]; o[2] = p[i + 2]; }
NM_FN void wave_sync() {}
NM_FN void sched_fence() {}
}
#endif
```

Measured before the change: 84.02 million env-steps/s.

## Repack LDS joint, factor and link records for 2/4-wide vector loads

```diff
diff --git a/nightmare_rl_amd/csrc/nm_core.h b/nightmare_rl_amd/csrc/nm_core.h
--- a/nightmare_rl_amd/csrc/nm_core.h
+++ b/nightmare_rl_amd/csrc/nm_core.h
@@ -91,19 +91,32 @@
 constexpr uint64_t kNoiseKey = 0x4E4F495345ull;
 constexpr int kDbgN = 256;
 
-template <class real> struct Sh {
+#define NM_REC alignas(4 * sizeof(real))
+constexpr int kJntN = 8;
+constexpr int kFacN = 24;
+constexpr int kFacW = 0, kFacMinv = 18;
+constexpr int kLinkTmp = 24;
+constexpr int kLegTmp = 3 * kLinkTmp;
+constexpr int kRotTmp = 12;
+constexpr int kScRec = 12;
+template <class real> struct NM_REC Sh {
   real qpos[28], qvel[24], warm[24], ctrl[20];
   real Rb[9], wv[6];
-  real anc[kNU * 3], axs[kNU * 3];
+  NM_REC real jnt[kNU * kJntN];
   real colR[kNCOL * 9], colp[kNCOL * 3];
-  real Minv[kNLEG * 6], W[kNLEG * 18], Lb[15], Dbi[6];
-  real MinvH[kNLEG * 6], WH[kNLEG * 18], LbH[15], DbiH[6];
+  NM_REC real fac[kNLEG * kFacN];
+  NM_REC real Lb[16];
+  NM_REC real Dbi[8];
+  NM_REC real facH[kNLEG * kFacN];
+  NM_REC real LbH[16];
+  NM_REC real DbiH[8];
   real qas[24], qfs[24], qfc[24];
   real vv[24];
   real sens[16], cvb[6];
   real bh[2];
-  real mbb[36], sc[36];
-  real legtmp[kNLEG * 66];
+  NM_REC real mbb[36];
+  NM_REC real sc[36];
+  NM_REC real legtmp[kNLEG * kLegTmp];
   NM_FN real* cpos() { return legtmp; }
   NM_FN real* cnrm() { return legtmp + 3 * kMaxConBig; }
   NM_FN real* cdist() { return legtmp + 6 * kMaxConBig; }
@@ -125,7 +138,38 @@
   int hcache[8];
 };
 
-static_assert(kNLEG * 66 >= 9 * kMaxConBig, "contact list must fit the leg staging area");
+static_assert(kNLEG * kLegTmp >= 9 * kMaxConBig, "contact list must fit the leg staging area");
+static_assert(kNLEG * kLegTmp >= kNLEG * 3 * kRotTmp, "joint rotations must fit the leg staging area");
+template <class real> constexpr bool sh_records_aligned() {
+  constexpr size_t a = 4 * sizeof(real);
+  return sizeof(Sh<real>) % a == 0 && offsetof(Sh<real>, jnt) % a == 0 && offsetof(Sh<real>, fac) % a == 0 && offsetof(Sh<real>, Lb) % a == 0 &&
+         offsetof(Sh<real>, Dbi) % a == 0 && offsetof(Sh<real>, facH) % a == 0 && offsetof(Sh<real>, mbb) % a == 0 &&
+         offsetof(Sh<real>, sc) % a == 0 && offsetof(Sh<real>, legtmp) % a == 0 && kJntN % 4 == 0 && kFacN % 4 == 0 &&
+         kFacMinv % 2 == 0 && (kFacMinv + 2) % 4 == 0 && kLinkTmp % 4 == 0 && kRotTmp % 4 == 0 && kScRec % 4 == 0 &&
+         kScRec + kLinkTmp <= 36;
+}
+static_assert(sh_records_aligned<float>() && sh_records_aligned<double>(), "LDS records read as vectors must start at multiples of 4 words");
+template <class T, class I, class X> NM_FN void ld_jnt(const T* p, const I& rec, X* anc, X* ax) {
+  X t[4], u[4];
+  ldsv4(p, rec, t);
+  ldsv4(p, rec + 4, u);
+  anc[0] = t[0]; anc[1] = t[1]; anc[2] = t[2];
+  ax[0] = u[0]; ax[1] = u[1]; ax[2] = u[2];
+}
+template <class T, class I, class X> NM_FN void ld_facW(const T* p, const I& rec, X* W) {
+  ldsv4(p, rec + kFacW, W); ldsv4(p, rec + (kFacW + 4), W + 4); ldsv4(p, rec + (kFacW + 8), W + 8); ldsv4(p, rec + (kFacW + 12), W + 12);
+  ldsv2(p, rec + (kFacW + 16), W + 16);
+}
+template <class T, class I, class X> NM_FN void ld_facMinv(const T* p, const I& rec, X* Mi) {
+  ldsv2(p, rec + kFacMinv, Mi);
+  ldsv4(p, rec + (kFacMinv + 2), Mi + 2);
+}
+template <class T, class I, class X> NM_FN void ld_Lb(const T* p, const I& rec, X* L) {
+  X t[4];
+  ldsv4(p, rec, L); ldsv4(p, rec + 4, L + 4); ldsv4(p, rec + 8, L + 8); ldsv4(p, rec + 12, t);
+  L[12] = t[0]; L[13] = t[1]; L[14] = t[2];
+}
+template <class T, class I, class X> NM_FN void ld_Dbi(const T* p, const I& rec, X* D) { ldsv4(p, rec, D); ldsv2(p, rec + 4, D + 4); }
 template <class real, int G> struct ShW {
   Sh<real> e[G];
   alignas(16) real jrow[kMaxRow * kJRow];
@@ -292,8 +336,6 @@
 #define NM_ESTAMP(k) nm_stamp(k)
 #define NM_BSTAMP(k)
 #endif
-
-constexpr int kLinkTmp = 22;
 
 template <class real> NM_FN V<real> legsum(const V<real>& x, const VB& isleg) {
   return gsum8(sel(isleg, x, V<real>(real(0))));
@@ -313,7 +355,7 @@
 #define STG(field, i, val) stsv(lds, eo + (NM_OFS(field) + (i)), val, st_all)
 #define LDL(field, idx) ldsv(lds, eo + (idx) + NM_OFS(field))
 #define STL(field, idx, val) stsv(lds, eo + (idx) + NM_OFS(field), val, st_leg)
-  const V<int> slot = leg * (3 * kLinkTmp);
+  const V<int> slot = eo + (NM_OFS(legtmp) + leg * kLegTmp);
 
   vr Rb[9];
   {
@@ -360,8 +402,10 @@
     Rl[0] = co + oc * ax[0] * ax[0]; Rl[1] = oc * ax[0] * ax[1] - s_ * ax[2]; Rl[2] = oc * ax[0] * ax[2] + s_ * ax[1];
     Rl[3] = oc * ax[0] * ax[1] + s_ * ax[2]; Rl[4] = co + oc * ax[1] * ax[1]; Rl[5] = oc * ax[1] * ax[2] - s_ * ax[0];
     Rl[6] = oc * ax[0] * ax[2] - s_ * ax[1]; Rl[7] = oc * ax[1] * ax[2] + s_ * ax[0]; Rl[8] = co + oc * ax[2] * ax[2];
-#pragma unroll
-    for (int j = 0; j < 9; j++) STL(legtmp, leg * 27 + lk * 9 + j, Rl[j]);
+    const V<int> ro = eo + (NM_OFS(legtmp) + leg * (3 * kRotTmp)) + lk * kRotTmp;
+    stsv4(lds, ro, Rl, st_leg);
+    stsv4(lds, ro + 4, Rl + 4, st_leg);
+    stsv(lds, ro + 8, Rl[8], st_leg);
     wave_sync();
   }
 #endif
@@ -402,8 +446,12 @@
         matvec3(aw, R0, ax);
         vr Rl[9];
 #ifndef NM_NO_ROLE_ROT
-#pragma unroll
-        for (int j = 0; j < 9; j++) Rl[j] = LDL(legtmp, leg * 27 + (k * 9 + j));
+        {
+          const V<int> ro = eo + (NM_OFS(legtmp) + leg * (3 * kRotTmp)) + k * kRotTmp;
+          ldsv4(lds, ro, Rl);
+          ldsv4(lds, ro + 4, Rl + 4);
+          Rl[8] = ldsv(lds, ro + 8);
+        }
         (void)q;
 #else
         vr s, co;
@@ -415,10 +463,11 @@
 #endif
         matmul3(R, R0, Rl);
       }
-#pragma unroll
-      for (int j = 0; j < 3; j++) {
-        STL(anc, leg * 9 + (3 * k + j), pos[j]);
-        STL(axs, leg * 9 + (3 * k + j), aw[j]);
+      {
+        const V<int> jo = eo + NM_OFS(jnt) + (leg * 3 + k) * kJntN;
+        const vr r4[4] = {pos[0], pos[1], pos[2], pos[2]}, a4[4] = {aw[0], aw[1], aw[2], aw[2]};
+        stsv4(lds, jo, r4, st_leg);
+        stsv4(lds, jo + 4, a4, st_leg);
       }
       if (k == 2) {
 #pragma unroll
@@ -484,13 +533,17 @@
 #pragma unroll
         for (int j = 0; j < 6; j++) f[j] = f[j] + t6[j];
       }
-      const V<int> o = sel(isbase, V<int>(NM_OFS(sc) + 9 - NM_OFS(legtmp)), slot + mylink * kLinkTmp);
-#pragma unroll
-      for (int j = 0; j < 6; j++) STL(legtmp, o + j, cS[j]);
-#pragma unroll
-      for (int j = 0; j < 10; j++) STL(legtmp, o + (6 + j), I10[j]);
-#pragma unroll
-      for (int j = 0; j < 6; j++) STL(legtmp, o + (16 + j), f[j]);
+      const V<int> o = sel(isbase, eo + V<int>(NM_OFS(sc) + kScRec), slot + mylink * kLinkTmp);
+      vr rec[22];
+#pragma unroll
+      for (int j = 0; j < 6; j++) rec[j] = cS[j];
+#pragma unroll
+      for (int j = 0; j < 10; j++) rec[6 + j] = I10[j];
+#pragma unroll
+      for (int j = 0; j < 6; j++) rec[16 + j] = f[j];
+#pragma unroll
+      for (int j = 0; j < 20; j += 4) stsv4(lds, o + j, rec + j, st_leg);
+      stsv2(lds, o + 20, rec + 20, st_leg);
       if (last) {
 #pragma unroll
         for (int j = 0; j < 3; j++) stsv(lds, eo + mylink * 3 + (NM_OFS(sc) + j), legsum<real>(mcom[j], isleg), st_all);
@@ -508,13 +561,16 @@
   for (int k = 2; k >= 0; k--) {
     sched_fence();
     const V<int> o = slot + k * kLinkTmp;
-    vr S[6], F[6];
-#pragma unroll
-    for (int j = 0; j < 6; j++) S[j] = LDL(legtmp, o + j);
-#pragma unroll
-    for (int j = 0; j < 10; j++) Ic[j] += LDL(legtmp, o + (6 + j));
-#pragma unroll
-    for (int j = 0; j < 6; j++) fs[j] += LDL(legtmp, o + (16 + j));
+    vr S[6], F[6], rec[22];
+#pragma unroll
+    for (int j = 0; j < 20; j += 4) ldsv4(lds, o + j, rec + j);
+    ldsv2(lds, o + 20, rec + 20);
+#pragma unroll
+    for (int j = 0; j < 6; j++) S[j] = rec[j];
+#pragma unroll
+    for (int j = 0; j < 10; j++) Ic[j] += rec[6 + j];
+#pragma unroll
+    for (int j = 0; j < 6; j++) fs[j] += rec[16 + j];
     cl[k] = dot6<vr>(S, fs);
     inert_mul(F, Ic, S);
     Mlb[k][0] = F[3]; Mlb[k][1] = F[4]; Mlb[k][2] = F[5];
@@ -525,8 +581,8 @@
 #pragma unroll
     for (int jj = 0; jj < k; jj++) {
       vr Sj[6];
-#pragma unroll
-      for (int j = 0; j < 6; j++) Sj[j] = LDL(legtmp, slot + (jj * kLinkTmp + j));
+      ldsv4(lds, slot + jj * kLinkTmp, Sj);
+      ldsv2(lds, slot + (jj * kLinkTmp + 4), Sj + 4);
       Ml[(jj == 0) ? k : 4] = dot6<vr>(Sj, F);
     }
   }
@@ -534,8 +590,10 @@
   vr Icb[10], cbias[6];
   {
     vr Ib10[10];
-#pragma unroll
-    for (int j = 0; j < 10; j++) Ib10[j] = LDG(sc, 15 + j);
+    const V<int> ob = eo + (NM_OFS(sc) + kScRec);
+    ldsv2(lds, ob + 6, Ib10);
+    ldsv4(lds, ob + 8, Ib10 + 2);
+    ldsv4(lds, ob + 12, Ib10 + 6);
     if (last) {
       vr ipos[3] = {vr(M.basec[0]), vr(M.basec[1]), vr(M.basec[2])};
       vr d[3];
@@ -549,8 +607,10 @@
       STG(bh, 0, LDG(qpos, 2) + d[2]);
     }
     vr fb[6];
-#pragma unroll
-    for (int j = 0; j < 6; j++) fb[j] = LDG(sc, 25 + j) + legsum<real>(fs[j], isleg);
+    ldsv4(lds, ob + 16, fb);
+    ldsv2(lds, ob + 20, fb + 4);
+#pragma unroll
+    for (int j = 0; j < 6; j++) fb[j] = fb[j] + legsum<real>(fs[j], isleg);
     cbias[0] = fb[3]; cbias[1] = fb[4]; cbias[2] = fb[5];
 #pragma unroll
     for (int j = 0; j < 3; j++) cbias[3 + j] = Rb[j] * fb[0] + Rb[3 + j] * fb[1] + Rb[6 + j] * fb[2];
@@ -582,9 +642,9 @@
 
   {
     sched_fence();
-    constexpr int kFacH = NM_OFS(MinvH) - NM_OFS(Minv);
-    static_assert(NM_OFS(WH) - NM_OFS(W) == kFacH && NM_OFS(LbH) - NM_OFS(Lb) == kFacH && NM_OFS(DbiH) - NM_OFS(Dbi) == kFacH, "factor blocks");
-    static_assert(kNLEG * 66 >= 36 + 24 + 24, "leg staging area holds the second Schur complement and the junk rows");
+    constexpr int kFacH = NM_OFS(facH) - NM_OFS(fac);
+    static_assert(NM_OFS(LbH) - NM_OFS(Lb) == kFacH && NM_OFS(DbiH) - NM_OFS(Dbi) == kFacH, "factor blocks");
+    static_assert(kNLEG * kLegTmp >= 36 + 24 + 24, "leg staging area holds the second Schur complement and the junk rows");
     const V<int> eoF = eo + sel(pass1, V<int>(kFacH), V<int>(0));
     const V<int> eoS = eo + sel(pass1, V<int>(NM_OFS(legtmp)), V<int>(NM_OFS(sc)));
     const V<int> eoQ = eo + sel(pass1, V<int>(NM_OFS(legtmp) + 36), V<int>(NM_OFS(qfs)));
@@ -600,12 +660,18 @@
       ldl3_solve(r3, Mi, col);
       W[0][j] = r3[0]; W[1][j] = r3[1]; W[2][j] = r3[2];
     }
-#pragma unroll
-    for (int j = 0; j < 6; j++) stsv(lds, eoF + leg * 6 + (NM_OFS(Minv) + j), Mi[j], st_leg);
-#pragma unroll
-    for (int k = 0; k < 3; k++)
-#pragma unroll
-      for (int j = 0; j < 6; j++) stsv(lds, eoF + leg * 18 + (NM_OFS(W) + 6 * k + j), W[k][j], st_leg);
+    {
+      const V<int> fo = eoF + (NM_OFS(fac) + leg * kFacN);
+      vr rec[kFacN];
+#pragma unroll
+      for (int k = 0; k < 3; k++)
+#pragma unroll
+        for (int j = 0; j < 6; j++) rec[kFacW + 6 * k + j] = W[k][j];
+#pragma unroll
+      for (int j = 0; j < 6; j++) rec[kFacMinv + j] = Mi[j];
+#pragma unroll
+      for (int j = 0; j < kFacN; j += 4) stsv4(lds, fo + j, rec + j, st_leg);
+    }
 #pragma unroll
     for (int i = 0; i < 6; i++)
 #pragma unroll
@@ -616,10 +682,15 @@
     wave_sync();
     vr L[15], Di[6];
     ldl6([&](int r, int c) { return ldsv(lds, eoS + (6 * r + c)); }, L, Di, real(1));
-#pragma unroll
-    for (int j = 0; j < 15; j++) stsv(lds, eoF + (NM_OFS(Lb) + j), L[j], st_all);
-#pragma unroll
-    for (int j = 0; j < 6; j++) stsv(lds, eoF + (NM_OFS(Dbi) + j), Di[j], st_all);
+    {
+      const vr Lp[4] = {L[12], L[13], L[14], L[14]};
+      stsv4(lds, eoF + NM_OFS(Lb), L, st_all);
+      stsv4(lds, eoF + (NM_OFS(Lb) + 4), L + 4, st_all);
+      stsv4(lds, eoF + (NM_OFS(Lb) + 8), L + 8, st_all);
+      stsv4(lds, eoF + (NM_OFS(Lb) + 12), Lp, st_all);
+      stsv4(lds, eoF + NM_OFS(Dbi), Di, st_all);
+      stsv2(lds, eoF + (NM_OFS(Dbi) + 4), Di + 4, st_all);
+    }
     {
       vr y[3], t[3];
 #pragma unroll
@@ -1324,12 +1395,9 @@
 #pragma unroll
     for (int k = 0; k < 3; k++) {
       vr a[3], r[3], rel[3], mm[3];
-#pragma unroll
-      for (int j = 0; j < 3; j++) {
-        a[j] = ldsv(sh.axs, Lc * 9 + (3 * k + j));
-        r[j] = ldsv(sh.anc, Lc * 9 + (3 * k + j));
-        rel[j] = cp[j] - r[j];
-      }
+      ld_jnt(sh.jnt, (Lc * 3 + k) * kJntN, r, a);
+#pragma unroll
+      for (int j = 0; j < 3; j++) rel[j] = cp[j] - r[j];
       cross3(mm, rel, e);
       Fl[k] = sel(onleg, dot3<vr>(a, mm), vr(real(0)));
     }
@@ -1338,12 +1406,9 @@
 #pragma unroll
     for (int k = 0; k < 3; k++) {
       vr a[3], r[3], rel[3], mm[3];
-#pragma unroll
-      for (int j = 0; j < 3; j++) {
-        a[j] = ldsv(sh.axs, Lc1 * 9 + (3 * k + j));
-        r[j] = ldsv(sh.anc, Lc1 * 9 + (3 * k + j));
-        rel[j] = cp[j] - r[j];
-      }
+      ld_jnt(sh.jnt, (Lc1 * 3 + k) * kJntN, r, a);
+#pragma unroll
+      for (int j = 0; j < 3; j++) rel[j] = cp[j] - r[j];
       cross3(mm, rel, e);
       Fm[k] = sel(onleg1 & act, -dot3<vr>(a, mm), vr(real(0)));
     }
@@ -1355,17 +1420,23 @@
 #pragma unroll
   for (int k = 0; k < 3; k++) Fl[k] = sel(act, Fl[k], vr(real(0)));
   vr uF[6];
-#pragma unroll
-  for (int j = 0; j < 6; j++) {
-    uF[j] = Fb[j];
-#pragma unroll
-    for (int k = 0; k < 3; k++) uF[j] = uF[j] - ldsv(sh.W, Lc * 18 + (6 * k + j)) * Fl[k];
+  {
+    vr W[18];
+    ld_facW(sh.fac, Lc * kFacN, W);
+#pragma unroll
+    for (int j = 0; j < 6; j++) {
+      uF[j] = Fb[j];
+#pragma unroll
+      for (int k = 0; k < 3; k++) uF[j] = uF[j] - W[6 * k + j] * Fl[k];
+    }
   }
   if (anypair) {
+    vr W[18];
+    ld_facW(sh.fac, Lc1 * kFacN, W);
 #pragma unroll
     for (int j = 0; j < 6; j++)
 #pragma unroll
-      for (int k = 0; k < 3; k++) uF[j] = uF[j] - ldsv(sh.W, Lc1 * 18 + (6 * k + j)) * Fm[k];
+      for (int k = 0; k < 3; k++) uF[j] = uF[j] - W[6 * k + j] * Fm[k];
   }
 #pragma unroll
   for (int j = 0; j < 6; j++) stsv(jrow, lane * kJRow + j, uF[j], lane < kMaxRow);
@@ -1432,13 +1503,11 @@
   vr t[3], t1m[3] = {vr(real(0)), vr(real(0)), vr(real(0))}, xb[6];
   {
     vr Mi[6];
-#pragma unroll
-    for (int j = 0; j < 6; j++) Mi[j] = ldsv(sh.Minv, Lc * 6 + j);
+    ld_facMinv(sh.fac, Lc * kFacN, Mi);
     ldl3_solve(t, Mi, Jl);
     if (anypair) {
       vr Mi1[6];
-#pragma unroll
-      for (int j = 0; j < 6; j++) Mi1[j] = ldsv(sh.Minv, Lc1 * 6 + j);
+      ld_facMinv(sh.fac, Lc1 * kFacN, Mi1);
       ldl3_solve(t1m, Mi1, Jm);
     }
 #pragma unroll
@@ -1701,12 +1770,9 @@
 #pragma unroll
     for (int k = 0; k < 3; k++) {
       vr a[3], r[3], rel[3], mm[3];
-#pragma unroll
-      for (int j = 0; j < 3; j++) {
-        a[j] = SHR(axs, Lc * 9 + (3 * k + j));
-        r[j] = SHR(anc, Lc * 9 + (3 * k + j));
-        rel[j] = cp[j] - r[j];
-      }
+      ld_jnt(rb, ho + (NM_OFS(jnt) + (Lc * 3 + k) * kJntN), r, a);
+#pragma unroll
+      for (int j = 0; j < 3; j++) rel[j] = cp[j] - r[j];
       cross3(mm, rel, e);
       Fl[k] = sel(onleg, dot3<vr>(a, mm), vr(real(0)));
     }
@@ -1716,11 +1782,15 @@
 #pragma unroll
   for (int k = 0; k < 3; k++) Fl[k] = sel(act, Fl[k], vr(real(0)));
   vr uF[6];
-#pragma unroll
-  for (int j = 0; j < 6; j++) {
-    uF[j] = Fb[j];
-#pragma unroll
-    for (int k = 0; k < 3; k++) uF[j] = uF[j] - SHR(W, Lc * 18 + (6 * k + j)) * Fl[k];
+  {
+    vr W[18];
+    ld_facW(rb, ho + (NM_OFS(fac) + Lc * kFacN), W);
+#pragma unroll
+    for (int j = 0; j < 6; j++) {
+      uF[j] = Fb[j];
+#pragma unroll
+      for (int k = 0; k < 3; k++) uF[j] = uF[j] - W[6 * k + j] * Fl[k];
+    }
   }
 #pragma unroll
   for (int j = 0; j < 6; j++) stsv(jrow, lane * kJRow + j, uF[j], VB(true));
@@ -1771,14 +1841,11 @@
   vr t[3], xb[6];
   {
     vr Mi[6];
-#pragma unroll
-    for (int j = 0; j < 6; j++) Mi[j] = SHR(Minv, Lc * 6 + j);
+    ld_facMinv(rb, ho + (NM_OFS(fac) + Lc * kFacN), Mi);
     ldl3_solve(t, Mi, Jl);
     vr Lbv[15], Dbv[6];
-#pragma unroll
-    for (int j = 0; j < 15; j++) Lbv[j] = SHR(Lb, V<int>(j));
-#pragma unroll
-    for (int j = 0; j < 6; j++) Dbv[j] = SHR(Dbi, V<int>(j));
+    ld_Lb(rb, ho + NM_OFS(Lb), Lbv);
+    ld_Dbi(rb, ho + NM_OFS(Dbi), Dbv);
 #pragma unroll
     for (int j = 0; j < 6; j++) xb[j] = u[j];
     ldl6_solve(Lbv, Dbv, xb);
@@ -1983,12 +2050,13 @@
   const VB isleg = lane < kNLEG;
   const V<int> leg = vmin(lane, V<int>(kNLEG - 1));
   vr t[3], Mi[6], xb[6];
-#pragma unroll
-  for (int j = 0; j < 6; j++) Mi[j] = ldsv(sh.Minv, leg * 6 + j);
+  ld_facMinv(sh.fac, leg * kFacN, Mi);
   ldl3_solve(t, Mi, yl);
+  vr W[18];
+  ld_facW(sh.fac, leg * kFacN, W);
 #pragma unroll
   for (int j = 0; j < 6; j++) {
-    vr wy = ldsv(sh.W, leg * 18 + j) * yl[0] + ldsv(sh.W, leg * 18 + (6 + j)) * yl[1] + ldsv(sh.W, leg * 18 + (12 + j)) * yl[2];
+    vr wy = W[j] * yl[0] + W[6 + j] * yl[1] + W[12 + j] * yl[2];
     xb[j] = vr(yb[j] - lanesum6<real>(sel(isleg, wy, vr(real(0)))));
   }
   {
@@ -2004,7 +2072,7 @@
   for (int k = 0; k < 3; k++) {
     x[k] = t[k];
 #pragma unroll
-    for (int j = 0; j < 6; j++) x[k] = x[k] - ldsv(sh.W, leg * 18 + (6 * k + j)) * xb[j];
+    for (int j = 0; j < 6; j++) x[k] = x[k] - W[6 * k + j] * xb[j];
   }
   wave_sync();
 #pragma unroll
@@ -2097,12 +2165,13 @@
 #pragma unroll
       for (int kk = 0; kk < 3; kk++) {
         vr a[3], rel[3], mm[3], a1[3], rel1[3], mm1[3];
+        vr an[3], an1[3];
+        ld_jnt(sh.jnt, (Lc * 3 + kk) * kJntN, an, a);
+        ld_jnt(sh.jnt, (Lc1 * 3 + kk) * kJntN, an1, a1);
 #pragma unroll
         for (int j = 0; j < 3; j++) {
-          a[j] = ldsv(sh.axs, Lc * 9 + (3 * kk + j));
-          rel[j] = cp[j] - ldsv(sh.anc, Lc * 9 + (3 * kk + j));
-          a1[j] = ldsv(sh.axs, Lc1 * 9 + (3 * kk + j));
-          rel1[j] = cp[j] - ldsv(sh.anc, Lc1 * 9 + (3 * kk + j));
+          rel[j] = cp[j] - an[j];
+          rel1[j] = cp[j] - an1[j];
         }
         cross3(mm, rel, e);
         cross3(mm1, rel1, e);
@@ -2113,11 +2182,16 @@
       for (int j = 0; j < 6; j++) Fb[j] = sel(act & !onleg1, Fb[j], vr(real(0)));
     }
     vr uF[6];
-#pragma unroll
-    for (int j = 0; j < 6; j++) {
-      uF[j] = Fb[j];
-#pragma unroll
-      for (int kk = 0; kk < 3; kk++) uF[j] = uF[j] - ldsv(sh.W, Lc * 18 + (6 * kk + j)) * Fl[kk] - ldsv(sh.W, Lc1 * 18 + (6 * kk + j)) * Fm[kk];
+    {
+      vr W[18], W1[18];
+      ld_facW(sh.fac, Lc * kFacN, W);
+      ld_facW(sh.fac, Lc1 * kFacN, W1);
+#pragma unroll
+      for (int j = 0; j < 6; j++) {
+        uF[j] = Fb[j];
+#pragma unroll
+        for (int kk = 0; kk < 3; kk++) uF[j] = uF[j] - W[6 * kk + j] * Fl[kk] - W1[6 * kk + j] * Fm[kk];
+      }
     }
     vr u[6];
 #pragma unroll
@@ -2166,8 +2240,8 @@
     vr t[3], t1m[3], xb[6];
     {
       vr Mi[6], Mi1[6];
-#pragma unroll
-      for (int j = 0; j < 6; j++) { Mi[j] = ldsv(sh.Minv, Lc * 6 + j); Mi1[j] = ldsv(sh.Minv, Lc1 * 6 + j); }
+      ld_facMinv(sh.fac, Lc * kFacN, Mi);
+      ld_facMinv(sh.fac, Lc1 * kFacN, Mi1);
       ldl3_solve(t, Mi, r.Jl[k]);
       ldl3_solve(t1m, Mi1, r.Jm[k]);
 #pragma unroll
@@ -2350,8 +2424,8 @@
   const VB isleg = sub < V<int>(6);
 #define LDG(field, i) ldsv(lds, eo + (NM_OFS(field) + (i)))
 #define LDL(field, idx) ldsv(lds, eo + (idx) + NM_OFS(field))
-  constexpr int kFacH = NM_OFS(MinvH) - NM_OFS(Minv);
-  static_assert(NM_OFS(WH) - NM_OFS(W) == kFacH && NM_OFS(LbH) - NM_OFS(Lb) == kFacH && NM_OFS(DbiH) - NM_OFS(Dbi) == kFacH, "factor blocks");
+  constexpr int kFacH = NM_OFS(facH) - NM_OFS(fac);
+  static_assert(NM_OFS(LbH) - NM_OFS(Lb) == kFacH && NM_OFS(DbiH) - NM_OFS(Dbi) == kFacH, "factor blocks");
   static_assert(sizeof(Sh<real>::mbb) / sizeof(real) >= 24 && sizeof(Sh<real>::sc) / sizeof(real) >= 28 && sizeof(Sh<real>::vv) / sizeof(real) >= 24, "junk rows");
   const V<int> eoF = eo + sel(pass1, V<int>(kFacH), V<int>(0));
   vr xl[3], xb[6];
@@ -2359,28 +2433,31 @@
     vr y[3], t[3], Mi[6];
 #pragma unroll
     for (int k = 0; k < 3; k++) y[k] = LDL(qfc, leg * 3 + (6 + k)) + sel(pass1, LDL(qfs, leg * 3 + (6 + k)), vr(real(0)));
-#pragma unroll
-    for (int j = 0; j < 6; j++) Mi[j] = ldsv(lds, eoF + leg * 6 + (NM_OFS(Minv) + j));
+    const V<int> fo = eoF + (NM_OFS(fac) + leg * kFacN);
+    ld_facMinv(lds, fo, Mi);
     ldl3_solve(t, Mi, y);
-#pragma unroll
-    for (int j = 0; j < 6; j++) {
-      vr wy = ldsv(lds, eoF + leg * 18 + (NM_OFS(W) + j)) * y[0] + ldsv(lds, eoF + leg * 18 + (NM_OFS(W) + 6 + j)) * y[1] +
-              ldsv(lds, eoF + leg * 18 + (NM_OFS(W) + 12 + j)) * y[2];
-      xb[j] = LDG(qfc, j) - legsum<real>(wy, isleg) + sel(pass1, LDG(qfs, j), vr(real(0)));
+    {
+      vr W[18];
+      ld_facW(lds, fo, W);
+#pragma unroll
+      for (int j = 0; j < 6; j++) {
+        vr wy = W[j] * y[0] + W[6 + j] * y[1] + W[12 + j] * y[2];
+        xb[j] = LDG(qfc, j) - legsum<real>(wy, isleg) + sel(pass1, LDG(qfs, j), vr(real(0)));
+      }
     }
     {
       vr L[15], Di[6];
-#pragma unroll
-      for (int j = 0; j < 15; j++) L[j] = ldsv(lds, eoF + (NM_OFS(Lb) + j));
-#pragma unroll
-      for (int j = 0; j < 6; j++) Di[j] = ldsv(lds, eoF + (NM_OFS(Dbi) + j));
+      ld_Lb(lds, eoF + NM_OFS(Lb), L);
+      ld_Dbi(lds, eoF + NM_OFS(Dbi), Di);
       ldl6_solve(L, Di, xb);
     }
+    vr W[18];
+    ld_facW(lds, fo, W);
 #pragma unroll
     for (int k = 0; k < 3; k++) {
       vr x = t[k];
 #pragma unroll
-      for (int j = 0; j < 6; j++) x = x - ldsv(lds, eoF + leg * 18 + (NM_OFS(W) + 6 * k + j)) * xb[j];
+      for (int j = 0; j < 6; j++) x = x - W[6 * k + j] * xb[j];
       xl[k] = x;
     }
   }
diff --git a/nightmare_rl_amd/csrc/simt.h b/nightmare_rl_amd/csrc/simt.h
--- a/nightmare_rl_amd/csrc/simt.h
+++ b/nightmare_rl_amd/csrc/simt.h
@@ -176,9 +176,22 @@
   T* p = m ? a + i : reinterpret_cast<T*>(sink) + NM_TID;
   *p = v;
 }
-#define NM_GLOBAL(T) __attribute__((address_space(1))) T
+typedef float nm_f2 __attribute__((ext_vector_type(2)));
 typedef float nm_f4 __attribute__((ext_vector_type(4)));
 typedef double nm_d4 __attribute__((ext_vector_type(4)));
+typedef double nm_d2 __attribute__((ext_vector_type(2)));
+NM_FN void ldsv2(const float* a, int i, float* o) { const nm_f2 t = *reinterpret_cast<const nm_f2*>(a + i); o[0] = t.x; o[1] = t.y; }
+NM_FN void ldsv2(const double* a, int i, double* o) { const nm_d2 t = *reinterpret_cast<const nm_d2*>(a + i); o[0] = t.x; o[1] = t.y; }
+NM_FN void ldsv4(const float* a, int i, float* o) {
+  const nm_f4 t = *reinterpret_cast<const nm_f4*>(a + i);
+  o[0] = t.x; o[1] = t.y; o[2] = t.z; o[3] = t.w;
+}
+NM_FN void ldsv4(const double* a, int i, double* o) { ldsv2(a, i, o); ldsv2(a, i + 2, o + 2); }
+NM_FN void stsv2(float* a, int i, const float* v, bool m) { if (m) *reinterpret_cast<nm_f2*>(a + i) = nm_f2{v[0], v[1]}; }
+NM_FN void stsv2(double* a, int i, const double* v, bool m) { if (m) *reinterpret_cast<nm_d2*>(a + i) = nm_d2{v[0], v[1]}; }
+NM_FN void stsv4(float* a, int i, const float* v, bool m) { if (m) *reinterpret_cast<nm_f4*>(a + i) = nm_f4{v[0], v[1], v[2], v[3]}; }
+NM_FN void stsv4(double* a, int i, const double* v, bool m) { stsv2(a, i, v, m); stsv2(a, i + 2, v + 2, m); }
+#define NM_GLOBAL(T) __attribute__((address_space(1))) T
 template <class T> NM_FN T gldv(const T* p, int i) { return ((const NM_GLOBAL(T)*)p)[i]; }
 template <class T> NM_FN void gstv(T* p, int i, T v, bool m) { if (m) ((NM_GLOBAL(T)*)p)[i] = v; }
 template <class T> NM_FN T gld1(const T* p, size_t i) { return ((const NM_GLOBAL(T)*)p)[i]; }
@@ -200,6 +213,8 @@
 
 #else
 #include <cmath>
+#include <cstdio>
+#include <cstdlib>
 #include <cstring>
 #define NM_FN inline
 #define NM_COLD inline
@@ -324,6 +339,24 @@
 template <class T> NM_FN void stsv(T* a, const V<int>& i, T v, const VB& m) { for (int k = 0; k < NM_WAVE; k++) if (m.v[k]) a[i.v[k]] = v; }
 template <class T, class S> NM_FN void stsu(T* a, const V<int>& i, const V<T>& v, const VB& m, S*) { stsv(a, i, v, m); }
 template <class T, class S> NM_FN void stsu(T* a, const V<int>& i, T v, const VB& m, S*) { stsv(a, i, v, m); }
+template <int N, class T> NM_FN void lds_rec_check(const T* a, int i) {
+  constexpr size_t al = N * sizeof(T) < 16 ? N * sizeof(T) : 16;
+  if ((i % N) != 0 || (reinterpret_cast<uintptr_t>(a + i) % al) != 0) { fprintf(stderr, "simt: misaligned %d-word LDS record\n", N); abort(); }
+}
+template <int N, class T> NM_FN void ldsvn(const T* a, const V<int>& i, V<T>* o) {
+  for (int k = 0; k < NM_WAVE; k++) { lds_rec_check<N>(a, i.v[k]); for (int c = 0; c < N; c++) o[c].v[k] = a[i.v[k] + c]; }
+}
+template <int N, class T> NM_FN void ldsvn(const T* a, int i, T* o) { lds_rec_check<N>(a, i); for (int c = 0; c < N; c++) o[c] = a[i + c]; }
+template <int N, class T> NM_FN void stsvn(T* a, const V<int>& i, const V<T>* v, const VB& m) {
+  for (int k = 0; k < NM_WAVE; k++) {
+    lds_rec_check<N>(a, i.v[k]);
+    if (m.v[k]) for (int c = 0; c < N; c++) a[i.v[k] + c] = v[c].v[k];
+  }
+}
+template <class T, class I, class X> NM_FN void ldsv2(const T* a, const I& i, X* o) { ldsvn<2>(a, i, o); }
+template <class T, class I, class X> NM_FN void ldsv4(const T* a, const I& i, X* o) { ldsvn<4>(a, i, o); }
+template <class T> NM_FN void stsv2(T* a, const V<int>& i, const V<T>* v, const VB& m) { stsvn<2>(a, i, v, m); }
+template <class T> NM_FN void stsv4(T* a, const V<int>& i, const V<T>* v, const VB& m) { stsvn<4>(a, i, v, m); }
 template <class T> NM_FN T gld1(const T* p, size_t i) { return p[i]; }
 template <class T> NM_FN void gst1(T* p, size_t i, T v) { p[i] = v; }
 NM_FN void gadd1(float* p, size_t i, float v) { p[i] += v; }
```

Result: no change. 84.32 million env-steps/s (median of 6 runs) (+0.4%).
